# wangkenpu/rsrgan

Hardware: AMD Instinct MI355X
Metric: GAN train frames/sec (G+D step), 257-dim LPS->40-dim MFCC (higher is better)
Workload: dtype f32

## Files before the change

include/rsrgan.h:

```cpp
#ifndef RSRGAN_H_
#define RSRGAN_H_

#include <stddef.h>
#include <stdint.h>

#ifdef __cplusplus
extern "C" {
#endif

typedef enum rsrgan_status {
  RSRGAN_OK = 0,
  RSRGAN_ERR_INVALID = -1,
  RSRGAN_ERR_HIP = -2,
  RSRGAN_ERR_NO_DEVICE = -3,
  RSRGAN_ERR_STATE = -4
} rsrgan_status;

enum { RSRGAN_G_LSTM = 0, RSRGAN_G_RES_LSTM_L = 1, RSRGAN_G_RES_LSTM_BASE = 2,
       RSRGAN_G_DNN = 3,
       RSRGAN_G_RCED = 4,
       RSRGAN_G_BNLSTM = 5 ,
       RSRGAN_G_RES_LSTM_I = 6  };
enum { RSRGAN_D_LSTM = 0, RSRGAN_D_DNN = 1  };
enum { RSRGAN_NET_G = 0, RSRGAN_NET_D = 1 };

typedef enum rsrgan_scalar {
  RSRGAN_G_LEARNING_RATE = 0,
  RSRGAN_D_LEARNING_RATE = 1,
  RSRGAN_MSE_LAMBDA = 2,
  RSRGAN_D_REAL = 3,
  RSRGAN_D_FAKE = 4,
  RSRGAN_L2_SCALE = 5,
  RSRGAN_CLIP_NORM = 6,
  RSRGAN_ADAM_STEP = 7,
  RSRGAN_ADAM_STEP_D = 8,
  RSRGAN_SCALAR_COUNT_
} rsrgan_scalar;

typedef struct rsrgan_cfg {
  int32_t batch_size;
  int32_t max_frames;
  int32_t input_dim;
  int32_t output_dim;
  int32_t g_type;
  int32_t g_layers;
  int32_t g_cells;
  int32_t g_proj;
  int32_t d_type;
  int32_t d_layers;
  int32_t d_cells;
  int32_t d_proj;
  float   l2_scale;
  float   clip_norm;
  float   adam_beta1;
  float   adam_beta2;
  float   adam_eps;
  float   ema_decay;
  float   lrelu_alpha;
  float   forget_bias;
  int32_t cross_validation;
  int32_t flags;
  int32_t d_joint_off;
  int32_t d_joint_dim;
  int32_t g_splice;
} rsrgan_cfg;

enum {
  RSRGAN_FLAG_WAVEFRONT = 1,
  RSRGAN_FLAG_GRAPH = 2,
  RSRGAN_FLAG_NO_SPLITK_B = 8,
  RSRGAN_FLAG_SUPERVISED = 16,
  RSRGAN_FLAG_OVERLAP = 4,
  RSRGAN_FLAG_BATCH_NORM = 32
};

typedef struct rsrgan_handle_s* rsrgan_handle;

int rsrgan_default_cfg(int32_t g_type, rsrgan_cfg* cfg);

int rsrgan_create(const rsrgan_cfg* cfg, uint64_t seed, rsrgan_handle* out);
int rsrgan_destroy(rsrgan_handle h);
const char* rsrgan_last_error(void);

int rsrgan_set_scalar(rsrgan_handle h, int32_t which, double v);
int rsrgan_get_scalar(rsrgan_handle h, int32_t which, double* v);

int rsrgan_num_tensors(rsrgan_handle h, int32_t net);
int rsrgan_tensor_info(rsrgan_handle h, int32_t net, int32_t idx,
                       char* name, int32_t name_cap,
                       int32_t* rows, int32_t* cols, int64_t* dense_offset);
int64_t rsrgan_param_count(rsrgan_handle h, int32_t net);

int rsrgan_get_params(rsrgan_handle h, int32_t net, int32_t what, float* dense, void* stream);
int rsrgan_set_params(rsrgan_handle h, int32_t net, int32_t what, const float* dense, void* stream);
int rsrgan_get_grads(rsrgan_handle h, int32_t net, float* dense, void* stream);

int rsrgan_forward_g(rsrgan_handle h, const float* x, const int32_t* lengths, int32_t T,
                     float* y, void* stream);

int rsrgan_g_state_floats(rsrgan_handle h, int32_t* n);
int rsrgan_g_state_reset(rsrgan_handle h, const int32_t* row_mask, void* stream);
int rsrgan_g_state_get(rsrgan_handle h, float* dst, void* stream);
int rsrgan_g_state_set(rsrgan_handle h, const float* src, void* stream);
int rsrgan_forward_g_stream(rsrgan_handle h, const float* x, const int32_t* lengths, int32_t T,
                            float* y, void* stream);

int rsrgan_d_step(rsrgan_handle h, const float* x, const float* labels, const int32_t* lengths,
                  int32_t T, const float* noise_real, const float* noise_fake,
                  float* out_losses, int32_t train, void* stream);

int rsrgan_g_step(rsrgan_handle h, const float* x, const float* labels, const int32_t* lengths,
                  int32_t T, const float* noise_fake, float* out_losses,
                  int32_t train, int32_t reuse_g_forward, void* stream);

int rsrgan_d_backward(rsrgan_handle h, const float* x, const float* labels, const int32_t* lengths,
                      int32_t T, const float* noise_real, const float* noise_fake,
                      float* out_losses, void* stream);
int rsrgan_g_backward(rsrgan_handle h, const float* x, const float* labels, const int32_t* lengths,
                      int32_t T, const float* noise_fake, float* out_losses,
                      int32_t reuse_g_forward, void* stream);
int rsrgan_apply(rsrgan_handle h, int32_t net, void* stream);
int rsrgan_grad_buffer(rsrgan_handle h, int32_t net, float** ptr, int64_t* count);
int rsrgan_grad_bucket_count(rsrgan_handle h, int32_t net);
int rsrgan_grad_bucket_info(rsrgan_handle h, int32_t net, int32_t i, int64_t* offset, int64_t* count);
int rsrgan_grad_bucket_wait(rsrgan_handle h, int32_t net, int32_t i, void* stream);

int rsrgan_profile_begin(rsrgan_handle h);
int rsrgan_profile_read(rsrgan_handle h, int32_t* launches, double* total_us, double* alg_flops);
int rsrgan_profile_read_kind(rsrgan_handle h, int32_t kind, int32_t* launches, double* total_us, double* alg_flops);

int rsrgan_device_status(rsrgan_handle h, int32_t* code);

int rsrgan_set_dropout(rsrgan_handle h, float keep_prob, uint64_t seed);

int rsrgan_profile_launches(rsrgan_handle h, int64_t* n);
int rsrgan_op_launch_floor(int32_t n, int32_t mode, double* us_per_launch, void* stream);

int rsrgan_op_gemm(const float* A, int32_t lda, int32_t a_kcontig,
                   const float* B, int32_t ldb, int32_t b_kcontig,
                   float* C, int32_t ldc, int32_t M, int32_t N, int32_t K,
                   const float* bias, int32_t act, float alpha, int32_t accumulate, void* stream);

int rsrgan_op_gemm2(const float* A, int32_t lda, int32_t a_kcontig, const float* A2, int32_t lda2, int32_t M1,
                    const float* B, int32_t ldb, int32_t b_kcontig, float* C, int32_t ldc, int32_t M, int32_t N, int32_t K,
                    const float* bias, int32_t act, float alpha, int32_t accumulate,
                    int32_t map_rows_per, int64_t map_outer, int64_t map_inner, int32_t workers, int32_t force_cfg, void* stream);
#define RSRGAN_OP_NOT_APPLICABLE 1
int rsrgan_op_gemm_batch(int32_t nb, const float* const* A, int32_t lda, const float* const* A2, int32_t lda2, int32_t M1,
                         const float* const* B, int32_t ldb, float* const* C, int32_t ldc, int32_t M, int32_t N, int32_t K,
                         int32_t accumulate, int32_t workers, void* stream);
int rsrgan_op_gemm16_batch(int32_t n, const float* const* A, int32_t lda, const float* const* A2, int32_t lda2, int32_t M1,
                           const float* const* B, int32_t ldb, float* const* C, int32_t ldc, int32_t M, int32_t N, int32_t K,
                           int32_t accumulate, void* stream);
int rsrgan_op_gemm_last_plan(int32_t out[8]);
int rsrgan_op_lstm_colsums(int32_t nb, const float* const* dz, const float* const* cprev, const float* const* ccur, float* const* db,
                           float* const* dwi, float* const* dwf, float* const* dwo, int32_t rows, int32_t H, void* stream);
int rsrgan_op_colsum(const float* a, int32_t lda, const float* b, int32_t ldb, float* out, int32_t rows, int32_t cols, int32_t tall,
                     void* stream);

typedef struct rsrgan_segan_cfg {
  int32_t batch_size;
  int32_t input_len;
  int32_t output_dim;
  int32_t n_layers;
  int32_t g_depths[16];
  int32_t d_depths[16];
  int32_t g_kwidth;
  int32_t d_kwidth;
  int32_t g_prelu;
  float   lrelu_alpha;
  float   vbn_eps;
  float   rms_decay;
  float   rms_eps;
} rsrgan_segan_cfg;
typedef struct rsrgan_segan_handle_s* rsrgan_segan_handle;
enum { RSRGAN_SEGAN_G_LR = 0, RSRGAN_SEGAN_D_LR = 1, RSRGAN_SEGAN_L1_LAMBDA = 2 };
int rsrgan_segan_default_cfg(rsrgan_segan_cfg* cfg);
int rsrgan_segan_create(const rsrgan_segan_cfg* cfg, uint64_t seed, rsrgan_segan_handle* out);
int rsrgan_segan_destroy(rsrgan_segan_handle h);
int rsrgan_segan_set_scalar(rsrgan_segan_handle h, int32_t which, double v);
int rsrgan_segan_num_tensors(rsrgan_segan_handle h, int32_t net);
int rsrgan_segan_tensor_info(rsrgan_segan_handle h, int32_t net, int32_t idx, char* name, int32_t name_cap, int32_t* rows, int32_t* cols,
                             int64_t* dense_offset);
int64_t rsrgan_segan_param_count(rsrgan_segan_handle h, int32_t net);
int rsrgan_segan_get_params(rsrgan_segan_handle h, int32_t net, int32_t what, float* dense, void* stream);
int rsrgan_segan_set_params(rsrgan_segan_handle h, int32_t net, int32_t what, const float* dense, void* stream);
int rsrgan_segan_forward_g(rsrgan_segan_handle h, const float* x, const float* z, float* y, void* stream);
int rsrgan_segan_d_backward(rsrgan_segan_handle h, const float* x, const float* labels, const float* z, const float* noise_ref,
                            const float* noise_real, const float* noise_fake, float* out_losses, int32_t train, void* stream);
int rsrgan_segan_g_backward(rsrgan_segan_handle h, const float* x, const float* labels, const float* z, const float* noise_ref,
                            const float* noise_fake, float* out_losses, int32_t train, void* stream);
int rsrgan_segan_grad_buffer(rsrgan_segan_handle h, int32_t net, float** ptr, int64_t* count);
int rsrgan_segan_apply(rsrgan_segan_handle h, int32_t net, void* stream);

int rsrgan_version(void);

#ifdef __cplusplus
}
#endif
#endif
```

rsrgan_amd/_lib.py:

```python
from __future__ import annotations

import ctypes as C
import os

_HERE = os.path.dirname(os.path.abspath(__file__))
LIB_PATH = os.path.join(_HERE, "lib", "librsrgan_hip.so")

G_TYPES = {"lstm": 0, "res_lstm_l": 1, "res_lstm_base": 2, "dnn": 3, "rced": 4, "bnlstm": 5, "res_lstm_i": 6}
FLAG_BATCH_NORM = 32
D_TYPES = {"lstm": 0, "dnn": 1}
NET_G, NET_D = 0, 1
SCALARS = {"g_learning_rate": 0, "d_learning_rate": 1, "mse_lambda": 2, "d_real": 3, "d_fake": 4,
           "l2_scale": 5, "clip_norm": 6, "adam_step": 7, "adam_step_d": 8}
WHAT = {"variables": 0, "adam_m": 1, "adam_v": 2, "ema": 3}

SYMBOLS = ["rsrgan_default_cfg", "rsrgan_create", "rsrgan_destroy", "rsrgan_last_error", "rsrgan_set_scalar",
           "rsrgan_get_scalar", "rsrgan_num_tensors", "rsrgan_tensor_info", "rsrgan_param_count",
           "rsrgan_get_params", "rsrgan_set_params", "rsrgan_get_grads", "rsrgan_forward_g",
           "rsrgan_g_state_floats", "rsrgan_g_state_reset", "rsrgan_g_state_get", "rsrgan_g_state_set", "rsrgan_forward_g_stream",
           "rsrgan_d_step",
           "rsrgan_g_step", "rsrgan_d_backward", "rsrgan_g_backward", "rsrgan_apply", "rsrgan_grad_buffer",
           "rsrgan_grad_bucket_count", "rsrgan_grad_bucket_info", "rsrgan_grad_bucket_wait",
           "rsrgan_profile_begin", "rsrgan_profile_read", "rsrgan_profile_read_kind", "rsrgan_profile_launches", "rsrgan_op_launch_floor", "rsrgan_device_status", "rsrgan_set_dropout",
           "rsrgan_op_gemm", "rsrgan_op_gemm2", "rsrgan_op_gemm_batch", "rsrgan_op_gemm16_batch", "rsrgan_op_gemm_last_plan",
           "rsrgan_op_lstm_colsums", "rsrgan_op_colsum", "rsrgan_version",
           "rsrgan_segan_default_cfg", "rsrgan_segan_create", "rsrgan_segan_destroy", "rsrgan_segan_set_scalar",
           "rsrgan_segan_num_tensors", "rsrgan_segan_tensor_info", "rsrgan_segan_param_count", "rsrgan_segan_get_params",
           "rsrgan_segan_set_params", "rsrgan_segan_forward_g", "rsrgan_segan_d_backward", "rsrgan_segan_g_backward",
           "rsrgan_segan_grad_buffer", "rsrgan_segan_apply"]


class RsrganCfg(C.Structure):
    _fields_ = [("batch_size", C.c_int32), ("max_frames", C.c_int32), ("input_dim", C.c_int32),
                ("output_dim", C.c_int32), ("g_type", C.c_int32), ("g_layers", C.c_int32), ("g_cells", C.c_int32),
                ("g_proj", C.c_int32), ("d_type", C.c_int32), ("d_layers", C.c_int32), ("d_cells", C.c_int32),
                ("d_proj", C.c_int32), ("l2_scale", C.c_float), ("clip_norm", C.c_float), ("adam_beta1", C.c_float),
                ("adam_beta2", C.c_float), ("adam_eps", C.c_float), ("ema_decay", C.c_float),
                ("lrelu_alpha", C.c_float), ("forget_bias", C.c_float), ("cross_validation", C.c_int32),
                ("flags", C.c_int32), ("d_joint_off", C.c_int32), ("d_joint_dim", C.c_int32), ("g_splice", C.c_int32)]


class SeganCfg(C.Structure):
    _fields_ = [("batch_size", C.c_int32), ("input_len", C.c_int32), ("output_dim", C.c_int32), ("n_layers", C.c_int32),
                ("g_depths", C.c_int32 * 16), ("d_depths", C.c_int32 * 16), ("g_kwidth", C.c_int32), ("d_kwidth", C.c_int32),
                ("g_prelu", C.c_int32), ("lrelu_alpha", C.c_float), ("vbn_eps", C.c_float), ("rms_decay", C.c_float),
                ("rms_eps", C.c_float)]


class RsrganError(RuntimeError):
    pass


_lib = None


def load():
    global _lib
    if _lib is not None:
        return _lib
    if not os.path.exists(LIB_PATH):
        raise ImportError("%s is missing: build it with `python -c 'import __graft_entry__ as g; g.build()'` "
                          "(hipcc --offload-arch=gfx950); rsrgan_amd has no CPU fallback" % LIB_PATH)
    lib = C.CDLL(LIB_PATH)
    p, i32, i64, f32, vp = C.c_void_p, C.c_int32, C.c_int64, C.c_float, C.c_void_p
    lib.rsrgan_last_error.restype = C.c_char_p
    lib.rsrgan_default_cfg.argtypes = [i32, C.POINTER(RsrganCfg)]
    lib.rsrgan_create.argtypes = [C.POINTER(RsrganCfg), C.c_uint64, C.POINTER(vp)]
    lib.rsrgan_destroy.argtypes = [vp]
    lib.rsrgan_set_scalar.argtypes = [vp, i32, C.c_double]
    lib.rsrgan_get_scalar.argtypes = [vp, i32, C.POINTER(C.c_double)]
    lib.rsrgan_num_tensors.argtypes = [vp, i32]
    lib.rsrgan_tensor_info.argtypes = [vp, i32, i32, C.c_char_p, i32, C.POINTER(i32), C.POINTER(i32), C.POINTER(i64)]
    lib.rsrgan_param_count.argtypes = [vp, i32]
    lib.rsrgan_param_count.restype = i64
    lib.rsrgan_get_params.argtypes = [vp, i32, i32, p, vp]
    lib.rsrgan_set_params.argtypes = [vp, i32, i32, p, vp]
    lib.rsrgan_get_grads.argtypes = [vp, i32, p, vp]
    lib.rsrgan_forward_g.argtypes = [vp, p, p, i32, p, vp]
    lib.rsrgan_g_state_floats.argtypes = [vp, C.POINTER(i32)]
    lib.rsrgan_g_state_reset.argtypes = [vp, p, vp]
    lib.rsrgan_g_state_get.argtypes = [vp, p, vp]
    lib.rsrgan_g_state_set.argtypes = [vp, p, vp]
    lib.rsrgan_forward_g_stream.argtypes = [vp, p, p, i32, p, vp]
    lib.rsrgan_d_step.argtypes = [vp, p, p, p, i32, p, p, p, i32, vp]
    lib.rsrgan_g_step.argtypes = [vp, p, p, p, i32, p, p, i32, i32, vp]
    lib.rsrgan_d_backward.argtypes = [vp, p, p, p, i32, p, p, p, vp]
    lib.rsrgan_g_backward.argtypes = [vp, p, p, p, i32, p, p, i32, vp]
    lib.rsrgan_apply.argtypes = [vp, i32, vp]
    lib.rsrgan_grad_buffer.argtypes = [vp, i32, C.POINTER(p), C.POINTER(i64)]
    lib.rsrgan_grad_bucket_count.argtypes = [vp, i32]
    lib.rsrgan_grad_bucket_info.argtypes = [vp, i32, i32, C.POINTER(i64), C.POINTER(i64)]
    lib.rsrgan_grad_bucket_wait.argtypes = [vp, i32, i32, vp]
    lib.rsrgan_profile_begin.argtypes = [vp]
    lib.rsrgan_profile_read.argtypes = [vp, C.POINTER(i32), C.POINTER(C.c_double), C.POINTER(C.c_double)]
    lib.rsrgan_profile_read_kind.argtypes = [vp, i32, C.POINTER(i32), C.POINTER(C.c_double), C.POINTER(C.c_double)]
    lib.rsrgan_device_status.argtypes = [vp, C.POINTER(i32)]
    lib.rsrgan_set_dropout.argtypes = [vp, f32, C.c_uint64]
    lib.rsrgan_profile_launches.argtypes = [vp, C.POINTER(i64)]
    lib.rsrgan_op_launch_floor.argtypes = [i32, i32, C.POINTER(C.c_double), vp]
    lib.rsrgan_op_gemm.argtypes = [p, i32, i32, p, i32, i32, p, i32, i32, i32, i32, p, i32, f32, i32, vp]
    pp = C.POINTER(C.c_void_p)
    lib.rsrgan_op_gemm2.argtypes = [p, i32, i32, p, i32, i32, p, i32, i32, p, i32, i32, i32, i32, p, i32, f32, i32, i32, i64, i64, i32, i32, vp]
    lib.rsrgan_op_gemm_batch.argtypes = [i32, pp, i32, pp, i32, i32, pp, i32, pp, i32, i32, i32, i32, i32, i32, vp]
    lib.rsrgan_op_gemm16_batch.argtypes = [i32, pp, i32, pp, i32, i32, pp, i32, pp, i32, i32, i32, i32, i32, vp]
    lib.rsrgan_op_gemm_last_plan.argtypes = [C.POINTER(i32)]
    lib.rsrgan_op_lstm_colsums.argtypes = [i32, pp, pp, pp, pp, pp, pp, pp, i32, i32, vp]
    lib.rsrgan_op_colsum.argtypes = [p, i32, p, i32, p, i32, i32, i32, vp]
    lib.rsrgan_segan_default_cfg.argtypes = [C.POINTER(SeganCfg)]
    lib.rsrgan_segan_create.argtypes = [C.POINTER(SeganCfg), C.c_uint64, C.POINTER(vp)]
    lib.rsrgan_segan_destroy.argtypes = [vp]
    lib.rsrgan_segan_set_scalar.argtypes = [vp, i32, C.c_double]
    lib.rsrgan_segan_num_tensors.argtypes = [vp, i32]
    lib.rsrgan_segan_tensor_info.argtypes = [vp, i32, i32, C.c_char_p, i32, C.POINTER(i32), C.POINTER(i32), C.POINTER(i64)]
    lib.rsrgan_segan_param_count.argtypes = [vp, i32]
    lib.rsrgan_segan_param_count.restype = i64
    lib.rsrgan_segan_get_params.argtypes = [vp, i32, i32, p, vp]
    lib.rsrgan_segan_set_params.argtypes = [vp, i32, i32, p, vp]
    lib.rsrgan_segan_forward_g.argtypes = [vp, p, p, p, vp]
    lib.rsrgan_segan_d_backward.argtypes = [vp, p, p, p, p, p, p, p, i32, vp]
    lib.rsrgan_segan_g_backward.argtypes = [vp, p, p, p, p, p, p, i32, vp]
    lib.rsrgan_segan_grad_buffer.argtypes = [vp, i32, C.POINTER(p), C.POINTER(i64)]
    lib.rsrgan_segan_apply.argtypes = [vp, i32, vp]
    _lib = lib
    return lib


OP_NOT_APPLICABLE = 1
GEMM_CLASSES = {0: "none", 1: "gemm16", 2: "n32", 3: "k_gemm", 4: "k_gemm_s", 5: "gemm16_batch", 6: "k_gemm_batch", 7: "k_gemm_s_batch"}
GEMM_PLAN_FIELDS = ("cls", "bm", "bn", "W", "n_dp", "fixup", "splits", "Ur")
GEMM_FORMS = [("k_gemm", 128, 128), ("k_gemm", 96, 128), ("k_gemm", 128, 96), ("k_gemm", 256, 64), ("k_gemm", 256, 32),
              ("k_gemm_s", 256, 256), ("k_gemm_s", 128, 256), ("k_gemm_s", 256, 128)]


def ptr_table(ptrs):
    return (C.c_void_p * max(len(ptrs), 1))(*[None if q is None else q for q in ptrs])


def check(rc):
    if rc != 0:
        raise RsrganError("librsrgan_hip error %d: %s" % (rc, load().rsrgan_last_error().decode()))
```

rsrgan_amd/csrc/capi.cpp:

```cpp
#include <cstring>
#include <exception>
#include <new>
#include <vector>

#include "model.h"

using namespace rsr;

struct rsrgan_handle_s { Model m; };

#define CHECK_H(h)                                                    \
  if (!(h)) { set_error("null handle"); return RSRGAN_ERR_INVALID; }

template <class F>
static int guard(const char* what, F&& body) {
  try {
    return body();
  } catch (const std::bad_alloc&) {
    set_error("%s: out of host memory", what);
  } catch (const std::exception& e) {
    set_error("%s: %s", what, e.what());
  } catch (...) {
    set_error("%s: unknown C++ exception", what);
  }
// ... 459 lines not shown
  if (g) (void)hipGraphDestroy(g);
  if (s) (void)hipStreamDestroy(s);
  (void)stream;
  return rc;
}

static const size_t g_op_ws_floats = (size_t)32 << 20;
static const size_t g_op_scratch_floats = (size_t)2 << 20;
static float* op_ws() {
  static float* ws = nullptr;
  if (!ws && hipMalloc((void**)&ws, g_op_ws_floats * sizeof(float)) != hipSuccess) ws = nullptr;
  return ws;
}
static float* op_scratch() {
  static float* sc = nullptr;
  if (!sc && hipMalloc((void**)&sc, g_op_scratch_floats * sizeof(float)) != hipSuccess) sc = nullptr;
  return sc;
}
#define OP_REFUSE(cond, ...) do { if (cond) { set_error(__VA_ARGS__); return RSRGAN_ERR_INVALID; } } while (0)
struct WorkersScope {
  int saved;
  explicit WorkersScope(int w) : saved(g_gemm_workers) { if (w > 0) g_gemm_workers = w; }
  ~WorkersScope() { g_gemm_workers = saved; }
};

int rsrgan_op_gemm(const float* A, int32_t lda, int32_t a_kc, const float* B, int32_t ldb, int32_t b_kc, float* C, int32_t ldc,
                   int32_t M, int32_t N, int32_t K, const float* bias, int32_t act, float alpha, int32_t accumulate, void* stream) {
  if (!A || !B || !C || (lda & 3) || (ldb & 3)) { set_error("op_gemm: null pointer or leading dimension not a multiple of 4"); return RSRGAN_ERR_INVALID; }
  float* ws = op_ws();
  launch_gemm(A, lda, a_kc != 0, B, ldb, b_kc != 0, C, ldc, M, N, K, bias, act, alpha, accumulate != 0, (hipStream_t)stream,
              ws, ws ? g_op_ws_floats : 0);
  if (hipGetLastError() != hipSuccess) { set_error("op_gemm launch failed"); return RSRGAN_ERR_HIP; }
  return RSRGAN_OK;
}

int rsrgan_op_gemm2(const float* A, int32_t lda, int32_t a_kc, const float* A2, int32_t lda2, int32_t M1, const float* B, int32_t ldb,
                    int32_t b_kc, float* C, int32_t ldc, int32_t M, int32_t N, int32_t K, const float* bias, int32_t act, float alpha,
                    int32_t accumulate, int32_t map_rows_per, int64_t map_outer, int64_t map_inner, int32_t workers, int32_t force_cfg,
                    void* stream) {
  OP_REFUSE(!A || !B || !C, "op_gemm2: null pointer (A, B or C)");
  OP_REFUSE(M <= 0 || N <= 0 || K <= 0, "op_gemm2: M, N, K must be positive (got %d, %d, %d)", M, N, K);
  OP_REFUSE((lda & 3) || (ldb & 3) || (ldc & 3) || (A2 && (lda2 & 3)), "op_gemm2: leading dimension not a multiple of 4 (lda %d, lda2 %d, ldb %d, ldc %d)", lda, lda2, ldb, ldc);
  OP_REFUSE(workers < 0 || workers > 256, "op_gemm2: workers = %d outside 0 (default) .. 256", workers);
  OP_REFUSE(force_cfg < -1 || force_cfg > 7, "op_gemm2: force_cfg = %d outside -1 (planner) .. 7", force_cfg);
  OP_REFUSE(map_rows_per < 0, "op_gemm2: row map with rows_per = %d", map_rows_per);
  if (map_rows_per > 0) {
    OP_REFUSE(A2 != nullptr, "op_gemm2: A2 together with a row map");
    OP_REFUSE(b_kc != 0, "op_gemm2: a row map together with b_kcontig");
    OP_REFUSE((map_outer & 3) || (map_inner & 3), "op_gemm2: row map strides not multiples of 4 (outer %lld, inner %lld)", (long long)map_outer, (long long)map_inner);
  }
  if (A2) {
    OP_REFUSE(a_kc != 0, "op_gemm2: A2 together with a_kcontig (the stacked operand is m-contiguous)");
    OP_REFUSE(M1 <= 0 || M1 >= M, "op_gemm2: M1 = %d outside (0, M = %d)", M1, M);
    OP_REFUSE(M1 & 3, "op_gemm2: M1 = %d is not a multiple of 4: every kernel moves the stacked operand in 16-byte chunks", M1);
  }
  float* ws = op_ws();
  {
    WorkersScope wsc(workers);
    const GemmRowMap ma{map_rows_per, (long long)map_outer, (long long)map_inner};
    launch_gemm_mapped(A, lda, ma, A2, lda2, M1, a_kc != 0, B, ldb, b_kc != 0, C, ldc, M, N, K, bias, act, alpha, accumulate != 0,
                       (hipStream_t)stream, ws, ws ? g_op_ws_floats : 0, force_cfg);
  }
  if (hipGetLastError() != hipSuccess) { set_error("op_gemm2 launch failed"); return RSRGAN_ERR_HIP; }
  return RSRGAN_OK;
}

int rsrgan_op_gemm_batch(int32_t nb, const float* const* A, int32_t lda, const float* const* A2, int32_t lda2, int32_t M1,
                         const float* const* B, int32_t ldb, float* const* C, int32_t ldc, int32_t M, int32_t N, int32_t K,
                         int32_t accumulate, int32_t workers, void* stream) {
  OP_REFUSE(nb < 1 || nb > 64, "op_gemm_batch: nb = %d outside 1 .. 64 (more than %d: not applicable)", nb, GEMM_MAXB);
  OP_REFUSE(!A || !B || !C, "op_gemm_batch: null pointer table (A, B or C)");
  for (int b = 0; b < nb; ++b) OP_REFUSE(!A[b] || !B[b] || !C[b] || (A2 && !A2[b]), "op_gemm_batch: null pointer in problem %d", b);
  OP_REFUSE(M <= 0 || N <= 0 || K <= 0, "op_gemm_batch: M, N, K must be positive (got %d, %d, %d)", M, N, K);
  OP_REFUSE((lda & 3) || (ldb & 3) || (ldc & 3) || (A2 && (lda2 & 3)), "op_gemm_batch: leading dimension not a multiple of 4 (lda %d, lda2 %d, ldb %d, ldc %d)", lda, lda2, ldb, ldc);
  OP_REFUSE(workers < 0 || workers > 256, "op_gemm_batch: workers = %d outside 0 (default) .. 256", workers);
  if (A2) {
    OP_REFUSE(M1 <= 0 || M1 >= M, "op_gemm_batch: M1 = %d outside (0, M = %d)", M1, M);
    OP_REFUSE(M1 & 3, "op_gemm_batch: M1 = %d is not a multiple of 4: the kernels move the stacked operand in 16-byte chunks", M1);
  }
  float* ws = op_ws();
  bool ran;
  {
    WorkersScope wsc(workers);
    ran = launch_gemm_batch(nb, A, lda, A2, lda2, M1, B, ldb, C, ldc, M, N, K, accumulate != 0, (hipStream_t)stream, ws, ws ? g_op_ws_floats : 0);
  }
  if (hipGetLastError() != hipSuccess) { set_error("op_gemm_batch launch failed"); return RSRGAN_ERR_HIP; }
  return ran ? RSRGAN_OK : RSRGAN_OP_NOT_APPLICABLE;
}

int rsrgan_op_gemm16_batch(int32_t n, const float* const* A, int32_t lda, const float* const* A2, int32_t lda2, int32_t M1,
                           const float* const* B, int32_t ldb, float* const* C, int32_t ldc, int32_t M, int32_t N, int32_t K,
                           int32_t accumulate, void* stream) {
  OP_REFUSE(n < 1 || n > GEMM16_MAXB, "op_gemm16_batch: n = %d outside the table (1 .. %d)", n, GEMM16_MAXB);
  OP_REFUSE(!A || !B || !C, "op_gemm16_batch: null pointer table (A, B or C)");
  for (int p = 0; p < n; ++p) OP_REFUSE(!A[p] || !B[p] || !C[p] || (A2 && !A2[p]), "op_gemm16_batch: null pointer in problem %d", p);
  OP_REFUSE(M <= 0 || N <= 0 || K <= 0, "op_gemm16_batch: M, N, K must be positive (got %d, %d, %d)", M, N, K);
  OP_REFUSE((lda & 3) || (ldb & 3) || (ldc & 3) || (A2 && (lda2 & 3)), "op_gemm16_batch: leading dimension not a multiple of 4 (lda %d, lda2 %d, ldb %d, ldc %d)", lda, lda2, ldb, ldc);
  if (A2) {
    OP_REFUSE(M1 <= 0 || M1 >= M, "op_gemm16_batch: M1 = %d outside (0, M = %d)", M1, M);
    OP_REFUSE(M1 & 3, "op_gemm16_batch: M1 = %d is not a multiple of 4: k_gemm16 loads the stacked operand as float4", M1);
  }
  Gemm16Batch bt{};
  bt.n = n;
  for (int p = 0; p < n; ++p) { bt.A[p] = A[p]; bt.A2[p] = A2 ? A2[p] : nullptr; bt.B[p] = B[p]; bt.C[p] = C[p]; }
  float* ws = op_ws();
  launch_gemm16_batch(bt, lda, lda2, M1, ldb, ldc, M, N, K, accumulate != 0, (hipStream_t)stream, ws, ws ? g_op_ws_floats : 0);
  if (hipGetLastError() != hipSuccess) { set_error("op_gemm16_batch launch failed"); return RSRGAN_ERR_HIP; }
  return RSRGAN_OK;
}

int rsrgan_op_gemm_last_plan(int32_t out[8]) {
  OP_REFUSE(!out, "op_gemm_last_plan: null pointer");
  const GemmPlanRecord& r = g_gemm_last_plan;
  out[0] = r.cls; out[1] = r.bm; out[2] = r.bn; out[3] = r.W; out[4] = r.n_dp; out[5] = r.fixup; out[6] = r.splits; out[7] = r.Ur;
  return RSRGAN_OK;
}

int rsrgan_op_lstm_colsums(int32_t nb, const float* const* dz, const float* const* cprev, const float* const* ccur, float* const* db,
                           float* const* dwi, float* const* dwf, float* const* dwo, int32_t rows, int32_t H, void* stream) {
  OP_REFUSE(nb < 1 || nb > 4, "op_lstm_colsums: nb = %d outside the table (1 .. 4)", nb);
  OP_REFUSE(!dz || !cprev || !ccur || !db || !dwi || !dwf || !dwo, "op_lstm_colsums: null pointer table");
  for (int p = 0; p < nb; ++p)
    OP_REFUSE(!dz[p] || !cprev[p] || !ccur[p] || !db[p] || !dwi[p] || !dwf[p] || !dwo[p], "op_lstm_colsums: null pointer in layer %d", p);
  OP_REFUSE(rows <= 0 || H <= 0, "op_lstm_colsums: rows and H must be positive (got %d, %d)", rows, H);
  OP_REFUSE((size_t)nb * 64 * 7 * (size_t)H > g_op_scratch_floats, "op_lstm_colsums: nb x 64 x 7 x H = %zu floats of partials exceed the entry's scratch", (size_t)nb * 64 * 7 * (size_t)H);
  float* sc = op_scratch();
  if (!sc) { set_error("op_lstm_colsums: hipMalloc failed"); return RSRGAN_ERR_HIP; }
  if (nb == 1) launch_lstm_colsums(dz[0], cprev[0], ccur[0], db[0], dwi[0], dwf[0], dwo[0], rows, H, sc, (hipStream_t)stream);
  else {
    ColsumsBatch cb{};
    cb.n = nb;
    for (int p = 0; p < nb; ++p) { cb.dz[p] = dz[p]; cb.cprev[p] = cprev[p]; cb.ccur[p] = ccur[p]; cb.db[p] = db[p]; cb.dwi[p] = dwi[p]; cb.dwf[p] = dwf[p]; cb.dwo[p] = dwo[p]; }
    launch_lstm_colsums_batch(cb, rows, H, sc, (hipStream_t)stream);
  }
  if (hipGetLastError() != hipSuccess) { set_error("op_lstm_colsums launch failed"); return RSRGAN_ERR_HIP; }
  return RSRGAN_OK;
}

int rsrgan_op_colsum(const float* a, int32_t lda, const float* b, int32_t ldb, float* out, int32_t rows, int32_t cols, int32_t tall,
                     void* stream) {
  OP_REFUSE(!a || !out, "op_colsum: null pointer (a or out)");
  OP_REFUSE(rows <= 0 || cols <= 0, "op_colsum: rows and cols must be positive (got %d, %d)", rows, cols);
  OP_REFUSE(lda < cols || (b && ldb < cols), "op_colsum: leading dimension below cols = %d (lda %d, ldb %d)", cols, lda, ldb);
  OP_REFUSE(tall && b, "op_colsum: the tall form has no multiplier b");
  OP_REFUSE((size_t)(tall ? 512 : 64) * (size_t)cols > g_op_scratch_floats, "op_colsum: cols = %d exceeds the entry's scratch", cols);
  float* sc = op_scratch();
  if (!sc) { set_error("op_colsum: hipMalloc failed"); return RSRGAN_ERR_HIP; }
  if (tall) launch_colsum_tall(a, lda, out, rows, cols, sc, g_op_scratch_floats, (hipStream_t)stream);
  else launch_colsum(a, lda, b, ldb, out, rows, cols, sc, (hipStream_t)stream);
  if (hipGetLastError() != hipSuccess) { set_error("op_colsum launch failed"); return RSRGAN_ERR_HIP; }
  return RSRGAN_OK;
}

}
```

rsrgan_amd/csrc/dnn.cpp:

```cpp
#include "model.h"

namespace rsr {

#define HIPC(expr)                                                                   \
  do {                                                                               \
    hipError_t e_ = (expr);                                                          \
    if (e_ != hipSuccess) {                                                          \
      set_error("%s failed: %s (%s:%d)", #expr, hipGetErrorString(e_), __FILE__, __LINE__); \
      return RSRGAN_ERR_HIP;                                                         \
    }                                                                                \
  } while (0)

static const float kDClipLo = -0.5f, kDClipHi = 1.5f;

BnVars Model::bn_vars(const ParamSet& ps, const int (&tbn)[8]) const {
  BnVars v;
  v.beta = ps.W(tbn[0]); v.gamma = ps.W(tbn[1]); v.mm = ps.W(tbn[2]); v.mv = ps.W(tbn[3]);
  v.rm = ps.W(tbn[4]); v.rmw = ps.W(tbn[5]); v.rs = ps.W(tbn[6]); v.rsw = ps.W(tbn[7]);
  return v;
}
BnVars Model::bn_vars(const ParamSet& ps, const FcLayer& F) const { return bn_vars(ps, F.tbn); }

static inline uint64_t splitmix64(uint64_t x) {
  x += 0x9E3779B97F4A7C15ull;
// ... 68 lines not shown

void Model::rced_forward(int rows, hipStream_t s) {
  const size_t M = (size_t)rows * rcS * rcW;
  for (size_t l = 0; l < gconv.size(); ++l) {
    const ConvLayer& L = gconv[l];
    if (rc_ft_fwd[l]) {
      const float* src = rc_act[l];
      int ldc = L.ldCin;
      if (l == 0) { launch_expand_c4(x_tm, ldDin, rcS * rcW, rc_x4, (size_t)rows, s); src = rc_x4; ldc = 4; }
      launch_conv_fwd(src, ldc, L.Cin, rc_ft_fwd[l], L.bn ? nullptr : G.W(L.tb), !L.bn, L.bn ? L.pre : rc_act[l + 1], L.ldCout, L.Cout, rows,
                      rcS, rcW, L.fw, s);
    } else {
      float* col = rc_keep_cols ? rc_cols[l] : rc_col;
      launch_im2col(rc_act[l], l == 0 ? (size_t)ldDin : (size_t)rcS * rcW * L.ldCin, L.ldCin, L.Cin, rcS, rcW, rcS, L.fw, col, L.ldK, M, s);
      gemm(col, L.ldK, true, G.W(L.tW), L.ldCout, false, L.bn ? L.pre : rc_act[l + 1], L.ldCout, (int)M, L.Cout, L.K, L.bn ? nullptr : G.W(L.tb),
           L.bn ? 0 : 2, 0.f, false, s);
    }
    if (L.bn)
      launch_bn_forward(L.pre, L.ldCout, rc_act[l + 1], L.ldCout, (int)M, L.Cout, bn_vars(G, L.tbn), L.stat, L.ldCout, bn_training(), true,
                        scratch, scratch_floats, s);
  }
  gemm(rc_act[gconv.size()], rc_fc.ld_in, true, G.W(rc_fc.tW), ldDout, false, y_tm, ldDout, rows, Dout, rc_fc.in, G.W(rc_fc.tb), 0, 0.f, false, s);
}

void Model::rced_backward(int rows, float* dy, hipStream_t s) {
  const size_t M = (size_t)rows * rcS * rcW;
  const int Lc = (int)gconv.size();
  gemm(rc_act[Lc], rc_fc.ld_in, false, dy, ldDout, false, G.Gd(rc_fc.tW), ldDout, rc_fc.in, Dout, rows, nullptr, 0, 0.f, false, s);
  launch_colsum(dy, ldDout, nullptr, 0, G.Gd(rc_fc.tb), rows, Dout, scratch, s);
  float* d = rc_dA;
  float* other = rc_dB;
  gemm(dy, ldDout, true, G.W(rc_fc.tW), ldDout, true, d, rc_fc.ld_in, rows, rc_fc.in, Dout, nullptr, 0, 0.f, false, s);
  bool d_masked = false;
  for (int l = Lc - 1; l >= 0; --l) {
    const ConvLayer& L = gconv[l];
    if (L.bn)
      launch_bn_backward(d, L.ldCout, rc_act[l + 1], L.ldCout, L.pre, L.ldCout, (int)M, L.Cout, L.stat, L.ldCout, G.Gd(L.tbn[0]), G.Gd(L.tbn[1]),
                         false, true, bn_sums, scratch, scratch_floats, s);
    else if (!d_masked)
      launch_lrelu_bwd(rc_act[l + 1], d, M, L.Cout, L.ldCout, 0.f, s);
    d_masked = false;
    bool db_done = false;
    if (rc_wgrad_implicit[l] && rc_wg_ws) {
      launch_conv_wgrad(l == 0 ? rc_x4 : rc_act[l], l == 0 ? 4 : L.ldCin, L.Cin, d, L.ldCout, L.Cout, G.Gd(L.tW), L.ldCout, rc_wg_ws, rows,
                        rcS, rcW, L.fw, s, L.bn ? nullptr : G.Gd(L.tb));
      db_done = !L.bn;
    } else {
      float* col = rc_keep_cols ? rc_cols[l] : rc_col;
      if (!rc_keep_cols)
        launch_im2col(rc_act[l], l == 0 ? (size_t)ldDin : (size_t)rcS * rcW * L.ldCin, L.ldCin, L.Cin, rcS, rcW, rcS, L.fw, col, L.ldK, M, s);
      gemm(col, L.ldK, false, d, L.ldCout, false, G.Gd(L.tW), L.ldCout, L.K, L.Cout, (int)M, nullptr, 0, 0.f, false, s);
    }
    if (!L.bn && !db_done) launch_colsum_tall(d, L.ldCout, G.Gd(L.tb), (int)M, L.Cout, scratch, scratch_floats, s);
    if (l > 0) {
      if (rc_ft_bwd[l]) {
        d_masked = !gconv[l - 1].bn;
        launch_conv_fwd(d, L.ldCout, L.Cout, rc_ft_bwd[l], nullptr, false, other, L.ldCin, L.Cin, rows, rcS, rcW, L.fw, s,
                        d_masked ? rc_act[l] : nullptr);
      } else {
        gemm(d, L.ldCout, true, G.W(L.tW), L.ldCout, true, rc_dcol, L.ldK, (int)M, L.K, L.Cout, nullptr, 0, 0.f, false, s);
        launch_col2im(rc_dcol, L.ldK, L.Cin, rcS, rcW, rcS, L.fw, other, L.ldCin, M, s);
      }
      std::swap(d, other);
    }
  }
}

void Model::g_frame_forward(int rows, hipStream_t s) {
  if (g_rced()) rced_forward(rows, s);
  else fc_forward(G, gfc, g_act, rows, s);
}
void Model::g_frame_backward(int rows, float* dy, hipStream_t s) {
  if (g_rced()) rced_backward(rows, dy, s);
  else fc_backward(G, gfc, g_act, rows, dy, true, false, s);
}

void Model::bn_commit_run(bool with_d, hipStream_t s) {
  BnCommitList cl; cl.n = 0;
  bn_commit_stack(G, gfc, 2, 0, cl);
  for (const ConvLayer& L : gconv)
    if (L.bn && cl.n < 24) cl.e[cl.n++] = BnCommit{bn_vars(G, L.tbn), L.stat, L.Cout, L.ldCout, 2, 0};
  if (with_d) bn_commit_stack(D, dfc, 2, 1, cl);
  launch_bn_commit_many(cl, s);
}

void Model::d_dnn_forward_loss(int T, int Nd, int n_real, bool want_grads, float* loss3, hipStream_t s, int calls, int call0) {
  fc_forward(D, dfc, d_act, T * Nd, s, calls, call0);
  launch_lsgan(logits, 4, want_grads ? dlogits : nullptr, T, Nd, n_real, dyn + DYN_D_REAL,
               n_real > 0 ? dyn + DYN_D_FAKE : dyn + DYN_D_REAL, loss3, s, true, kDClipLo, kDClipHi);
}

int Model::dnn_d_backward(const float* x, const float* labels, int T, float* out_losses, bool want_grads, hipStream_t s) {
  const int R = T * B;
  if (!x || !labels) { set_error("null input pointer"); return RSRGAN_ERR_INVALID; }
  if (T <= 0 || T > Tmax) { set_error("T=%d outside (0, max_frames=%d]", T, Tmax); return RSRGAN_ERR_INVALID; }
  bn_eval_call = !want_grads;
  if (want_grads) ++drop_run;
  launch_pack_tm(x, x_tm, B, T, Din, ldDin, s);
  launch_pack_tm(labels, lab_tm, B, T, Dout, ldDout, s);
  cur_T = T;
  g_frame_forward(R, s);
  g_fwd_valid = true;
  launch_build_joint(x_tm, ldDin, cfg.d_joint_off, cfg.d_joint_dim, lab_tm, ldDout, Dout, joint, ldJ, 0, R, s);
  launch_build_joint(x_tm, ldDin, cfg.d_joint_off, cfg.d_joint_dim, y_tm, ldDout, Dout, joint, ldJ, R, R, s);
  d_dnn_forward_loss(1, 2 * R, R, want_grads, losses, s, 2);
  if (want_grads) {
    fc_backward(D, dfc, d_act, 2 * R, dlogits, true, false, s, 2);
    if (bn_training()) bn_commit_run(true, s);
    { finish_buckets(RSRGAN_NET_D, s); d_grads_ready = true; }
  }
  if (out_losses) launch_copy_f(losses, out_losses, 3, s);
  HIPC(hipGetLastError());
  return RSRGAN_OK;
}

int Model::dnn_g_backward(const float* x, const float* labels, int T, float* out_losses, bool want_grads, bool reuse, hipStream_t s) {
  const int R = T * B;
  bn_eval_call = !want_grads;
  if (bn_on()) reuse = false;
  if (want_grads) ++drop_run;
  if (drop_training()) reuse = false;
  if (reuse) {
    if (!g_fwd_valid || T != cur_T) { set_error("reuse_g_forward without a valid generator forward"); return RSRGAN_ERR_STATE; }
  } else {
    if (!x || !labels) { set_error("null input pointer"); return RSRGAN_ERR_INVALID; }
    if (T <= 0 || T > Tmax) { set_error("T=%d outside (0, max_frames=%d]", T, Tmax); return RSRGAN_ERR_INVALID; }
    launch_pack_tm(x, x_tm, B, T, Din, ldDin, s);
    launch_pack_tm(labels, lab_tm, B, T, Dout, ldDout, s);
    cur_T = T;
    g_frame_forward(R, s);
    g_fwd_valid = true;
  }
  const bool sup = supervised();
  if (sup) {
    HIPC(hipMemsetAsync(losses + 3, 0, sizeof(float), s));
  } else if (bn_training() && want_grads) {
    launch_build_joint(x_tm, ldDin, cfg.d_joint_off, cfg.d_joint_dim, lab_tm, ldDout, Dout, joint, ldJ, 0, R, s);
    launch_build_joint(x_tm, ldDin, cfg.d_joint_off, cfg.d_joint_dim, y_tm, ldDout, Dout, joint, ldJ, R, R, s);
    fc_forward(D, dfc, d_act, 2 * R, s, 2);
    launch_lsgan(logits + (size_t)R * 4, 4, dlogits + (size_t)R * 4, 1, R, 0, dyn + DYN_D_REAL, dyn + DYN_D_REAL, tmp3, s, true, kDClipLo, kDClipHi);
    launch_copy_f(tmp3 + 1, losses + 3, 1, s);
  } else {
    launch_build_joint(x_tm, ldDin, cfg.d_joint_off, cfg.d_joint_dim, y_tm, ldDout, Dout, joint, ldJ, 0, R, s);
    d_dnn_forward_loss(1, R, 0, want_grads, tmp3, s, 1, 1);
    launch_copy_f(tmp3 + 1, losses + 3, 1, s);
  }
  const bool l2_on = !cfg.cross_validation && scal[RSRGAN_L2_SCALE] > 0.0;
  if (want_grads) {
    if (!sup) {
      float* dj = bn_training() ? fc_backward(D, dfc, d_act, R, dlogits + (size_t)R * 4, false, true, s, 1, R, 1)
                                : fc_backward(D, dfc, d_act, R, dlogits, false, true, s);
      launch_slice_cols(dj, ldJ, cfg.d_joint_dim, dy_buf, ldDout, R, Dout, s);
    }
    launch_mse(y_tm, lab_tm, ldDout, dy_buf, R, Dout, dyn + DYN_LAMBDA, !sup, losses + 4, scratch, s);
    g_frame_backward(R, dy_buf, s);
    if (l2_on) {
      launch_l2(G.w, G.g, G.ct, dyn + DYN_L2, G.partial, s);
      launch_l2_total(G.partial, G.ct.n_chunks, dyn + DYN_L2, losses + 5, s);
    }
    if (bn_training()) bn_commit_run(!sup, s);
    { finish_buckets(RSRGAN_NET_G, s); g_grads_ready = true; }
  } else {
    launch_mse(y_tm, lab_tm, ldDout, nullptr, R, Dout, dyn + DYN_LAMBDA, false, losses + 4, scratch, s);
  }
  if (!(want_grads && l2_on)) HIPC(hipMemsetAsync(losses + 5, 0, sizeof(float), s));
  launch_g_total(losses + 3, dyn + DYN_LAMBDA, s);
  if (out_losses) launch_copy_f(losses + 3, out_losses, 4, s);
  HIPC(hipGetLastError());
  return RSRGAN_OK;
}

}
```

rsrgan_amd/csrc/kernels.h:

```cpp
#pragma once
#include <hip/hip_runtime.h>
#include <stdint.h>

#include "switches.h"

namespace rsr {

constexpr int MAXJ = 8;

struct Place { int x0, nx, sb, se, nb, w; };
constexpr int JOBMAP_MAX = 768;
struct JobMap { int valid; unsigned char job[JOBMAP_MAX]; };
struct PlanItem { int ncol, nrow; double cost; int mult; };
int plan_places(int n, const PlanItem* items, Place* out);

enum { DYN_G_LR = 0, DYN_D_LR = 1, DYN_LAMBDA = 2, DYN_D_REAL = 3, DYN_D_FAKE = 4, DYN_L2 = 5, DYN_CLIP = 6,
       DYN_B1 = 7, DYN_B2 = 8, DYN_EPS = 9, DYN_EMA = 10, DYN_ADAM_LRT = 11, DYN_ADAM_LRT_D = 12, DYN_COUNT = 16 };

struct FwdGateJob {
  const float* x;
  const float* KxT;
  const float* m;
  const float* KhT;
  const float* Wsw;
// ... 136 lines not shown
  const float *KxT, *KhT;
  const float *bias, *wi, *wf, *wo, *Wp;
  float *gates, *c, *h, *mst, *out;
  const float* in;
  float* dmt;
  int I, P, ldI, ldP, ldH;
  float* res_out;
};
struct GPersistArgs {
  GPersistLayer L[GP_MAXL];
  int nl, N, T, H;
  int NT, NC;
  const int* len;
  unsigned long long *gran1, *gran2;
  unsigned* ctl;
  float forget_bias;
  unsigned long long* gran3;
  const float* dout_top;
  int ld_dout;
  float* din0;
  int ld_din0;
  int res;
  int tags;
  int dout_trail;
  int fwd_trail;
  int ngl, grp0;
  int nrt;
  int sched;
  int carry;
};
constexpr int GP_TMAX = 2046;
bool gpersist_plan(GPersistArgs& a);
void gpersist_arm_bytes(void* p, size_t bytes, hipStream_t s);
extern thread_local int g_gemm_workers;
int gpersist_grid(const GPersistArgs& a);
int gpersist_dt_grid(const GPersistArgs& a, const DPersistArgs& d);
void launch_glstm_fwd_dt(const GPersistArgs& a, const DPersistArgs& d, hipStream_t s);
size_t dpersist_fwdt_lds_bytes();
void launch_glstm_bwd_dt(const GPersistArgs& a, const DPersistArgs& d, hipStream_t s);
size_t gpersist_lds_bytes();
int device_cu_count();
bool resident_probe(int grid, int threads, size_t lds_bytes);
size_t gpersist_gran1_bytes(const GPersistArgs& a);
size_t gpersist_gran2_bytes(const GPersistArgs& a);
size_t gpersist_gran3_bytes(const GPersistArgs& a);
void gpersist_arm(const GPersistArgs& a, hipStream_t s);
void launch_glstm_fwd(const GPersistArgs& a, hipStream_t s);
bool gpersist_np_plan(GPersistArgs& a, int nt_force = 0);
size_t gpersist_np_gran2_bytes(const GPersistArgs& a);
size_t gpersist_np_lds_bytes();
void launch_glstm_np_fwd(const GPersistArgs& a, hipStream_t s);
size_t gpersist_np_gran1_bytes(const GPersistArgs& a);
size_t gpersist_np_gran3_bytes(const GPersistArgs& a);
void gpersist_np_arm(const GPersistArgs& a, hipStream_t s);
void launch_glstm_np_bwd(const GPersistArgs& a, hipStream_t s);
void launch_glstm_bwd(const GPersistArgs& a, hipStream_t s);
extern long long g_chain_launches;
void launch_floor_chain(float* a, float* b, int n, int mode, hipStream_t s);

struct GemmRowMap { int rows_per; long long outer; long long inner; };
enum { GEMM_CLS_NONE = 0, GEMM_CLS_GEMM16 = 1, GEMM_CLS_N32 = 2, GEMM_CLS_KGEMM = 3, GEMM_CLS_KGEMM_S = 4, GEMM_CLS_GEMM16_B = 5,
       GEMM_CLS_KGEMM_B = 6, GEMM_CLS_KGEMM_S_B = 7 };
struct GemmPlanRecord { int cls, bm, bn, W, n_dp, fixup, splits, Ur; };
extern thread_local GemmPlanRecord g_gemm_last_plan;
void launch_gemm_mapped(const float* A, int lda, const GemmRowMap& ma, const float* A2, int lda2, int M1, bool a_kc, const float* B, int ldb,
                        bool b_kc, float* C, int ldc, int M, int N, int K, const float* bias, int act, float alpha,
                        bool accumulate, hipStream_t s, float* ws, size_t ws_floats, int force_cfg = -1);
constexpr int GEMM16_MAXB = 4;
struct Gemm16Batch { const float* A[GEMM16_MAXB]; const float* A2[GEMM16_MAXB]; const float* B[GEMM16_MAXB]; float* C[GEMM16_MAXB]; int n; };
void launch_gemm16_batch(const Gemm16Batch& bt, int lda, int lda2, int M1, int ldb, int ldc, int M, int N, int K, bool accumulate,
                         hipStream_t s, float* ws, size_t ws_floats);
void launch_gemm2(const float* A, int lda, const float* A2, int lda2, int M1, bool a_kc, const float* B, int ldb, bool b_kc,
                  float* C, int ldc, int M, int N, int K, const float* bias, int act, float alpha, bool accumulate,
                  hipStream_t s, float* ws, size_t ws_floats);
constexpr int GEMM_MAXB = 4;
bool launch_gemm_batch(int nb, const float* const* A, int lda, const float* const* A2, int lda2, int M1, const float* const* B, int ldb,
                       float* const* C, int ldc, int M, int N, int K, bool accumulate, hipStream_t s, float* ws, size_t ws_floats);
void launch_gemm(const float* A, int lda, bool a_kc, const float* B, int ldb, bool b_kc,
                 float* C, int ldc, int M, int N, int K,
                 const float* bias, int act, float alpha, bool accumulate, hipStream_t s,
                 float* splitk_ws = nullptr, size_t splitk_ws_floats = 0);

struct StagePack { const float* src; float* dst; int D, ld; };
struct StageCopy { const void* src; void* dst; int n; };
struct StageJobs { StagePack pack[2]; StageCopy copy[4]; int B, T; int Bt; };
void launch_stage_inputs(const StageJobs& j, hipStream_t s);
void launch_pack_tm(const float* src_bm, float* dst_tm, int B, int T, int D, int ld, hipStream_t s);
void launch_unpack_bm(const float* src_tm, int ld, float* dst_bm, int B, int T, int D, hipStream_t s, int Bt = 0);
void launch_build_d_input(const float* lab_tm, const float* y_tm, const float* noise_r, const float* noise_f,
                          float* xd, int B, int T, int D, int ld, bool with_real, hipStream_t s);
void launch_add_noise_rows(const float* src_tm, const float* noise, float* dst, int B, int T, int D, int ld,
                           int Ns, int row0, hipStream_t s);
void launch_transpose(const float* src, int lds, float* dst, int ldd, int R, int C, hipStream_t s);
void launch_fill(float* p, size_t n, float v, hipStream_t s);
struct SwizzleJob { const float* src; float* dst; int ld, gates, H, C, c0, K1, I, P, kx, nct, nkb, blk_base; };
struct SwizzleList { int n; SwizzleJob j[24]; };
void launch_swizzle_many(SwizzleList& sl, hipStream_t s);
inline size_t swizzle_floats(int nct, int nkb) { return (size_t)nct * nkb * 256; }
struct TransposeJob { const float* src; float* dst; int lds, ldd, R, C, blk_base; };
struct TransposeList { int n; TransposeJob j[16]; };
void launch_transpose_many(TransposeList& tl, hipStream_t s);
size_t conv_prep_floats(int S, int fw, int C);
void launch_conv_prep(const float* F, int ldf_src, int S, int fw, int Cin, int Cout, bool flip, float* Ft, hipStream_t s);
bool conv_fwd_supported(int C, int N, int S, int W, int fw);
void launch_conv_fwd(const float* in, int ldc_in, int C, const float* Ft, const float* bias, bool relu, float* out, int ldc_out, int N,
                     int R, int S, int W, int fw, hipStream_t s,
                     const float* mask = nullptr );
bool conv_wgrad_supported(int C, int N, int S, int W, int fw);
size_t conv_wgrad_ws_floats(int C, int R, int S, int W, int fw);
void launch_conv_wgrad(const float* in, int ldc_in, int C, const float* d, int ldc_d, int N, float* dW, int ldw, float* ws, int R, int S,
                       int W, int fw, hipStream_t s,
                       float* db = nullptr );
void launch_im2col(const float* src, size_t row_stride, int ldc, int C, int S, int W, int kh, int kw, float* col, int ldk, size_t M,
                   hipStream_t s);
void launch_expand_c4(const float* src, int ld_src, int n, float* dst, size_t rows, hipStream_t s);
void launch_col2im(const float* dcol, int ldk, int C, int S, int W, int kh, int kw, float* dst, int ldc, size_t M, hipStream_t s);
struct GStateLayer { float *c, *mst; int H, P, ldP, off; };
struct GStateArgs { GStateLayer L[GP_MAXL]; int nl, SF, rows, dir; float* state; size_t slot; const int* mask; };
void launch_gstate(const GStateArgs& a, hipStream_t s);
struct ZeroList { int n; float* p[32]; unsigned len[32]; };
void launch_zero_many(const ZeroList& zl, hipStream_t s);
struct ColsumsBatch { const float* dz[4]; const float* cprev[4]; const float* ccur[4]; float* db[4]; float* dwi[4]; float* dwf[4]; float* dwo[4]; int n; };
void launch_lstm_colsums_batch(const ColsumsBatch& bt, int rows, int H, float* scratch, hipStream_t s);
void launch_lstm_colsums(const float* dz, const float* cprev, const float* ccur, float* db, float* dwi, float* dwf, float* dwo,
                         int rows, int H, float* scratch , hipStream_t s);
void launch_lrelu_bwd(const float* hval, float* d, size_t rows, int cols, int ld, float alpha, hipStream_t s);
void launch_dropout_fwd(float* y, size_t rows, int cols, int ld, unsigned long long key, unsigned thr, float keep, hipStream_t s);
void launch_dropout_bwd(const float* y, float* d, size_t rows, int cols, int ld, float keep, hipStream_t s);
void launch_colsum_tall(const float* a, int lda, float* out, int rows, int cols, float* scratch, size_t scratch_floats, hipStream_t s);

struct BnVars {
  float *beta, *gamma;
  float *mm, *mv, *rm, *rmw, *rs, *rsw;
};
constexpr int BN_STAT_ROWS = 6;
void launch_bn_forward(const float* z, int ldz, float* y, int ldy, int rows, int cols, const BnVars& v, float* stat, int ldc, bool training,
                       bool relu, float* scratch, size_t scratch_floats, hipStream_t s, int calls = 1);
void launch_bn_backward(float* dy, int ldd, const float* y, int ldy, const float* z, int ldz, int rows, int cols, const float* stat, int ldc,
                        float* dbeta, float* dgamma, bool accumulate, bool relu, float* sums, float* scratch, size_t scratch_floats,
                        hipStream_t s, int calls = 1);
void launch_bn_commit(int cols, const BnVars& v, const float* stat, int ldc, int times, hipStream_t s);
struct BnCommit { BnVars v; const float* stat; int cols, ldc, times0, times1; };
struct BnCommitList { int n; BnCommit e[24]; };
void launch_bn_commit_many(const BnCommitList& cl, hipStream_t s);
void launch_colsum(const float* a, int lda, const float* b, int ldb, float* out, int rows, int cols,
                   float* scratch , hipStream_t s);

constexpr int DH_MAXR = 64;
struct DHeadArgs {
  const float* top; int ldt; const float* w; int ldw; const float* b;
  float* logits; int ldl; float* dlogits; float* dout; int ldo; float* gw; float* gb;
  int T, Nd, n_real, dR; const float* t_real; const float* t_fake; float* loss3; float* part; int want_grads, want_wgrads;
  int Bp, Bt;
};
void launch_dhead(const DHeadArgs& a, hipStream_t s);
void launch_lsgan(const float* logits, int ldl, float* dlogits, int T, int Nd, int n_real,
                  const float* target_real, const float* target_fake, float* loss3, hipStream_t s,
                  bool clip_on = false, float clip_lo = 0.f, float clip_hi = 0.f, int Bp = 0, int Bt = 0);
void launch_build_joint(const float* x, int ldx, int off, int dim, const float* tail, int ldt, int Dt, float* joint, int ldj,
                        int row0, int R, hipStream_t s);
void launch_slice_cols(const float* src, int lds, int off, float* dst, int ldd, int R, int C, hipStream_t s);
void launch_mse(const float* y, const float* lab, int ld, float* dy, int rows, int D, const float* lambda,
                bool accumulate, float* loss_out, float* scratch , hipStream_t s, int Bp = 0, int Bt = 0);
void launch_g_total(float* l4 , const float* lambda, hipStream_t s);
void launch_copy_f(const float* src, float* dst, int n, hipStream_t s);

struct ChunkTable {
  const int* tensor;
  const int* off;
  const int* len;
  const int* t_first;
  const int* t_count;
  const int* t_l2;
  int n_chunks, n_tensors;
};
void launch_sumsq(const float* g, const ChunkTable& ct, float* partial, hipStream_t s);
void launch_dw_reduce(const float* ws, size_t stride, int ntiles, const long long* src, float* g, const ChunkTable& ct, float* partial, hipStream_t s);
void launch_l2(const float* w, float* g, const ChunkTable& ct, const float* l2_scale, float* partial, hipStream_t s);
void launch_l2_total(const float* partial, int n_chunks, const float* l2_scale, float* out, hipStream_t s);
void launch_apply_sgd(float* w, const float* g, float* ema, const ChunkTable& ct, const float* partial,
                      const float* dyn, hipStream_t s);
void launch_apply_adam(float* w, const float* g, float* m, float* v, float* ema, const ChunkTable& ct,
                       const float* partial, const float* dyn, hipStream_t s, int lrt_slot = DYN_ADAM_LRT);
void launch_adam_tick(float* dyn, int* t, double b1, double b2, hipStream_t s, int lr_slot = DYN_G_LR, int lrt_slot = DYN_ADAM_LRT);
void launch_pad_copy(const float* dense, float* padded, int rows, int cols, int ld, bool to_padded, hipStream_t s);

}
```

rsrgan_amd/csrc/kernels.hip:

```cpp
#include <algorithm>
#include <cstdlib>

#include "kernels.h"

namespace rsr {

typedef float f32x4 __attribute__((ext_vector_type(4)));

__device__ __forceinline__ float sigmoid_(float x) { return 1.0f / (1.0f + expf(-x)); }

#ifdef RSR_TRACE
__device__ unsigned long long g_trace[8192 * 16];
#define TR_BEGIN() do { if (threadIdx.x == 0 && blockIdx.x < 8192) { unsigned long long* t_ = g_trace + (size_t)blockIdx.x * 16; \
    t_[0] = __builtin_amdgcn_s_memrealtime(); t_[1] = __builtin_amdgcn_s_memtime(); \
    t_[14] = __builtin_amdgcn_s_getreg(4 | (0 << 6) | (31 << 11)); t_[15] = __builtin_amdgcn_s_getreg(20 | (0 << 6) | (3 << 11)); \
    for (int i_ = 2; i_ < 14; ++i_) t_[i_] = 0; } } while (0)
#define TR_ID(ptr) do { if (threadIdx.x == 0 && blockIdx.x < 8192) g_trace[(size_t)blockIdx.x * 16 + 12] = (unsigned long long)(size_t)(ptr); } while (0)
#define TR(i) do { if (threadIdx.x == 0 && blockIdx.x < 8192) g_trace[(size_t)blockIdx.x * 16 + (i)] = __builtin_amdgcn_s_memtime(); } while (0)
#define TR_END() do { if (threadIdx.x == 0 && blockIdx.x < 8192) { g_trace[(size_t)blockIdx.x * 16 + 9] = __builtin_amdgcn_s_memtime(); \
    g_trace[(size_t)blockIdx.x * 16 + 13] = __builtin_amdgcn_s_memrealtime(); } } while (0)
#else
#define TR_BEGIN() do { } while (0)
#define TR_ID(ptr) do { } while (0)
#define TR(i) do { } while (0)
// ... 1346 lines not shown
  __syncthreads();
  if (g == 0 && c < cols) out[c] = ((red[0][threadIdx.x] + red[1][threadIdx.x]) + red[2][threadIdx.x]) + red[3][threadIdx.x];
}
void launch_colsum_tall(const float* a, int lda, float* out, int rows, int cols, float* scratch, size_t scratch_floats, hipStream_t s) {
  int slices = (int)std::min<size_t>(512, scratch_floats / (size_t)std::max(cols, 1));
  slices = std::max(1, std::min(slices, (rows + 63) / 64));
  const int per = (rows + slices - 1) / slices;
  slices = (rows + per - 1) / per;
  hipLaunchKernelGGL(k_colsum1_n, dim3((cols + 63) / 64, slices), dim3(256), 0, s, a, lda, scratch, rows, cols, per);
  hipLaunchKernelGGL(k_colsum2_n, dim3((cols + 63) / 64), dim3(256), 0, s, scratch, out, cols, slices);
}

__global__ __launch_bounds__(256) void k_lstm_colsums1(const float* __restrict__ dz, const float* __restrict__ cprev,
                                                       const float* __restrict__ ccur, float* __restrict__ scratch, int rows, int H) {
  __shared__ float red[7][4][64];
  const int c = blockIdx.x * 64 + (threadIdx.x & 63), rl = threadIdx.x >> 6;
  const int per = (rows + CS_SLICES - 1) / CS_SLICES;
  const int rbeg = blockIdx.y * per, rend = min(rows, rbeg + per);
  float s[7] = {0.f, 0.f, 0.f, 0.f, 0.f, 0.f, 0.f};
  if (c < H) {
#pragma unroll 4
    for (int r = rbeg + rl; r < rend; r += 4) {
      const float* z = dz + (size_t)r * 4 * H + c;
      const float di = z[0], dj = z[H], df = z[2 * H], d_o = z[3 * H];
      const float cp = cprev[(size_t)r * H + c], cc = ccur[(size_t)r * H + c];
      s[0] += di; s[1] += dj; s[2] += df; s[3] += d_o; s[4] += di * cp; s[5] += df * cp; s[6] += d_o * cc;
    }
  }
#pragma unroll
  for (int k = 0; k < 7; ++k) red[k][rl][threadIdx.x & 63] = s[k];
  __syncthreads();
  if (rl == 0 && c < H) {
    const int x = threadIdx.x;
#pragma unroll
    for (int k = 0; k < 7; ++k)
      scratch[((size_t)blockIdx.y * 7 + k) * H + c] = ((red[k][0][x] + red[k][1][x]) + red[k][2][x]) + red[k][3][x];
  }
}
__global__ void k_lstm_colsums2(const float* __restrict__ scratch, float* __restrict__ db, float* __restrict__ dwi,
                                float* __restrict__ dwf, float* __restrict__ dwo, int H) {
  const int c = blockIdx.x * blockDim.x + threadIdx.x;
  if (c >= H) return;
  float s[7] = {0.f, 0.f, 0.f, 0.f, 0.f, 0.f, 0.f};
#pragma unroll 8
  for (int i = 0; i < CS_SLICES; ++i)
#pragma unroll
    for (int k = 0; k < 7; ++k) s[k] += scratch[((size_t)i * 7 + k) * H + c];
  db[c] = s[0]; db[H + c] = s[1]; db[2 * H + c] = s[2]; db[3 * H + c] = s[3];
  dwi[c] = s[4]; dwf[c] = s[5]; dwo[c] = s[6];
}
__global__ __launch_bounds__(256) void k_lstm_colsums1_b(const ColsumsBatch bt, float* __restrict__ scratch, int rows, int H) {
  __shared__ float red[7][4][64];
  const int p = blockIdx.z;
  const float* __restrict__ dz = bt.dz[p]; const float* __restrict__ cprev = bt.cprev[p]; const float* __restrict__ ccur = bt.ccur[p];
  scratch += (size_t)p * CS_SLICES * 7 * H;
  const int c = blockIdx.x * 64 + (threadIdx.x & 63), rl = threadIdx.x >> 6;
  const int per = (rows + CS_SLICES - 1) / CS_SLICES;
  const int rbeg = blockIdx.y * per, rend = min(rows, rbeg + per);
  float s[7] = {0.f, 0.f, 0.f, 0.f, 0.f, 0.f, 0.f};
  if (c < H) {
#pragma unroll 4
    for (int r = rbeg + rl; r < rend; r += 4) {
      const float* z = dz + (size_t)r * 4 * H + c;
      const float di = z[0], dj = z[H], df = z[2 * H], d_o = z[3 * H];
      const float cp = cprev[(size_t)r * H + c], cc = ccur[(size_t)r * H + c];
      s[0] += di; s[1] += dj; s[2] += df; s[3] += d_o; s[4] += di * cp; s[5] += df * cp; s[6] += d_o * cc;
    }
  }
#pragma unroll
  for (int k = 0; k < 7; ++k) red[k][rl][threadIdx.x & 63] = s[k];
  __syncthreads();
  if (rl == 0 && c < H) {
    const int x = threadIdx.x;
#pragma unroll
    for (int k = 0; k < 7; ++k)
      scratch[((size_t)blockIdx.y * 7 + k) * H + c] = ((red[k][0][x] + red[k][1][x]) + red[k][2][x]) + red[k][3][x];
  }
}
__global__ void k_lstm_colsums2_b(const float* __restrict__ scratch, const ColsumsBatch bt, int H) {
  const int p = blockIdx.y;
  scratch += (size_t)p * CS_SLICES * 7 * H;
  const int c = blockIdx.x * blockDim.x + threadIdx.x;
  if (c >= H) return;
  float s[7] = {0.f, 0.f, 0.f, 0.f, 0.f, 0.f, 0.f};
#pragma unroll 8
  for (int i = 0; i < CS_SLICES; ++i)
#pragma unroll
    for (int k = 0; k < 7; ++k) s[k] += scratch[((size_t)i * 7 + k) * H + c];
  float* db = bt.db[p];
  db[c] = s[0]; db[H + c] = s[1]; db[2 * H + c] = s[2]; db[3 * H + c] = s[3];
  bt.dwi[p][c] = s[4]; bt.dwf[p][c] = s[5]; bt.dwo[p][c] = s[6];
}
void launch_lstm_colsums_batch(const ColsumsBatch& bt, int rows, int H, float* scratch, hipStream_t s) {
  hipLaunchKernelGGL(k_lstm_colsums1_b, dim3((H + 63) / 64, CS_SLICES, bt.n), dim3(256), 0, s, bt, scratch, rows, H);
  hipLaunchKernelGGL(k_lstm_colsums2_b, dim3((H + 255) / 256, bt.n), dim3(256), 0, s, scratch, bt, H);
}
void launch_lstm_colsums(const float* dz, const float* cprev, const float* ccur, float* db, float* dwi, float* dwf, float* dwo,
                         int rows, int H, float* scratch, hipStream_t s) {
  hipLaunchKernelGGL(k_lstm_colsums1, dim3((H + 63) / 64, CS_SLICES), dim3(256), 0, s, dz, cprev, ccur, scratch, rows, H);
  hipLaunchKernelGGL(k_lstm_colsums2, dim3((H + 255) / 256), dim3(256), 0, s, scratch, db, dwi, dwf, dwo, H);
}

void launch_colsum(const float* a, int lda, const float* b, int ldb, float* out, int rows, int cols, float* scratch, hipStream_t s) {
  hipLaunchKernelGGL(k_colsum1, dim3((cols + 63) / 64, CS_SLICES), dim3(256), 0, s, a, lda, b, ldb, scratch, rows, cols);
  hipLaunchKernelGGL(k_colsum2, dim3((cols + 255) / 256), dim3(256), 0, s, scratch, out, cols);
}

__device__ __forceinline__ float block_sum_1024(float v, float* red) {
  for (int o = 32; o > 0; o >>= 1) v += __shfl_down(v, o, 64);
  const int w = threadIdx.x >> 6;
  if ((threadIdx.x & 63) == 0) red[w] = v;
  __syncthreads();
  float s = 0.f;
  const int nw = (blockDim.x + 63) >> 6;
  for (int i = 0; i < nw; ++i) s += red[i];
  __syncthreads();
  return s;
}

__global__ __launch_bounds__(1024) void k_lsgan(const float* __restrict__ logits, int ldl, float* __restrict__ dlogits,
                                                int T, int Nd, int n_real, const float* __restrict__ t_real,
                                                const float* __restrict__ t_fake, float* __restrict__ loss3,
                                                int clip_on, float clip_lo, float clip_hi, int Bp, int Bt) {
  __shared__ float red[16];
  const int rows = T * Nd;
  const float tr = *t_real, tf = *t_fake;
  const int nr_ = Bp > 0 ? n_real / Bp * Bt : n_real, nf_ = Bp > 0 ? (Nd - n_real) / Bp * Bt : Nd - n_real;
  const float cr = (float)T * (float)nr_, cf = (float)T * (float)nf_;
  float sr = 0.f, sf = 0.f;
  for (int r = threadIdx.x; r < rows; r += blockDim.x) {
    const bool real = (r % Nd) < n_real;
    const bool valid = Bp <= 0 || ((r % Nd) % Bp) < Bt;
    const float raw = logits[(size_t)r * ldl];
    const float val = clip_on ? fminf(fmaxf(raw, clip_lo), clip_hi) : raw;
    const float d = valid ? val - (real ? tr : tf) : 0.f;
    if (real) sr += d * d; else sf += d * d;
    if (dlogits) dlogits[(size_t)r * ldl] = (clip_on && (raw < clip_lo || raw > clip_hi)) ? 0.f : 2.f * d / (real ? cr : cf);
  }
  sr = block_sum_1024(sr, red);
  sf = block_sum_1024(sf, red);
  if (threadIdx.x == 0) {
    const float lr_ = n_real > 0 ? sr / cr : 0.f;
    const float lf_ = (Nd - n_real) > 0 ? sf / cf : 0.f;
    loss3[0] = lr_; loss3[1] = lf_; loss3[2] = lr_ + lf_;
  }
}
void launch_lsgan(const float* logits, int ldl, float* dlogits, int T, int Nd, int n_real,
                  const float* t_real, const float* t_fake, float* loss3, hipStream_t s, bool clip_on, float clip_lo, float clip_hi,
                  int Bp, int Bt) {
  hipLaunchKernelGGL(k_lsgan, dim3(1), dim3(1024), 0, s, logits, ldl, dlogits, T, Nd, n_real, t_real, t_fake, loss3,
                     clip_on ? 1 : 0, clip_lo, clip_hi, Bp, Bt);
}

__global__ __launch_bounds__(64) void k_dhead1(const DHeadArgs a) {
  __shared__ float wsh[DH_MAXR + 1];
  const int lane = threadIdx.x;
  const int rows = a.T * a.Nd, dR = a.dR;
  if (lane < dR) wsh[lane] = a.w[(size_t)lane * a.ldw];
  if (lane == 0) wsh[DH_MAXR] = a.b[0];
  __syncthreads();
  const int r = blockIdx.x * 64 + lane;
  const bool on = r < rows;
  const float tr = *a.t_real, tf = *a.t_fake;
  const int nr_ = a.Bp > 0 ? a.n_real / a.Bp * a.Bt : a.n_real, nf_ = a.Bp > 0 ? (a.Nd - a.n_real) / a.Bp * a.Bt : a.Nd - a.n_real;
  const float cr = (float)a.T * (float)nr_, cf = (float)a.T * (float)nf_;
  float x[DH_MAXR];
  float logit = wsh[DH_MAXR];
  const float* xr = a.top + (size_t)(on ? r : 0) * a.ldt;
#pragma unroll
  for (int c = 0; c < DH_MAXR; c += 4) {
    float4 v = make_float4(0.f, 0.f, 0.f, 0.f);
    if (c < dR) v = *reinterpret_cast<const float4*>(xr + c);
    x[c] = v.x; x[c + 1] = v.y; x[c + 2] = v.z; x[c + 3] = v.w;
  }
#pragma unroll
  for (int c = 0; c < DH_MAXR; ++c) if (c < dR) logit += x[c] * wsh[c];
  const bool real = on && (r % a.Nd) < a.n_real;
  const bool valid = a.Bp <= 0 || ((r % a.Nd) % a.Bp) < a.Bt;
  const float d = valid ? logit - (real ? tr : tf) : 0.f;
  float sr = (on && real) ? d * d : 0.f, sf = (on && !real) ? d * d : 0.f;
  const float dl = on ? 2.f * d / (real ? cr : cf) : 0.f;
  if (on) {
    a.logits[(size_t)r * a.ldl] = logit;
    if (a.want_grads) {
      a.dlogits[(size_t)r * a.ldl] = dl;
      float* o = a.dout + (size_t)r * a.ldo;
#pragma unroll
      for (int c = 0; c < DH_MAXR; c += 4)
        if (c < dR) *reinterpret_cast<float4*>(o + c) = make_float4(dl * wsh[c], dl * wsh[c + 1], dl * wsh[c + 2], dl * wsh[c + 3]);
    }
  }
  auto wsum = [&](float v) { for (int o = 32; o > 0; o >>= 1) v += __shfl_down(v, o, 64); return v; };
  float* part = a.part + (size_t)blockIdx.x * (DH_MAXR + 3);
  sr = wsum(sr); sf = wsum(sf);
  if (lane == 0) { part[0] = sr; part[1] = sf; }
  if (a.want_wgrads) {
    const float sd = wsum(dl);
    if (lane == 0) part[2] = sd;
#pragma unroll
    for (int c = 0; c < DH_MAXR; ++c)
      if (c < dR) { const float v = wsum(x[c] * dl); if (lane == 0) part[3 + c] = v; }
  }
}
__global__ __launch_bounds__(1024) void k_dhead2(const DHeadArgs a, int nblocks) {
  __shared__ float tot[DH_MAXR + 3];
  const int q = threadIdx.x >> 4, j = threadIdx.x & 15;
  const int nq = a.want_wgrads ? 3 + a.dR : 2;
  float s = 0.f;
  if (q < nq)
    for (int b = j; b < nblocks; b += 16) s += a.part[(size_t)b * (DH_MAXR + 3) + q];
  s += __shfl_xor(s, 8); s += __shfl_xor(s, 4); s += __shfl_xor(s, 2); s += __shfl_xor(s, 1);
  if (q < nq && j == 0) {
    tot[q] = s;
    if (a.want_wgrads) {
      if (q == 2) a.gb[0] = s;
      if (q >= 3) a.gw[(size_t)(q - 3) * a.ldw] = s;
    }
  }
  __syncthreads();
  if (threadIdx.x == 0) {
    const int nr_ = a.Bp > 0 ? a.n_real / a.Bp * a.Bt : a.n_real, nf_ = a.Bp > 0 ? (a.Nd - a.n_real) / a.Bp * a.Bt : a.Nd - a.n_real;
    const float cr = (float)a.T * (float)nr_, cf = (float)a.T * (float)nf_;
    const float lr_ = a.n_real > 0 ? tot[0] / cr : 0.f;
    const float lf_ = (a.Nd - a.n_real) > 0 ? tot[1] / cf : 0.f;
    a.loss3[0] = lr_; a.loss3[1] = lf_; a.loss3[2] = lr_ + lf_;
  }
}
void launch_dhead(const DHeadArgs& a, hipStream_t s) {
  const int rows = a.T * a.Nd, nb = (rows + 63) / 64;
  hipLaunchKernelGGL(k_dhead1, dim3(nb), dim3(64), 0, s, a);
  hipLaunchKernelGGL(k_dhead2, dim3(1), dim3(1024), 0, s, a, nb);
}

__global__ void k_build_joint(const float* __restrict__ x, int ldx, int off, int dim, const float* __restrict__ tail, int ldt, int Dt,
                              float* __restrict__ joint, int ldj, int row0, int R) {
  const int W = dim + Dt;
  const size_t total = (size_t)R * W;
  for (size_t i = (size_t)blockIdx.x * blockDim.x + threadIdx.x; i < total; i += (size_t)gridDim.x * blockDim.x) {
    const int r = (int)(i / W), c = (int)(i % W);
    joint[(size_t)(row0 + r) * ldj + c] = c < dim ? x[(size_t)r * ldx + off + c] : tail[(size_t)r * ldt + (c - dim)];
  }
}
void launch_build_joint(const float* x, int ldx, int off, int dim, const float* tail, int ldt, int Dt, float* joint, int ldj,
                        int row0, int R, hipStream_t s) {
  const size_t total = (size_t)R * (dim + Dt);
  const int blocks = (int)min((size_t)2048, (total + 255) / 256);
  hipLaunchKernelGGL(k_build_joint, dim3(blocks), dim3(256), 0, s, x, ldx, off, dim, tail, ldt, Dt, joint, ldj, row0, R);
}
__global__ void k_slice_cols(const float* __restrict__ src, int lds_, int off, float* __restrict__ dst, int ldd, int R, int C) {
  const size_t total = (size_t)R * C;
  for (size_t i = (size_t)blockIdx.x * blockDim.x + threadIdx.x; i < total; i += (size_t)gridDim.x * blockDim.x) {
    const int r = (int)(i / C), c = (int)(i % C);
    dst[(size_t)r * ldd + c] = src[(size_t)r * lds_ + off + c];
  }
}
void launch_slice_cols(const float* src, int lds_, int off, float* dst, int ldd, int R, int C, hipStream_t s) {
  const size_t total = (size_t)R * C;
  const int blocks = (int)min((size_t)2048, (total + 255) / 256);
  hipLaunchKernelGGL(k_slice_cols, dim3(blocks), dim3(256), 0, s, src, lds_, off, dst, ldd, R, C);
}

constexpr int MSE_BLOCKS = 256;
__global__ __launch_bounds__(256) void k_mse1(const float* __restrict__ y, const float* __restrict__ lab, int ld,
                                              float* __restrict__ dy, int rows, int D, const float* __restrict__ lambda,
                                              int accumulate, float* __restrict__ scratch, int Bp, int Bt) {
  __shared__ float red[16];
  const size_t total = (size_t)rows * D;
  const int rows_eff = Bp > 0 ? rows / Bp * Bt : rows;
  const float scale = dy ? (*lambda) / (float)rows_eff : 0.f;
  float s = 0.f;
  for (size_t i = (size_t)blockIdx.x * blockDim.x + threadIdx.x; i < total; i += (size_t)gridDim.x * blockDim.x) {
    const size_t r = i / D; const int c = (int)(i % D);
    const size_t o = r * ld + c;
    const bool valid = Bp <= 0 || (int)(r % Bp) < Bt;
    const float d = valid ? y[o] - lab[o] : 0.f;
    s += d * d;
    if (dy) dy[o] = (accumulate ? dy[o] : 0.f) + scale * d;
  }
  s = block_sum_1024(s, red);
  if (threadIdx.x == 0) scratch[blockIdx.x] = s;
}
__global__ void k_mse2(const float* __restrict__ scratch, int rows, float* __restrict__ out) {
  if (threadIdx.x == 0) {
    float s = 0.f;
    for (int i = 0; i < MSE_BLOCKS; ++i) s += scratch[i];
    *out = 0.5f * s / (float)rows;
  }
}
void launch_mse(const float* y, const float* lab, int ld, float* dy, int rows, int D, const float* lambda,
                bool accumulate, float* loss_out, float* scratch, hipStream_t s, int Bp, int Bt) {
  hipLaunchKernelGGL(k_mse1, dim3(MSE_BLOCKS), dim3(256), 0, s, y, lab, ld, dy, rows, D, lambda, accumulate ? 1 : 0, scratch, Bp, Bt);
  hipLaunchKernelGGL(k_mse2, dim3(1), dim3(64), 0, s, scratch, Bp > 0 ? rows / Bp * Bt : rows, loss_out);
}

__global__ void k_g_total(float* l4, const float* lambda) {
  if (threadIdx.x == 0) l4[3] = l4[0] + (*lambda) * l4[1] + l4[2];
}
void launch_g_total(float* l4, const float* lambda, hipStream_t s) {
  hipLaunchKernelGGL(k_g_total, dim3(1), dim3(64), 0, s, l4, lambda);
}
__global__ void k_copy_f(const float* src, float* dst, int n) {
  const int i = blockIdx.x * blockDim.x + threadIdx.x;
  if (i < n) dst[i] = src[i];
}
void launch_copy_f(const float* src, float* dst, int n, hipStream_t s) {
  hipLaunchKernelGGL(k_copy_f, dim3((n + 255) / 256), dim3(256), 0, s, src, dst, n);
}


__global__ __launch_bounds__(256) void k_sumsq(const float* __restrict__ g, ChunkTable ct, float* __restrict__ partial) {
  __shared__ float red[16];
  const int c = blockIdx.x;
  const float* p = g + ct.off[c];
  const int n = ct.len[c];
  float s = 0.f;
  for (int i = threadIdx.x * 4; i < n; i += 1024) {
    const float4 v = *reinterpret_cast<const float4*>(p + i);
    s += (v.x * v.x + v.y * v.y) + (v.z * v.z + v.w * v.w);
  }
  s = block_sum_1024(s, red);
  if (threadIdx.x == 0) partial[c] = s;
}
void launch_sumsq(const float* g, const ChunkTable& ct, float* partial, hipStream_t s) {
  hipLaunchKernelGGL(k_sumsq, dim3(ct.n_chunks), dim3(256), 0, s, g, ct, partial);
}

__global__ __launch_bounds__(256) void k_dw_reduce(const float* __restrict__ ws, size_t stride, int ntiles, const long long* __restrict__ src,
                                                   float* __restrict__ g, ChunkTable ct, float* __restrict__ partial) {
  __shared__ float red[16];
  const int c = blockIdx.x;
  const int t = ct.tensor[c];
  const int off = ct.off[c], n = ct.len[c];
  const long long so = src[t];
  float s = 0.f;
  if (so < 0) {
    for (int i = threadIdx.x * 4; i < n; i += 1024) {
      const float4 v = *reinterpret_cast<const float4*>(g + off + i);
      s += (v.x * v.x + v.y * v.y) + (v.z * v.z + v.w * v.w);
    }
  } else {
    const float* p = ws + so + (off - ct.off[ct.t_first[t]]);
    for (int i = threadIdx.x * 4; i < n; i += 1024) {
      float4 a = *reinterpret_cast<const float4*>(p + i);
      for (int r = 1; r < ntiles; ++r) {
        const float4 b = *reinterpret_cast<const float4*>(p + (size_t)r * stride + i);
        a.x += b.x; a.y += b.y; a.z += b.z; a.w += b.w;
      }
      *reinterpret_cast<float4*>(g + off + i) = a;
      s += (a.x * a.x + a.y * a.y) + (a.z * a.z + a.w * a.w);
    }
  }
  s = block_sum_1024(s, red);
  if (threadIdx.x == 0) partial[c] = s;
}
void launch_dw_reduce(const float* ws, size_t stride, int ntiles, const long long* src, float* g, const ChunkTable& ct, float* partial, hipStream_t s) {
  hipLaunchKernelGGL(k_dw_reduce, dim3(ct.n_chunks), dim3(256), 0, s, ws, stride, ntiles, src, g, ct, partial);
}

__global__ __launch_bounds__(256) void k_l2(const float* __restrict__ w, float* __restrict__ g, ChunkTable ct,
                                            const float* __restrict__ l2_scale, float* __restrict__ partial) {
  __shared__ float red[16];
  const int c = blockIdx.x;
  const bool on = ct.t_l2[ct.tensor[c]] != 0;
  const int off = ct.off[c], n = ct.len[c];
  const float sc = *l2_scale;
  float s = 0.f;
  if (on) {
    for (int i = threadIdx.x; i < n; i += 256) {
      const float v = w[off + i];
      s += v * v;
      g[off + i] += sc * v;
    }
  }
  s = block_sum_1024(s, red);
  if (threadIdx.x == 0) partial[c] = s;
}
void launch_l2(const float* w, float* g, const ChunkTable& ct, const float* l2_scale, float* partial, hipStream_t s) {
  hipLaunchKernelGGL(k_l2, dim3(ct.n_chunks), dim3(256), 0, s, w, g, ct, l2_scale, partial);
}
__global__ __launch_bounds__(1024) void k_l2_total(const float* __restrict__ partial, int n, const float* __restrict__ l2_scale, float* out) {
  __shared__ float red[16];
  float s = 0.f;
  for (int i = threadIdx.x; i < n; i += blockDim.x) s += partial[i];
  s = block_sum_1024(s, red);
  if (threadIdx.x == 0) *out = 0.5f * (*l2_scale) * s;
}
void launch_l2_total(const float* partial, int n, const float* l2_scale, float* out, hipStream_t s) {
  hipLaunchKernelGGL(k_l2_total, dim3(1), dim3(1024), 0, s, partial, n, l2_scale, out);
}

__device__ __forceinline__ float tensor_clip_scale(const ChunkTable& ct, const float* partial, int c, float clip, float* red) {
  const int t = ct.tensor[c];
  const int first = ct.t_first[t], cnt = ct.t_count[t];
  float s = 0.f;
  for (int i = threadIdx.x; i < cnt; i += blockDim.x) s += partial[first + i];
  s = block_sum_1024(s, red);
  if (!(clip > 0.f)) return 1.0f;
  const float inv = s > 0.f ? 1.0f / sqrtf(s) : __builtin_inff();
  return clip * fminf(inv, 1.0f / clip);
}

__global__ __launch_bounds__(256) void k_apply_sgd(float* __restrict__ w, const float* __restrict__ g, float* __restrict__ ema,
                                                   ChunkTable ct, const float* __restrict__ partial, const float* __restrict__ dyn) {
  __shared__ float red[16];
  const int c = blockIdx.x;
  const float scale = tensor_clip_scale(ct, partial, c, dyn[DYN_CLIP], red);
  const float lr = dyn[DYN_D_LR], dec = dyn[DYN_EMA];
  const int off = ct.off[c], n = ct.len[c];
  for (int i = threadIdx.x; i < n; i += 256) {
    const float nw = w[off + i] - lr * (g[off + i] * scale);
    w[off + i] = nw;
    if (ema) ema[off + i] = dec * ema[off + i] + (1.f - dec) * nw;
  }
}
void launch_apply_sgd(float* w, const float* g, float* ema, const ChunkTable& ct, const float* partial, const float* dyn, hipStream_t s) {
  hipLaunchKernelGGL(k_apply_sgd, dim3(ct.n_chunks), dim3(256), 0, s, w, g, ema, ct, partial, dyn);
}

__global__ __launch_bounds__(256) void k_apply_adam(float* __restrict__ w, const float* __restrict__ g, float* __restrict__ m,
                                                    float* __restrict__ v, float* __restrict__ ema, ChunkTable ct,
                                                    const float* __restrict__ partial, const float* __restrict__ dyn, int lrt_slot) {
  __shared__ float red[16];
  const int c = blockIdx.x;
  const float scale = tensor_clip_scale(ct, partial, c, dyn[DYN_CLIP], red);
  const float b1 = dyn[DYN_B1], b2 = dyn[DYN_B2], eps = dyn[DYN_EPS], lrt = dyn[lrt_slot], dec = dyn[DYN_EMA];
  const int off = ct.off[c], n = ct.len[c];
  for (int i = threadIdx.x; i < n; i += 256) {
    const float gg = g[off + i] * scale;
    const float mm = b1 * m[off + i] + (1.f - b1) * gg;
    const float vv = b2 * v[off + i] + (1.f - b2) * gg * gg;
    m[off + i] = mm; v[off + i] = vv;
    const float nw = w[off + i] - lrt * mm / (sqrtf(vv) + eps);
    w[off + i] = nw;
    if (ema) ema[off + i] = dec * ema[off + i] + (1.f - dec) * nw;
  }
}
void launch_apply_adam(float* w, const float* g, float* m, float* v, float* ema, const ChunkTable& ct,
                       const float* partial, const float* dyn, hipStream_t s, int lrt_slot) {
  hipLaunchKernelGGL(k_apply_adam, dim3(ct.n_chunks), dim3(256), 0, s, w, g, m, v, ema, ct, partial, dyn, lrt_slot);
}

__global__ void k_adam_tick(float* dyn, int* t, double b1, double b2, int lr_slot, int lrt_slot) {
  if (threadIdx.x == 0) {
    const int tt = *t + 1;
    *t = tt;
    dyn[lrt_slot] = (float)((double)dyn[lr_slot] * sqrt(1.0 - pow(b2, (double)tt)) / (1.0 - pow(b1, (double)tt)));
  }
}
void launch_adam_tick(float* dyn, int* t, double b1, double b2, hipStream_t s, int lr_slot, int lrt_slot) {
  hipLaunchKernelGGL(k_adam_tick, dim3(1), dim3(64), 0, s, dyn, t, b1, b2, lr_slot, lrt_slot);
}

__global__ void k_pad_copy(const float* __restrict__ dense_c, float* __restrict__ dense_m, float* __restrict__ padded,
                           int rows, int cols, int ld, int to_padded) {
  const size_t total = (size_t)rows * cols;
  for (size_t i = (size_t)blockIdx.x * blockDim.x + threadIdx.x; i < total; i += (size_t)gridDim.x * blockDim.x) {
    const size_t r = i / cols; const int c = (int)(i % cols);
    if (to_padded) padded[r * ld + c] = dense_c[i];
    else dense_m[i] = padded[r * ld + c];
  }
}
void launch_pad_copy(const float* dense, float* padded, int rows, int cols, int ld, bool to_padded, hipStream_t s) {
  const size_t total = (size_t)rows * cols;
  const int blocks = (int)min((size_t)1024, (total + 255) / 256);
  hipLaunchKernelGGL(k_pad_copy, dim3(blocks), dim3(256), 0, s, dense, const_cast<float*>(dense), padded, rows, cols, ld, to_padded ? 1 : 0);
}

}
```

rsrgan_amd/csrc/model.cpp:

```cpp
#include "model.h"

#include <cmath>
#include <cstdarg>
#include <cstdio>
#include <cstdlib>
#include <cstring>
#include <random>

namespace rsr {

static thread_local char g_err[512] = "";
void set_error(const char* fmt, ...) {
  va_list ap;
  va_start(ap, fmt);
  vsnprintf(g_err, sizeof(g_err), fmt, ap);
  va_end(ap);
}
const char* get_error() { return g_err; }

#define HIPC(expr)                                                                   \
  do {                                                                               \
    hipError_t e_ = (expr);                                                          \
    if (e_ != hipSuccess) {                                                          \
      set_error("%s failed: %s (%s:%d)", #expr, hipGetErrorString(e_), __FILE__, __LINE__); \
// ... 354 lines not shown
        g_res.push_back(alloc<float>(TB * ldP));
        g_ins[l + 1] = g_res.back();
      } else {
        g_ins[l + 1] = g_st[l].out;
      }
    }
  }
  const int gmaxld = std::max(std::max(ldP, ldDin), ldDout);
  g_dA = alloc<float>(TB * gmaxld); g_dB = alloc<float>(TB * gmaxld); g_dC = alloc<float>(TB * gmaxld);
  const size_t TB2 = TB * 2;
  const int ldPd = d_dnn() ? 4 : pad4(dR);
  xd = alloc<float>(TB2 * ldDout); logits = alloc<float>(TB2 * 4); dlogits = alloc<float>(TB2 * 4);
  if (d_dnn()) {
    ldJ = pad4(c.d_joint_dim + Dout);
    if (c.d_joint_dim > 0) joint = alloc<float>(TB2 * ldJ);
    d_act.push_back(c.d_joint_dim > 0 ? joint : xd);
    for (size_t l = 0; l + 1 < dfc.size(); ++l) d_act.push_back(alloc<float>(TB2 * dfc[l].ld_out));
    d_act.push_back(logits);
    dy_buf = alloc<float>(TB * ldDout);
  }
  if (g_dnn() || d_dnn()) {
    int mx = std::max(ldJ, ldDin);
    for (auto& F : gfc) mx = std::max(mx, std::max(F.ld_in, F.ld_out));
    for (auto& F : dfc) mx = std::max(mx, std::max(F.ld_in, F.ld_out));
    fc_dA = alloc<float>(TB2 * mx); fc_dB = alloc<float>(TB2 * mx);
    if (bn_on()) {
      bn_sums = alloc<float>((size_t)2 * mx);
      for (auto& F : gfc) if (F.bn) { F.pre = alloc<float>(TB * F.ld_out); F.stat = alloc<float>((size_t)2 * BN_STAT_ROWS * F.ld_out); }
      for (auto& F : dfc) if (F.bn) { F.pre = alloc<float>(TB2 * F.ld_out); F.stat = alloc<float>((size_t)2 * BN_STAT_ROWS * F.ld_out); }
    }
  }
  adam_t_dev_d = alloc<int>(1);
  d_st.resize(dl.size());
  for (size_t l = 0; l < dl.size(); ++l) alloc_stash(*this, d_st[l], dl[l], 2 * B, Tmax);
  {
    bool ok = sw.dfold && !dl.empty();
    for (auto& L : dl) ok = ok && L.has_proj && L.H <= 288 && (L.ldH & 3) == 0;
    if (ok) {
      dl_fold.resize(dl.size()); dl_fold_K.resize(dl.size()); d_fold_st.resize(dl.size());
      for (size_t l = 0; l < dl.size(); ++l) {
        LstmLayer F = dl[l];
        F.has_proj = false; F.tWp = -1;
        F.I = l == 0 ? dl[0].I : dl[l - 1].H; F.ldI = l == 0 ? dl[0].ldI : dl[l - 1].ldH;
        F.P = dl[l].H; F.ldP = dl[l].ldH;
        F.KxT = F.KhT = F.WpT = nullptr; F.WpT_sw = F.Wp_sw = F.Kb_full = F.Kb_rec = nullptr;
        const int ncb = (F.H + 15) / 16;
        F.Wg_full = alloc<float>(swizzle_floats(4 * ncb, (F.ldI + F.ldP + 15) / 16));
        F.Wg_h = alloc<float>(swizzle_floats(4 * ncb, (F.ldP + 15) / 16));
        dl_fold_K[l] = alloc<float>((size_t)(F.I + F.H) * 4 * F.H);
        dl_fold[l] = F;
        LstmStash S = d_st[l];
        S.mst = alloc<float>((size_t)(Tmax + 1) * 2 * B * F.ldP);
        S.out = nullptr; S.dmt = nullptr; S.dmst = nullptr;
        d_fold_st[l] = S;
      }
    }
  }
  if (dp_live && !dl.empty() && dl.size() <= (size_t)DP_MAXL && B % 16 == 0) {
    const int nl_ = (int)dl.size();
    for (int rows : {2 * B, B}) {
      const int g_ = dpersist_grid(nl_, rows);
      if (g_ <= 128 && resident_probe(g_, 512, dpersist_lds_bytes())) { dp_max_grid = g_; break; }
    }
  }
  if (dp_max_grid > 0) {
    dp_gran_bytes = dpersist_granule_bytes((int)dl.size(), 2 * B, Tmax);
    dp_gran = (unsigned long long*)alloc<float>(dp_gran_bytes / sizeof(float));
    dp_ctl = (unsigned*)alloc<float>(16);
    HIPC(ctl_reset(dp_ctl));
    DPersistArgs pa{};
    pa.nl = (int)dl.size(); pa.N = 2 * B; pa.H = dl[0].H;
    for (size_t l = 0; l < dl.size(); ++l) { pa.L[l].I = dl[l].I; pa.L[l].P = dl[l].P; pa.L[l].ldP = dl[l].ldP; pa.L[l].ldI = dl[l].ldI; }
    bool shapes = switches().dw_inkernel && (dp_live & 2) && dpersist_dw_supported(pa) && !d_adam();
    for (auto& L : dl) shapes = shapes && L.has_proj && L.H == dl[0].H && L.ldH == dl[0].ldH;
    if (shapes && dpersist_grid(pa.nl, pa.N) == dp_max_grid) {
      const int nt = pa.N / 16;
      dw_stride = dpersist_dw_stride(pa);
      dw_ws = alloc<float>((size_t)pa.nl * nt * dw_stride);
      dw_flag = (unsigned*)alloc<float>(dpersist_dw_flag_bytes(pa.nl, pa.N, Tmax) / sizeof(float));
      std::vector<long long> src(D.t.size(), -1);
      const int IP = dl[0].I + dl[0].P, H4 = 4 * dl[0].H, H_ = dl[0].H;
      for (size_t l = 0; l < dl.size(); ++l) {
        const long long base = (long long)l * nt * (long long)dw_stride;
        src[dl[l].tK] = base; src[dl[l].tb] = base + (long long)IP * H4;
        const long long pp = base + (long long)(IP + 1) * H4;
        src[dl[l].twi] = pp; src[dl[l].twf] = pp + H_; src[dl[l].two] = pp + 2 * H_; src[dl[l].tWp] = pp + 3 * H_;
      }
      dw_src = (long long*)alloc<float>(src.size() * 2);
      if (dw_ws && dw_flag && dw_src) HIPC(hipMemcpy(dw_src, src.data(), src.size() * sizeof(long long), hipMemcpyHostToDevice));
      else dw_ws = nullptr;
    }
  }
  if (gp_live && !g_dnn() && !g_bnl()) {
    GPersistArgs ga{};
    gp_Tcap = std::min(Tmax, (int)GP_TMAX);
    gp_noproj = !gl.empty() && !gl[0].has_proj;
    if (gp_noproj) {
      bool fits = false;
      for (int nt : {2, 4}) {
        gp_np_nt = nt;
        if (gpersist_shape(ga, gp_Tcap) && resident_probe(gpersist_grid(ga), GP_THREADS, gpersist_np_lds_bytes())) { fits = true; break; }
      }
      if (!fits) gp_np_nt = 0;
      if (fits) {
        gp_gran2_bytes = gpersist_np_gran2_bytes(ga);
        gp_gran2 = (unsigned long long*)alloc<float>(gp_gran2_bytes / sizeof(float));
        gp_ctl = (unsigned*)alloc<float>(16);
        if (gp_np_nt == 2 && (gp_live & 2) && switches().gp_np_bwd) {
          gp_gran1 = (unsigned long long*)alloc<float>(gpersist_np_gran1_bytes(ga) / sizeof(float));
          gp_gran3 = (unsigned long long*)alloc<float>(gpersist_np_gran3_bytes(ga) / sizeof(float));
          if (!gp_gran1 || !gp_gran3) { gp_gran1 = gp_gran3 = nullptr; }
        }
        if (!gp_gran1) gp_gran1 = gp_gran2;
        if (gp_gran2 && gp_ctl) {
          HIPC(ctl_reset(gp_ctl));
          gpersist_rearm();
        } else { gp_gran1 = gp_gran2 = gp_gran3 = nullptr; gp_ctl = nullptr; }
      }
    } else if (gpersist_args(ga, gp_Tcap) && resident_probe(gpersist_grid(ga), GP_THREADS, gpersist_lds_bytes())) {
      gp_gran1 = (unsigned long long*)alloc<float>(gpersist_gran1_bytes(ga) / sizeof(float));
      gp_gran2_bytes = gpersist_gran2_bytes(ga);
      gp_gran2 = (unsigned long long*)alloc<float>(gp_gran2_bytes / sizeof(float));
      gp_ctl = (unsigned*)alloc<float>(16);
      bool bwd_ok = (gp_live & 2) != 0;
      for (auto& L : gl) bwd_ok = bwd_ok && L.P > 16;
      if (bwd_ok) gp_gran3 = (unsigned long long*)alloc<float>(gpersist_gran3_bytes(ga) / sizeof(float));
      if (gp_gran1 && gp_gran2 && gp_ctl) {
        HIPC(ctl_reset(gp_ctl));
        gpersist_rearm();
      } else { gp_gran1 = gp_gran2 = nullptr; gp_ctl = nullptr; }
    }
  }
  {
    GPersistArgs ga{};
    if (sw.trail && dp_gran && (dp_live & 2) && gp_gran1 && gp_gran3 && !gp_noproj && (gp_live & 2) && B % 32 == 0 && gpersist_args(ga, gp_Tcap))
      trail_fits = resident_probe(gpersist_grid(ga) + ((dpersist_trail_grid((int)dl.size(), B) + 7) & ~7), GP_THREADS,
                                  std::max(gpersist_lds_bytes(), dpersist_trail_lds_bytes()));
  }
  {
    lazy_sw = switches().lazy_swizzle && wavefront() && gp_gran1 && gp_gran3 && (gp_live & 3) == 3 && dp_gran && (dp_live & 3) == 3;
  }
  drop_ctr = (unsigned long long*)alloc<float>(4);
  HIPC(hipMemset(drop_ctr, 0, 16));
  const int dmaxld = std::max(ldPd, ldDout);
  d_dA = alloc<float>(TB2 * dmaxld); d_dB = alloc<float>(TB2 * dmaxld);
  len_dev = alloc<int>(2 * B);
  zeros = alloc<float>(64);
  noise_r_buf = alloc<float>((size_t)B * Dout); noise_f_buf = alloc<float>((size_t)B * Dout);
  if (hipStreamCreateWithFlags(&main_s, hipStreamNonBlocking) != hipSuccess) main_s = nullptr;
  if (main_s && (hipEventCreateWithFlags(&ev_in, hipEventDisableTiming) != hipSuccess ||
                 hipEventCreateWithFlags(&ev_out, hipEventDisableTiming) != hipSuccess)) { (void)hipStreamDestroy(main_s); main_s = nullptr; }
  dyn = alloc<float>(DYN_COUNT); adam_t_dev = alloc<int>(1);
  losses = alloc<float>(8); tmp3 = alloc<float>(4);
  size_t maxcols = 7 * (size_t)std::max(c.g_cells, c.d_cells);
  maxcols = std::max(maxcols, (size_t)Din + 4);
  maxcols = std::max(maxcols, (size_t)std::max(ldP, ldDin));
  scratch_floats = std::max<size_t>(4 * 64 * maxcols, 16384);
  scratch = alloc<float>(scratch_floats);
  scratch2 = alloc<float>(std::max<size_t>(4 * 64 * maxcols, 1024));
  g_fc_out_wT = g_dnn() ? nullptr : alloc<float>((size_t)Dout * ldP);
  if (hipStreamCreateWithFlags(&side, hipStreamNonBlocking) != hipSuccess) side = nullptr;
  if (hipEventCreateWithFlags(&ev_last, hipEventDisableTiming) != hipSuccess) ev_last = nullptr;
  {
    if (sw.dpipe > 0 && trail_fits && side && !d_dnn() && dp_max_grid >= dpersist_grid((int)dl.size(), B)) {
      const size_t gb = dpersist_granule_bytes((int)dl.size(), B, Tmax) / 2;
      dp_gran2 = (unsigned long long*)alloc<float>(gb / sizeof(float));
      dp_ctl2 = (unsigned*)alloc<float>(16);
      if (dp_gran2 && dp_ctl2 && hipEventCreateWithFlags(&ev_dfree, hipEventDisableTiming) == hipSuccess &&
          hipEventCreateWithFlags(&ev_real, hipEventDisableTiming) == hipSuccess) {
        HIPC(ctl_reset(dp_ctl2));
        dpipe = true;
      }
    }
  }
  if (side) {
    for (auto& e : ev_pool)
      if (hipEventCreateWithFlags(&e, hipEventDisableTiming) != hipSuccess) { side = nullptr; break; }
  }
  gemm_ws_floats = (size_t)32 << 20;
  gemm_ws = alloc<float>(gemm_ws_floats);
  if (!gemm_ws) gemm_ws_floats = 0;
  bwdb_ws_floats = (size_t)8 << 20;
  bwdb_ws = alloc<float>(bwdb_ws_floats);
  gemm_ws2 = alloc<float>(gemm_ws_floats ? gemm_ws_floats : 1);
  if (switches().dk_pad && !gl.empty() && gl[0].has_proj && gl[0].I % 4 != 0 && gl[0].ldI % 4 == 0 && gl.size() <= (size_t)GEMM_MAXB) {
    dk_tmp_per = (size_t)(gl[0].ldI + gl[0].P) * 4 * gl[0].H;
    dk_tmp = alloc<float>(dk_tmp_per * gl.size());
    if (!dk_tmp) dk_tmp_per = 0;
  }
  if (!gemm_ws2) side = nullptr;
  if (!side) dpipe = false;
  if (!scratch || !d_dB || !g_dB || !xd) { set_error("hipMalloc failed (activations)"); return RSRGAN_ERR_HIP; }

  std::mt19937_64 rng(seed);
  for (ParamSet* ps : {&G, &D}) {
    std::vector<float> host((size_t)ps->padded, 0.f);
    if (ps == &G && g_bnl()) bnl_init(host, seed);
    else for (auto& t : ps->t) {
      if (!t.l2) {
        if (t.bias_init != 0.f)
          for (int cc = 0; cc < t.cols; ++cc) host[(size_t)t.off + cc] = t.bias_init;
        continue;
      }
      const double fan_in = t.is_vector ? t.cols : t.rows, fan_out = t.xavier_fan_out > 0 ? t.xavier_fan_out : t.cols;
      const double lim = std::sqrt(6.0 / (fan_in + fan_out));
      std::uniform_real_distribution<double> u(-lim, lim);
      for (int r = 0; r < t.rows; ++r)
        for (int cc = 0; cc < t.cols; ++cc) host[(size_t)t.off + (size_t)r * t.ld + cc] = (float)u(rng);
    }
    HIPC(hipMemcpy(ps->w, host.data(), host.size() * sizeof(float), hipMemcpyHostToDevice));
    if (ps->ema) HIPC(hipMemcpy(ps->ema, host.data(), host.size() * sizeof(float), hipMemcpyHostToDevice));
  }
  scal[RSRGAN_G_LEARNING_RATE] = 8e-5; scal[RSRGAN_D_LEARNING_RATE] = 1e-3; scal[RSRGAN_MSE_LAMBDA] = 10.0;
  scal[RSRGAN_D_REAL] = 1.0; scal[RSRGAN_D_FAKE] = 0.0; scal[RSRGAN_L2_SCALE] = c.l2_scale;
  scal[RSRGAN_CLIP_NORM] = c.clip_norm; scal[RSRGAN_ADAM_STEP] = 0;
  float hdyn[DYN_COUNT] = {0};
  hdyn[DYN_G_LR] = 8e-5f; hdyn[DYN_D_LR] = 1e-3f; hdyn[DYN_LAMBDA] = 10.f; hdyn[DYN_D_REAL] = 1.f; hdyn[DYN_D_FAKE] = 0.f;
  hdyn[DYN_L2] = c.l2_scale; hdyn[DYN_CLIP] = c.clip_norm; hdyn[DYN_B1] = c.adam_beta1; hdyn[DYN_B2] = c.adam_beta2;
  hdyn[DYN_EPS] = c.adam_eps; hdyn[DYN_EMA] = c.ema_decay;
  HIPC(hipMemcpy(dyn, hdyn, sizeof(hdyn), hipMemcpyHostToDevice));
  refresh_transposes(RSRGAN_NET_G, nullptr);
  refresh_transposes(RSRGAN_NET_D, nullptr);
  { int rc = build_buckets(); if (rc) return rc; }
  HIPC(hipDeviceSynchronize());
  HIPC(hipGetLastError());
  return RSRGAN_OK;
}

void Model::destroy() {
  drop_graphs();
  if (main_s) {
    (void)hipStreamSynchronize(main_s);
    if (ev_in) (void)hipEventDestroy(ev_in);
    if (ev_out) (void)hipEventDestroy(ev_out);
    (void)hipStreamDestroy(main_s);
    main_s = nullptr;
  }
  if (side) {
    (void)hipStreamSynchronize(side);
    for (auto& e : ev_pool) if (e) (void)hipEventDestroy(e);
    (void)hipStreamDestroy(side);
    side = nullptr;
  }
  if (ev_last) { (void)hipEventDestroy(ev_last); ev_last = nullptr; ev_last_set = false; }
  if (ev_dfree) { (void)hipEventDestroy(ev_dfree); ev_dfree = nullptr; }
  if (ev_real) { (void)hipEventDestroy(ev_real); ev_real = nullptr; }
  dpipe = false;
  for (auto& v : gbk) { for (auto& b : v) if (b.ev) (void)hipEventDestroy(b.ev); v.clear(); }
  for (auto& e : prof_ev) if (e) (void)hipEventDestroy(e);
  prof_ev.clear();
  for (auto& e : prof_gp_ev) if (e) (void)hipEventDestroy(e);
  prof_gp_ev.clear();
  for (auto& e : prof_gb_ev) if (e) (void)hipEventDestroy(e);
  prof_gb_ev.clear();
  for (void* p : allocs) (void)hipFree(p);
  allocs.clear();
}

int Model::build_buckets() {
  auto range = [](const ParamSet& ps, int lo, int hi, GradBucket& b) {
    b.off = ps.t[lo].off;
    b.count = (hi + 1 < (int)ps.t.size() ? ps.t[hi + 1].off : ps.padded) - b.off;
  };
  auto whole = [](const ParamSet& ps, std::vector<GradBucket>& v) { GradBucket b; b.off = 0; b.count = ps.padded; v.assign(1, b); };
  whole(D, gbk[RSRGAN_NET_D]);
  whole(G, gbk[RSRGAN_NET_G]);
  if (!g_dnn() && wavefront()) {
    std::vector<GradBucket> v;
    bool ok = true;
    GradBucket b;
    range(G, g_fc_out_w, g_fc_out_b, b); ok = ok && g_fc_out_b == g_fc_out_w + 1; v.push_back(b);
    if (cfg.g_type == RSRGAN_G_LSTM) { range(G, g_fc_in_w, g_fc_in_b, b); ok = ok && g_fc_in_b == g_fc_in_w + 1; v.push_back(b); }
    for (auto& L : gl) {
      const int lo = L.tK, hi = L.has_proj ? L.tWp : L.two;
      ok = ok && L.tb > lo && L.tb < hi && L.twf > lo && L.twi > lo && L.two <= hi && hi - lo == (L.has_proj ? 5 : 4);
      range(G, lo, hi, b); v.push_back(b);
    }
    int64_t covered = 0;
    for (auto& x : v) covered += x.count;
    if (ok && covered == G.padded) gbk[RSRGAN_NET_G] = v;
  }
  for (auto& v : gbk)
    for (auto& b : v)
      if (hipEventCreateWithFlags(&b.ev, hipEventDisableTiming) != hipSuccess) { set_error("hipEventCreate failed"); return RSRGAN_ERR_HIP; }
  return RSRGAN_OK;
}
void Model::mark_bucket(int net, int i, hipStream_t s) {
  GradBucket& b = gbk[net][i];
  (void)hipEventRecord(b.ev, s);
  b.marked = true;
}
void Model::finish_buckets(int net, hipStream_t s) {
  for (auto& b : gbk[net]) {
    if (!b.marked) (void)hipEventRecord(b.ev, s);
    b.marked = false;
  }
}

void Model::refresh_transposes(int net, hipStream_t s) {
  const ParamSet& ps = net == RSRGAN_NET_G ? G : D;
  auto& layers = net == RSRGAN_NET_G ? gl : dl;
  TransposeList tl{};
  auto add = [&](const float* src, int lds_, float* dst, int ldd, int R, int C) {
    if (tl.n == 16) { launch_transpose_many(tl, s); tl.n = 0; }
    tl.j[tl.n++] = TransposeJob{src, dst, lds_, ldd, R, C, 0};
  };
// ... 835 lines not shown
      for (int l = Lc - 1; l >= 0; --l) {
        const int t = T - 1 - (d - off - (Lc - 1 - l));
        if (t < 0 || t >= T) continue;
        if (aj.n == MAXJ) flush_a();
        BwdAJob& a = aj.j[aj.n++]; fill_bwd_a(a, ch[l], t); ab += bwd_a_blocks(ch[l].L->H, ch[l].N);
        ak = std::max(ak, kb16(ch[l].L->ldP));
      }
    }
    flush_a();
    for (size_t c = 0; c < chains.size(); ++c) {
      Chain& ch = chains[c];
      const int Lc = (int)ch.size(), off = offsets ? (*offsets)[c] : 0;
      for (int l = Lc - 1; l >= 0; --l) {
        const int t = T - 1 - (d - off - (Lc - 1 - l));
        if (t < 0 || t >= T) continue;
        const LayerRun& R = ch[l];
        if (bj.n == MAXJ) flush_b();
        BwdBJob& b = bj.j[bj.n++]; fill_bwd_b(b, R, t, R.din != nullptr); bb += job_blocks(b.nblk_c, R.N);
        bk = std::max(bk, kb16(4 * R.L->H));
      }
    }
    if (fcs)
      for (auto& F : *fcs) {
        const int t = T - 1 - (d - F.offset);
        if (t < 0 || t >= T) continue;
        if (bj.n == MAXJ) flush_b();
        BwdBJob& b = bj.j[bj.n++]; fill_fc_bwd(b, F, t); bb += job_blocks(b.nblk_c, F.N);
        bk = std::max(bk, kb16(F.ld_in));
      }
    flush_b();
    if (ovl) {
      for (size_t c = 0; c < chains.size(); ++c) {
        Chain& ch = chains[c];
        if (!ch[0].want_wgrads) continue;
        const int off = offsets ? (*offsets)[c] : 0, Lc = (int)ch.size();
        while (chunk_done[c] < nchunk && d >= (T - 1 - chunk_lo(chunk_done[c])) + off + Lc - 1) {
          const int cc = chunk_done[c]++;
          hipEvent_t ev = ev_pool[ev_next++ & 15];
          (void)hipEventRecord(ev, s);
          (void)hipStreamWaitEvent(side, ev, 0);
          for (auto& R : ch)
            if (R.want_wgrads) layer_wgrads_gemms(R, chunk_lo(cc), chunk_hi(cc), cc > 0, side);
        }
      }
    }
  }
  if (ovl) {
    for (auto& ch : chains)
      for (auto& R : ch)
        if (R.want_wgrads) layer_wgrads_colsums(R, T, side, scratch2);
    hipEvent_t ev = ev_pool[ev_next++ & 15];
    (void)hipEventRecord(ev, side);
    (void)hipStreamWaitEvent(s, ev, 0);
  } else if (!defer_wgrads) {
    for (auto& ch : chains)
      for (auto& R : ch)
        if (R.want_wgrads) layer_wgrads(R, T, s);
  }
}

int Model::prepare_batch(const float* x, const float* labels, const int32_t* lengths, int T, hipStream_t s, const float** nr,
                         const float** nf, hipStream_t early) {
  if (T <= 0 || T > Tmax) { set_error("T=%d outside (0, max_frames=%d]", T, Tmax); return RSRGAN_ERR_INVALID; }
  if (!x || (!lengths && !g_dnn())) { set_error("null input pointer"); return RSRGAN_ERR_INVALID; }
  StageJobs j{}; j.B = B; j.T = T; j.Bt = Bt;
  j.pack[0] = StagePack{x, x_tm, Din, ldDin};
  if (labels) j.pack[1] = StagePack{labels, lab_tm, Dout, ldDout};
  if (lengths) { j.copy[0] = StageCopy{lengths, len_dev, Bt}; j.copy[1] = StageCopy{lengths, len_dev + B, Bt}; }
  if (nr && *nr) { j.copy[2] = StageCopy{*nr, noise_r_buf, Bt * Dout}; *nr = noise_r_buf; }
  if (nf && *nf) { j.copy[3] = StageCopy{*nf, noise_f_buf, Bt * Dout}; *nf = noise_f_buf; }
  if (early) {
    StageJobs e{}; e.B = B; e.T = T; e.Bt = Bt;
    e.pack[1] = j.pack[1]; e.copy[0] = j.copy[0]; e.copy[1] = j.copy[1]; e.copy[2] = j.copy[2];
    j.pack[1] = StagePack{}; j.copy[0] = StageCopy{}; j.copy[1] = StageCopy{}; j.copy[2] = StageCopy{};
    (void)hipStreamWaitEvent(early, ev_dfree, 0);
    launch_stage_inputs(e, early);
  }
  launch_stage_inputs(j, s);
  cur_T = T;
  g_fwd_valid = false;
  return RSRGAN_OK;
}

Chain Model::g_chain(int T) {
  (void)T;
  Chain ch;
  const bool res = cfg.g_type == RSRGAN_G_RES_LSTM_L;
  for (size_t l = 0; l < gl.size(); ++l) {
    LayerRun R;
    R.ps = &G; R.L = &gl[l]; R.S = &g_st[l]; R.in = g_ins[l];
    R.N = B; R.Ns = B; R.row0 = 0; R.len = len_dev;
    R.zx_batched = (l == 0);
    R.carry = g_carry;
    if (res) { R.res_in = g_ins[l]; R.res_out = g_res[l]; }
    if (g_resi()) { R.res_in = g_ins[0]; R.res_out = g_res[l]; }
    if (seq_drop_on()) R.drop = DropSpec{drop_ctr, drop_seed, (1ull << 40) | ((unsigned long long)l << 20), drop_thr(), keep_prob};
    ch.push_back(R);
  }
  return ch;
}

Chain Model::d_chain(int N, int Ns, int row0) {
  Chain ch;
  for (size_t l = 0; l < dl.size(); ++l) {
    LayerRun R;
    R.ps = &D; R.L = &dl[l]; R.S = &d_st[l]; R.in = l == 0 ? xd : d_st[l - 1].out;
    R.N = N; R.Ns = Ns; R.row0 = row0; R.len = len_dev + row0;
    R.zx_batched = false;
    ch.push_back(R);
  }
  return ch;
}

void Model::gstate_xfer(int dir, int T, int rows, const int* mask, hipStream_t s) {
  GStateArgs a{};
  a.nl = (int)gl.size(); a.SF = g_state_sf; a.rows = rows; a.dir = dir; a.state = g_state; a.slot = (size_t)T * B; a.mask = mask;
  int off = 0;
  for (size_t l = 0; l < gl.size(); ++l) {
    a.L[l] = GStateLayer{g_st[l].c, g_st[l].mst, gl[l].H, gl[l].P, gl[l].ldP, off};
    off += gl[l].H + gl[l].P;
  }
  launch_gstate(a, s);
}

void Model::g_forward_head(int T, hipStream_t s) {
  if (cfg.g_type == RSRGAN_G_LSTM) {
    const int P = gR, ldP = pad4(P);
    gemm(x_tm, ldDin, true, G.W(g_fc_in_w), ldP, false, g_h0, ldP, T * B, P, Din, G.W(g_fc_in_b), 1, cfg.lrelu_alpha, false, s);
  }
}
void Model::g_forward_tail(int T, hipStream_t s) {
  const int P = gR, ldP = pad4(P);
  gemm(g_ins[gl.size()], ldP, true, G.W(g_fc_out_w), ldDout, false, y_tm, ldDout, T * B, Dout, P, G.W(g_fc_out_b), 0, 0.f, false, s);
  g_fwd_valid = true;
}
void Model::g_forward(int T, hipStream_t s, Chain* extra) {
  if (g_dnn()) { bn_eval_call = false; g_frame_forward(T * B, s); g_fwd_valid = true; return; }
  if (g_bnl()) { bnl_forward(T, false, s); return; }
  g_forward_head(T, s);
  if (!extra && persist_forward_g(T, s)) { g_forward_tail(T, s); return; }
  std::vector<Chain> chains;
  chains.push_back(g_chain(T));
  if (extra) chains.push_back(*extra);
  rnn_forward(chains, T, s);
  g_forward_tail(T, s);
}

void Model::d_logits(int N, int T, hipStream_t s) {
  const int ldPd = pad4(dR);
  gemm(d_st[dl.size() - 1].out, ldPd, true, D.W(d_fc_w), 4, false, logits, 4, T * N, 1, dR, D.W(d_fc_b), 0, 0.f, false, s);
}

bool Model::d_head(int N, int T, int n_real, const float* t_real, const float* t_fake, float* loss3, bool want_grads, bool want_wgrads,
                   hipStream_t s) {
  const int ldPd = pad4(dR), nb = (T * N + 63) / 64;
  if (!switches().dhead || d_dnn() || dl.empty() || dR % 4 != 0 || dR + 3 > 64 ||
      (size_t)nb * (DH_MAXR + 3) > scratch_floats) return false;
  DHeadArgs a{};
  a.top = d_st[dl.size() - 1].out; a.ldt = ldPd; a.w = D.W(d_fc_w); a.ldw = 4; a.b = D.W(d_fc_b);
  a.logits = logits; a.ldl = 4; a.dlogits = dlogits; a.dout = d_dB; a.ldo = ldPd; a.gw = D.Gd(d_fc_w); a.gb = D.Gd(d_fc_b);
  a.T = T; a.Nd = N; a.n_real = n_real; a.dR = dR; a.t_real = t_real; a.t_fake = t_fake; a.loss3 = loss3; a.part = scratch;
  a.want_grads = want_grads ? 1 : 0; a.want_wgrads = want_wgrads ? 1 : 0;
  a.Bp = pad_Bp(); a.Bt = Bt;
  launch_dhead(a, s);
  return true;
}

void Model::d_backward_pass(int N, int T, bool want_wgrads, bool need_dx0, const float* dlog, hipStream_t s, bool head_done) {
  const int R = T * N;
  const int ldPd = pad4(dR);
  const size_t Ld = dl.size();
  const float* top = d_st[Ld - 1].out;
  if (want_wgrads && !head_done) {
    gemm(top, ldPd, false, dlog, 4, false, D.Gd(d_fc_w), 4, dR, 1, R, nullptr, 0, 0.f, false, s);
    launch_colsum(dlog, 4, nullptr, 0, D.Gd(d_fc_b), R, 1, scratch, s);
  }
  float* cur = d_dB;
  float* other = d_dA;
  if (!head_done) gemm(dlog, 4, true, D.W(d_fc_w), 4, true, cur, ldPd, R, dR, 1, nullptr, 0, 0.f, false, s);
  std::vector<Chain> chains(1, d_chain(N, N, 0));
  Chain& ch = chains[0];
  for (int l = (int)Ld - 1; l >= 0; --l) {
    ch[l].dout = cur;
    ch[l].din = (l > 0 || need_dx0) ? other : nullptr;
    ch[l].din_accumulate = false;
    ch[l].want_wgrads = want_wgrads;
    std::swap(cur, other);
  }
  if (!persist_backward(ch, T, s)) rnn_backward(chains, T, s);
  last_dx0 = cur;
}

void Model::g_backward_pass(int T, float* dy, hipStream_t s) {
  const int R = T * B;
  const int P = gR, ldP = pad4(P);
  const size_t Lg = gl.size();
  gemm(g_ins[Lg], ldP, false, dy, ldDout, false, G.Gd(g_fc_out_w), ldDout, P, Dout, R, nullptr, 0, 0.f, false, s);
  launch_colsum(dy, ldDout, nullptr, 0, G.Gd(g_fc_out_b), R, Dout, scratch, s);
  float* cur = g_dA;
  float* other = g_dB;
  gemm(dy, ldDout, true, G.W(g_fc_out_w), ldDout, true, cur, ldP, R, P, Dout, nullptr, 0, 0.f, false, s);
  std::vector<Chain> chains(1, g_chain(T));
  Chain& ch = chains[0];
  for (auto& r : ch) r.want_wgrads = true;
  if (cfg.g_type == RSRGAN_G_LSTM) {
    for (int l = (int)Lg - 1; l >= 0; --l) {
      ch[l].dout = cur; ch[l].din = other; ch[l].din_accumulate = false;
      std::swap(cur, other);
    }
    if (!persist_backward_g(ch, T, s)) rnn_backward(chains, T, s);
    launch_lrelu_bwd(g_h0, cur, (size_t)R, P, ldP, cfg.lrelu_alpha, s);
    gemm(x_tm, ldDin, false, cur, ldP, false, G.Gd(g_fc_in_w), ldP, Din, P, R, nullptr, 0, 0.f, false, s);
    launch_colsum(cur, ldP, nullptr, 0, G.Gd(g_fc_in_b), R, P, scratch, s);
  } else if (cfg.g_type == RSRGAN_G_RES_LSTM_L) {
    for (int l = (int)Lg - 1; l >= 0; --l) {
      ch[l].dout = cur; ch[l].din = l > 0 ? cur : nullptr; ch[l].din_accumulate = true;
    }
    if (!persist_backward_g(ch, T, s)) rnn_backward(chains, T, s);
  } else {
    for (int l = (int)Lg - 1; l >= 0; --l) {
      ch[l].dout = cur; ch[l].din = l > 0 ? other : nullptr; ch[l].din_accumulate = false;
      std::swap(cur, other);
    }
    if (!persist_backward_g(ch, T, s)) rnn_backward(chains, T, s);
  }
}

int Model::d_backward(const float* x, const float* labels, const int32_t* lengths, int T, const float* nr, const float* nf,
                      float* out_losses, bool want_grads, hipStream_t s) {
  if (!labels) { set_error("labels required"); return RSRGAN_ERR_INVALID; }
  if (supervised()) { set_error("RSRGAN_FLAG_SUPERVISED: the trainer graph has no discriminator step"); return RSRGAN_ERR_STATE; }
  if (g_dnn()) return dnn_d_backward(x, labels, T, out_losses, want_grads, s);
  if (d_dnn()) { nr = nullptr; nf = nullptr; }
  bn_eval_call = !want_grads;
  dfree_current = false;
  bool dsplit = false;
  if (dpipe && (!nr || sw.dpipe >= 2) && wavefront() && gp_fwd_on() && !d_dnn() && !seq_drop_on() && T > 0 && T <= Tmax) {
    Chain dchk = d_chain(B, 2 * B, B);
    dsplit = persist_forward_real(T, side, true) && persist_forward_g_trail(dchk, T, s, nf, true);
  }
  int rc = prepare_batch(x, labels, lengths, T, s, &nr, &nf, dsplit ? side : nullptr);
  if (rc) return rc;
  if (dsplit) {
    launch_add_noise_rows(lab_tm, nr, xd, B, T, Dout, ldDout, 2 * B, 0, side);
    (void)persist_forward_real(T, side);
    (void)hipEventRecord(ev_real, side);
    (void)hipStreamWaitEvent(s, ev_real, 0);
  }
  if (seq_drop_on()) launch_drop_tick(drop_ctr, s);
  const bool inl = fused_apply && switches().fused_seg && want_grads && !d_dnn() && graphs_on();
  const unsigned kbits = (want_grads ? 1u : 0u) | (nr ? 2u : 0u) | (nf ? 4u : 0u) | (inl ? 8u : 0u) | (dsplit ? 16u : 0u);
  run_seg(seg_key(SEG_D, T, kbits), s, [&]() {
  if (!dsplit) launch_add_noise_rows(lab_tm, nr, xd, B, T, Dout, ldDout, 2 * B, 0, s);
  bool g_done = false;
  if (dsplit) {
    g_forward_head(T, s);
    Chain dch = d_chain(B, 2 * B, B);
    g_done = persist_forward_g_trail(dch, T, s, nf);
  }
  if (!g_done && wavefront() && gp_fwd_on()) {
    g_forward_head(T, s);
    g_done = persist_forward_g(T, s);
    if (g_done) {
      g_forward_tail(T, s);
      launch_add_noise_rows(y_tm, nf, xd, B, T, Dout, ldDout, 2 * B, B, s);
      if (!d_dnn()) {
        std::vector<Chain> chains(1, d_chain(2 * B, 2 * B, 0));
        if (!persist_forward(chains[0], T, s)) rnn_forward(chains, T, s);
      }
    }
  }
  if (g_done) {
  } else if (wavefront()) {
    if (!gp_fwd_on()) g_forward_head(T, s);
    const int Lg = (int)gl.size(), ldP = pad4(gR);
    std::vector<Chain> chains{g_chain(T)};
    std::vector<int> offs{0};
    if (!d_dnn()) {
      chains.push_back(d_chain(B, 2 * B, 0)); offs.push_back(0);
      chains.push_back(d_chain(B, 2 * B, B)); offs.push_back(Lg + 1);
    }
    FcStage F;
    F.offset = Lg; F.N = B; F.K = gR; F.D = Dout;
    F.in = g_ins[Lg]; F.ld_in = ldP; F.WT = g_fc_out_wT; F.bias = G.W(g_fc_out_b); F.noise = nf;
    F.y = y_tm; F.ldy = ldDout; F.out2 = xd; F.ld2 = ldDout; F.Ns2 = 2 * B; F.row02 = B;
    std::vector<FcStage> fcs{F};
    rnn_forward(chains, T, s, &offs, &fcs);
  } else {
    g_forward(T, s);
    launch_add_noise_rows(y_tm, nf, xd, B, T, Dout, ldDout, 2 * B, B, s);
    if (!d_dnn()) {
      std::vector<Chain> chains(1, d_chain(2 * B, 2 * B, 0));
      rnn_forward(chains, T, s);
    }
  }
  if (d_dnn()) {
    d_dnn_forward_loss(T, 2 * B, B, want_grads, losses, s);
    if (want_grads) fc_backward(D, dfc, d_act, T * 2 * B, dlogits, true, false, s);
  } else {
    const bool head = d_head(2 * B, T, B, dyn + DYN_D_REAL, dyn + DYN_D_FAKE, losses, want_grads, want_grads, s);
    if (!head) {
      d_logits(2 * B, T, s);
      launch_lsgan(logits, 4, want_grads ? dlogits : nullptr, T, 2 * B, B, dyn + DYN_D_REAL, dyn + DYN_D_FAKE, losses, s, false, 0.f, 0.f, pad_Bp(), Bt);
    }
    if (want_grads) d_backward_pass(2 * B, T, true, false, dlogits, s, head);
  }
  if (inl) apply_body(RSRGAN_NET_D, s);
  });
  d_partial_fresh = false;
  g_fwd_valid = true;
  if (inl) apply_inlined |= 2;
  if (want_grads) { finish_buckets(RSRGAN_NET_D, s); d_grads_ready = true; }
  if (out_losses) launch_copy_f(losses, out_losses, 3, s);
  HIPC(hipGetLastError());
  return RSRGAN_OK;
}

int Model::g_backward(const float* x, const float* labels, const int32_t* lengths, int T, const float* nf,
                      float* out_losses, bool want_grads, bool reuse, hipStream_t s) {
  if (!labels) { set_error("labels required"); return RSRGAN_ERR_INVALID; }
  if (g_dnn()) return dnn_g_backward(x, labels, T, out_losses, want_grads, reuse, s);
  if (g_bnl()) return bnl_step(x, labels, lengths, T, out_losses, want_grads, s);
  bn_eval_call = !want_grads;
  dfree_current = false;
  if (seq_drop_on()) { reuse = false; launch_drop_tick(drop_ctr, s); }
  if (supervised()) {
    int rc = prepare_batch(x, labels, lengths, T, s);
    if (rc) return rc;
    g_forward(T, s);
    const bool l2s = !cfg.cross_validation && scal[RSRGAN_L2_SCALE] > 0.0;
    HIPC(hipMemsetAsync(losses + 3, 0, sizeof(float), s));
    if (want_grads) {
      float* dy = g_dC;
      launch_mse(y_tm, lab_tm, ldDout, dy, T * B, Dout, dyn + DYN_LAMBDA, false, losses + 4, scratch, s, pad_Bp(), Bt);
      g_backward_pass(T, dy, s);
      if (l2s) {
        launch_l2(G.w, G.g, G.ct, dyn + DYN_L2, G.partial, s);
        launch_l2_total(G.partial, G.ct.n_chunks, dyn + DYN_L2, losses + 5, s);
      }
      { finish_buckets(RSRGAN_NET_G, s); g_grads_ready = true; }
    } else {
      launch_mse(y_tm, lab_tm, ldDout, nullptr, T * B, Dout, dyn + DYN_LAMBDA, false, losses + 4, scratch, s, pad_Bp(), Bt);
    }
    if (!(want_grads && l2s)) HIPC(hipMemsetAsync(losses + 5, 0, sizeof(float), s));
    launch_g_total(losses + 3, dyn + DYN_LAMBDA, s);
    if (out_losses) launch_copy_f(losses + 3, out_losses, 4, s);
    HIPC(hipGetLastError());
    return RSRGAN_OK;
  }
  if (d_dnn()) nf = nullptr;
  if (reuse) {
    if (!g_fwd_valid || T != cur_T) { set_error("reuse_g_forward without a valid generator forward"); return RSRGAN_ERR_STATE; }
  } else {
    int rc = prepare_batch(x, labels, lengths, T, s);
    if (rc) return rc;
  }
  nf = stage_noise(nf, noise_f_buf, s);
  const bool l2_on = !cfg.cross_validation && scal[RSRGAN_L2_SCALE] > 0.0;
  const bool wave_bwd = want_grads && !d_dnn() && wavefront();
  const bool fused_seg = switches().fused_seg;
  const bool bucketed = wave_bwd && gbk[RSRGAN_NET_G].size() > 1 && !overlap() && !(fused_apply && fused_seg);
  const int R = T * B, Ld = (int)dl.size(), Lg = (int)gl.size();
  const int ldPd = pad4(dR), P = gR, ldP = pad4(P);
  float* dy = g_dB;
  float* bufA = g_dA; float* bufB = g_dC;
  std::vector<Chain> bw_chains;
  auto build_bw_chains = [&]() {
    Chain dch = d_chain(B, B, 0);
    float* cur = d_dB; float* other = d_dA;
    for (int l = Ld - 1; l >= 0; --l) {
      dch[l].dout = cur; dch[l].want_wgrads = false;
      if (l == 0) { dch[l].din = dy; dch[l].din_accumulate = true; }
      else { dch[l].din = other; dch[l].din_accumulate = false; std::swap(cur, other); }
    }
    Chain gch = g_chain(T);
    bufA = g_dA; bufB = g_dC;
    for (int l = Lg - 1; l >= 0; --l) {
      gch[l].want_wgrads = true;
      if (cfg.g_type == RSRGAN_G_RES_LSTM_L) {
        gch[l].dout = g_dA; gch[l].din = l > 0 ? g_dA : nullptr; gch[l].din_accumulate = true;
      } else {
        const bool need = cfg.g_type == RSRGAN_G_LSTM || l > 0;
        gch[l].dout = bufA; gch[l].din = need ? bufB : nullptr; gch[l].din_accumulate = false;
        std::swap(bufA, bufB);
      }
    }
    bw_chains = std::vector<Chain>{dch, gch};
  };
  if (wave_bwd) build_bw_chains();
  const bool fc_side_env = switches().wgrad_streams >= 2 && switches().fc_side;
  const bool fcs_inside = wave_bwd && !bucketed && side && fc_side_env && cfg.g_type == RSRGAN_G_LSTM && dl[0].ldI == ldDout &&
                          persist_backward_g(bw_chains[1], T, s, true);
  const bool inl = fused_apply && fused_seg && wave_bwd && !bucketed && graphs_on() && !(cfg.g_type == RSRGAN_G_LSTM && !fcs_inside);
  const unsigned kbits = (want_grads ? 1u : 0u) | (nf ? 2u : 0u) | (reuse ? 4u : 0u) | (l2_on ? 8u : 0u) | (bucketed ? 16u : 0u) | (inl ? 32u : 0u);
  auto tail_body = [&]() {
    if (want_grads && l2_on) {
      launch_l2(G.w, G.g, G.ct, dyn + DYN_L2, G.partial, s);
      launch_l2_total(G.partial, G.ct.n_chunks, dyn + DYN_L2, losses + 5, s);
    } else {
      (void)hipMemsetAsync(losses + 5, 0, sizeof(float), s);
    }
    launch_g_total(losses + 3, dyn + DYN_LAMBDA, s);
  };

  bool trail_plan = false;
  if (wave_bwd && want_grads && !d_dnn() && dl[0].ldI == ldDout && persist_backward_g(bw_chains[1], T, s, true)) {
    Chain dc0 = bw_chains[0];
    dc0[0].din = nullptr;
    trail_plan = persist_backward_trail(dc0, T, s, dy, ldDout, g_dA, ldP, true);
  }
  const bool gsplit = dpipe && trail_plan;
  auto bwd_rest = [&]() {
    const int ldP_ = pad4(gR);
    StreamFn pre, post;
    if (fcs_inside) {
      pre = [&](hipStream_t q) {
        gemm(g_ins[Lg], ldP_, false, dy, ldDout, false, G.Gd(g_fc_out_w), ldDout, gR, Dout, R, nullptr, 0, 0.f, false, q);
        launch_colsum(dy, ldDout, nullptr, 0, G.Gd(g_fc_out_b), R, Dout, (side && q == side) ? scratch2 : scratch, q);
      };
      post = [&](hipStream_t q) {
        launch_lrelu_bwd(g_h0, bufA, (size_t)R, gR, ldP_, cfg.lrelu_alpha, q);
        gemm(x_tm, ldDin, false, bufA, ldP_, false, G.Gd(g_fc_in_w), ldP_, Din, gR, R, nullptr, 0, 0.f, false, q);
        launch_colsum(bufA, ldP_, nullptr, 0, G.Gd(g_fc_in_b), R, gR, (side && q == side) ? scratch2 : scratch, q);
      };
    }
    const int saved_w = g_gemm_workers;
    g_gemm_workers = std::min(saved_w, switches().dpipe_w);
    defer_wgrads = bucketed;
    gp_phase = 2; persist_backward_g(bw_chains[1], T, s, false, pre, post); gp_phase = 0;
    defer_wgrads = false;
    if (!fcs_inside) {
      gemm(g_ins[Lg], ldP_, false, dy, ldDout, false, G.Gd(g_fc_out_w), ldDout, gR, Dout, R, nullptr, 0, 0.f, false, s);
      launch_colsum(dy, ldDout, nullptr, 0, G.Gd(g_fc_out_b), R, Dout, scratch, s);
    }
    g_gemm_workers = saved_w;
    if (inl) { tail_body(); apply_body(RSRGAN_NET_G, s); }
  };
  run_seg(seg_key(SEG_G_MAIN, T, kbits | (trail_plan ? 64u : 0u) | (gsplit ? 128u : 0u)), s, [&]() {
  if (trail_plan) gpersist_arm_bytes(g_dA, (size_t)T * B * ldP * sizeof(float), s);
  bool g_done = false;
  if (!reuse && !wavefront()) g_forward(T, s);
  bool d_trailed = false;
  if (!reuse && wavefront() && gp_fwd_on()) {
    g_forward_head(T, s);
    if (!d_dnn()) {
      Chain dch = d_chain(B, B, 0);
      g_done = d_trailed = persist_forward_g_trail(dch, T, s, nf);
    }
    if (!g_done) {
      g_done = persist_forward_g(T, s);
      if (g_done) g_forward_tail(T, s);
    }
  }
  if (d_trailed) {
  } else if (!reuse && wavefront() && !g_done) {
    if (!gp_fwd_on()) g_forward_head(T, s);
    std::vector<Chain> chains{g_chain(T)};
    std::vector<int> offs{0};
    if (!d_dnn()) { chains.push_back(d_chain(B, B, 0)); offs.push_back(Lg + 1); }
    FcStage F;
    F.offset = Lg; F.N = B; F.K = gR; F.D = Dout;
    F.in = g_ins[Lg]; F.ld_in = pad4(gR); F.WT = g_fc_out_wT; F.bias = G.W(g_fc_out_b); F.noise = nf;
    F.y = y_tm; F.ldy = ldDout; F.out2 = xd; F.ld2 = ldDout; F.Ns2 = B; F.row02 = 0;
    std::vector<FcStage> fcs{F};
    rnn_forward(chains, T, s, &offs, &fcs);
  } else {
    const bool direct = !nf && !d_dnn() && dl[0].ldI == ldDout;
    if (!direct) launch_add_noise_rows(y_tm, nf, xd, B, T, Dout, ldDout, B, 0, s);
    if (!d_dnn()) {
      std::vector<Chain> chains(1, d_chain(B, B, 0));
      if (direct) chains[0][0].in = y_tm;
      if (!persist_forward(chains[0], T, s) && !fold_forward(chains[0], T, s)) rnn_forward(chains, T, s);
    }
  }
  bool g_head = false;
  if (d_dnn()) {
    d_dnn_forward_loss(T, B, 0, want_grads, tmp3, s);
  } else {
    g_head = d_head(B, T, 0, dyn + DYN_D_REAL, dyn + DYN_D_REAL, tmp3, want_grads, false, s);
    if (!g_head) {
      d_logits(B, T, s);
      launch_lsgan(logits, 4, want_grads ? dlogits : nullptr, T, B, 0, dyn + DYN_D_REAL, dyn + DYN_D_REAL, tmp3, s, false, 0.f, 0.f, pad_Bp(), Bt);
    }
  }
  launch_copy_f(tmp3 + 1, losses + 3, 1, s);
  if (want_grads && d_dnn()) {
    float* dyd = fc_backward(D, dfc, d_act, T * B, dlogits, false, true, s);
    launch_mse(y_tm, lab_tm, ldDout, dyd, T * B, Dout, dyn + DYN_LAMBDA, true, losses + 4, scratch, s, pad_Bp(), Bt);
    g_backward_pass(T, dyd, s);
  } else if (wave_bwd) {
    if (!g_head) gemm(dlogits, 4, true, D.W(d_fc_w), 4, true, d_dB, ldPd, R, dR, 1, nullptr, 0, 0.f, false, s);
    launch_mse(y_tm, lab_tm, ldDout, dy, R, Dout, dyn + DYN_LAMBDA, false, losses + 4, scratch, s, pad_Bp(), Bt);
    FcStage F;
    F.offset = Ld; F.N = B; F.K = Dout; F.D = P;
    F.in = dy; F.ld_in = ldDout; F.WT = G.W(g_fc_out_w); F.y = g_dA; F.ldy = ldP; F.accumulate = false;
    std::vector<int> offs{0, Ld + 1};
    std::vector<FcStage> fcs{F};
    defer_wgrads = bucketed;
    if (dl[0].ldI == ldDout && persist_backward_g(bw_chains[1], T, s, true)) {
      std::vector<Chain> dc1(1, bw_chains[0]);
      dc1[0][0].din = nullptr;
      const bool trailed = trail_plan && persist_backward_trail(dc1[0], T, s, dy, ldDout, g_dA, ldP);
      if (!trailed) {
        if (!persist_backward(dc1[0], T, s)) rnn_backward(dc1, T, s);
        const int H4d = 4 * dl[0].H;
        gemm(d_st[0].gates, H4d, true, D.W(dl[0].tK), H4d, true, dy, ldDout, R, dl[0].I, H4d, nullptr, 0, 0.f, true, s);
        gemm(dy, ldDout, true, G.W(g_fc_out_w), ldDout, true, g_dA, ldP, R, P, Dout, nullptr, 0, 0.f, false, s);
      }
      gp_trail_next = trailed;
      StreamFn pre, post;
      if (fcs_inside) {
        pre = [&](hipStream_t q) {
          gemm(g_ins[Lg], ldP, false, dy, ldDout, false, G.Gd(g_fc_out_w), ldDout, P, Dout, R, nullptr, 0, 0.f, false, q);
          launch_colsum(dy, ldDout, nullptr, 0, G.Gd(g_fc_out_b), R, Dout, (side && q == side) ? scratch2 : scratch, q);
        };
        post = [&](hipStream_t q) {
          launch_lrelu_bwd(g_h0, bufA, (size_t)R, P, ldP, cfg.lrelu_alpha, q);
          gemm(x_tm, ldDin, false, bufA, ldP, false, G.Gd(g_fc_in_w), ldP, Din, P, R, nullptr, 0, 0.f, false, q);
          launch_colsum(bufA, ldP, nullptr, 0, G.Gd(g_fc_in_b), R, P, (side && q == side) ? scratch2 : scratch, q);
        };
      }
      if (gsplit) {
        gp_phase = 1; persist_backward_g(bw_chains[1], T, s, false, pre, post); gp_phase = 0;
        gp_trail_next = false;
        return;
      }
      persist_backward_g(bw_chains[1], T, s, false, pre, post);
      gp_trail_next = false;
    } else {
      rnn_backward(bw_chains, T, s, &offs, &fcs);
    }
    defer_wgrads = false;
    if (!fcs_inside) {
      gemm(g_ins[Lg], ldP, false, dy, ldDout, false, G.Gd(g_fc_out_w), ldDout, P, Dout, R, nullptr, 0, 0.f, false, s);
      launch_colsum(dy, ldDout, nullptr, 0, G.Gd(g_fc_out_b), R, Dout, scratch, s);
    }
  } else if (want_grads) {
    d_backward_pass(B, T, false, true, dlogits, s, g_head);
    float* dyd = last_dx0;
    launch_mse(y_tm, lab_tm, ldDout, dyd, T * B, Dout, dyn + DYN_LAMBDA, true, losses + 4, scratch, s, pad_Bp(), Bt);
    g_backward_pass(T, dyd, s);
  } else {
    launch_mse(y_tm, lab_tm, ldDout, nullptr, T * B, Dout, dyn + DYN_LAMBDA, false, losses + 4, scratch, s, pad_Bp(), Bt);
  }
  if (inl) { tail_body(); apply_body(RSRGAN_NET_G, s); }
  });
  if (gsplit) {
    defer_wgrads = false;
    (void)hipEventRecord(ev_dfree, s);
    dfree_inside = true; dfree_current = true;
    run_seg(seg_key(SEG_G_MAIN, T, kbits | 64u | 256u), s, bwd_rest);
  }
  if (inl) apply_inlined |= 1;
  if (!reuse) g_fwd_valid = true;
  if (wave_bwd) {
    int bi = 0;
    if (bucketed) mark_bucket(RSRGAN_NET_G, bi++, s);
    if (cfg.g_type == RSRGAN_G_LSTM && !fcs_inside) {
      run_seg(seg_key(SEG_G_FCIN, T, kbits), s, [&]() {
        launch_lrelu_bwd(g_h0, bufA, (size_t)R, P, ldP, cfg.lrelu_alpha, s);
        gemm(x_tm, ldDin, false, bufA, ldP, false, G.Gd(g_fc_in_w), ldP, Din, P, R, nullptr, 0, 0.f, false, s);
        launch_colsum(bufA, ldP, nullptr, 0, G.Gd(g_fc_in_b), R, P, scratch, s);
      });
      if (bucketed) mark_bucket(RSRGAN_NET_G, bi++, s);
    }
    if (bucketed) {
      bool dkd = false;
      const bool gb = batch_wgrads(bw_chains[1], T, s, false, &dkd, true);
      if (gb) run_seg(seg_key(SEG_G_BATCH, T, kbits), s, [&]() { bool d_ = false; (void)batch_wgrads(bw_chains[1], T, s, false, &d_); });
      int li = 0;
      for (auto& Rr : bw_chains[1]) {
        run_seg(seg_key(SEG_G_LAYER0 + li, T, kbits), s, [&]() { if (gb) layer_wgrads_gemms(Rr, 0, T, false, s, true, false); else layer_wgrads(Rr, T, s); });
        mark_bucket(RSRGAN_NET_G, bi++, s);
        ++li;
      }
    }
  }
  if (!inl) run_seg(seg_key(SEG_G_TAIL, T, kbits), s, tail_body);
  if (want_grads) {
    if (l2_on) for (auto& bk : gbk[RSRGAN_NET_G]) bk.marked = false;
    finish_buckets(RSRGAN_NET_G, s);
    g_grads_ready = true;
  }
  if (out_losses) launch_copy_f(losses + 3, out_losses, 4, s);
  HIPC(hipGetLastError());
  return RSRGAN_OK;
}

int Model::bnl_step(const float* x, const float* labels, const int32_t* lengths, int T, float* out_losses, bool want_grads, hipStream_t s) {
  if (want_grads && cfg.cross_validation) {
    set_error("g_type bnlstm: gradients of the cross_validation model (moving-statistics batch norm) are not built");
    return RSRGAN_ERR_INVALID;
  }
  int rc = prepare_batch(x, labels, lengths, T, s);
  if (rc) return rc;
  const bool l2s = want_grads && scal[RSRGAN_L2_SCALE] > 0.0;
  run_seg(seg_key(SEG_BNL, T, (want_grads ? 1u : 0u) | (l2s ? 2u : 0u)), s, [&]() {
    bnl_forward(T, want_grads, s);
    (void)hipMemsetAsync(losses + 3, 0, sizeof(float), s);
    float* dy = want_grads ? g_dC : nullptr;
    launch_mse(y_tm, lab_tm, ldDout, dy, T * B, Dout, dyn + DYN_LAMBDA, false, losses + 4, scratch, s, pad_Bp(), Bt);
    if (want_grads) bnl_backward(T, dy, s);
    if (l2s) {
      launch_l2(G.w, G.g, G.ct, dyn + DYN_L2, G.partial, s);
      launch_l2_total(G.partial, G.ct.n_chunks, dyn + DYN_L2, losses + 5, s);
    } else {
      (void)hipMemsetAsync(losses + 5, 0, sizeof(float), s);
    }
    launch_g_total(losses + 3, dyn + DYN_LAMBDA, s);
  });
  if (want_grads) { finish_buckets(RSRGAN_NET_G, s); g_grads_ready = true; }
  g_fwd_valid = false;
  if (out_losses) launch_copy_f(losses + 3, out_losses, 4, s);
  HIPC(hipGetLastError());
  return RSRGAN_OK;
}

void Model::apply_body(int net, hipStream_t s) {
  if (net == RSRGAN_NET_D) {
    if (!d_partial_fresh) launch_sumsq(D.g, D.ct, D.partial, s);
    d_partial_fresh = false;
    if (d_adam()) {
      launch_adam_tick(dyn, adam_t_dev_d, (double)cfg.adam_beta1, (double)cfg.adam_beta2, s, DYN_D_LR, DYN_ADAM_LRT_D);
      launch_apply_adam(D.w, D.g, D.m, D.v, D.ema, D.ct, D.partial, dyn, s, DYN_ADAM_LRT_D);
    } else {
      launch_apply_sgd(D.w, D.g, D.ema, D.ct, D.partial, dyn, s);
    }
    refresh_transposes(RSRGAN_NET_D, s);
  } else {
    launch_sumsq(G.g, G.ct, G.partial, s);
    launch_adam_tick(dyn, adam_t_dev, (double)cfg.adam_beta1, (double)cfg.adam_beta2, s);
    launch_apply_adam(G.w, G.g, G.m, G.v, G.ema, G.ct, G.partial, dyn, s);
    refresh_transposes(RSRGAN_NET_G, s);
  }
}

int Model::apply(int net, hipStream_t s) {
  if (net == RSRGAN_NET_D) {
    if (!d_grads_ready) { set_error("apply(D) without gradients"); return RSRGAN_ERR_STATE; }
    if (!(apply_inlined & 2)) run_seg(seg_key(SEG_APPLY_D, 0, 0), s, [&]() { apply_body(RSRGAN_NET_D, s); });
    apply_inlined &= ~2;
    if (d_adam()) scal[RSRGAN_ADAM_STEP_D] += 1;
    d_grads_ready = false;
  } else if (net == RSRGAN_NET_G) {
    if (!g_grads_ready) { set_error("apply(G) without gradients"); return RSRGAN_ERR_STATE; }
    if (!(apply_inlined & 1)) run_seg(seg_key(SEG_APPLY_G, 0, 0), s, [&]() { apply_body(RSRGAN_NET_G, s); });
    if (dfree_current) dfree_inside = true;
    apply_inlined &= ~1;
    scal[RSRGAN_ADAM_STEP] += 1;
    g_grads_ready = false;
    g_fwd_valid = false;
  } else {
    set_error("bad net %d", net);
    return RSRGAN_ERR_INVALID;
  }
  HIPC(hipGetLastError());
  return RSRGAN_OK;
}

}
```

rsrgan_amd/csrc/model.h:

```cpp
#pragma once
#include <hip/hip_runtime.h>
#include <stdint.h>
#include <string>
#include <unordered_map>
#include <functional>
#include <vector>

#include "../../include/rsrgan.h"
#include "kernels.h"

namespace rsr {

inline int pad4(int x) { return (x + 3) & ~3; }

struct TensorDesc {
  std::string name;
  int rows, cols, ld;
  int64_t off;
  int64_t dense_off;
  bool l2;
  bool trainable = true;
  bool is_vector;
  int xavier_fan_out = 0;
  float bias_init = 0.f;
// ... 88 lines not shown
  float *mm_in, *mv_in, *mm_s, *mv_s, *mm_c, *mv_c;
  float *xh_in, *yin, *xh_s, *act, *cnew, *chat, *ccar, *h, *mst, *out;
  float *mu, *var;
  const float* dout;
  float *dz, *dhh, *dyc, *dmn, *dcc, *dmc;
};
struct BnlCell {
  int tWx, tWh, tin[4], tst[4], tb, twf, twi, two, tce[4], tWp;
  float *zx = nullptr, *xh_in = nullptr, *yin = nullptr, *xh_s = nullptr, *act = nullptr, *cnew = nullptr, *chat = nullptr;
  float *ccar = nullptr, *h = nullptr, *mst = nullptr, *out = nullptr, *mu = nullptr, *var = nullptr;
  float *dz = nullptr, *dyc = nullptr, *dmn = nullptr, *dcc = nullptr, *dmc = nullptr;
};
bool bnl_supported(int B);
void launch_bnl_bn_in(const BnlLayer& a, const float* zx, int T, hipStream_t s);
void launch_bnl_cell_fwd(const BnlLayer& a, int t, hipStream_t s);
void launch_bnl_proj(const BnlLayer& a, int t, hipStream_t s);
void launch_bnl_ema(const BnlLayer& a, int T, float decay, hipStream_t s);
void launch_bnl_cell_bwd(const BnlLayer& a, int t, hipStream_t s);
void launch_bnl_dm(const BnlLayer& a, int t, hipStream_t s);
void launch_bnl_bn_in_bwd(const BnlLayer& a, float* dzx, int T, hipStream_t s);

struct Model {
  rsrgan_cfg cfg{};
  const HandleSwitches sw;
  int B = 0, Tmax = 0, Din = 0, Dout = 0, ldDin = 0, ldDout = 0;
  int Bt = 0;
  int pad_Bp() const { return Bt != B ? B : 0; }
  int gR = 0, dR = 0;
  ParamSet G, D;
  std::vector<LstmLayer> gl, dl;
  int g_fc_in_w = -1, g_fc_in_b = -1, g_fc_out_w = -1, g_fc_out_b = -1, d_fc_w = -1, d_fc_b = -1;

  float *x_tm = nullptr, *lab_tm = nullptr, *g_h0 = nullptr, *y_tm = nullptr;
  std::vector<float*> g_ins;
  std::vector<float*> g_res;
  std::vector<LstmStash> g_st;
  float *g_dA = nullptr, *g_dB = nullptr, *g_dC = nullptr;
  float *xd = nullptr, *logits = nullptr, *dlogits = nullptr;
  std::vector<LstmStash> d_st;
  float *d_dA = nullptr, *d_dB = nullptr, *last_dx0 = nullptr;
  int *len_dev = nullptr;
  float *zeros = nullptr;
  std::vector<LstmLayer> dl_fold;
  std::vector<float*> dl_fold_K;
  std::vector<LstmStash> d_fold_st;
  bool fold_forward(Chain& ch, int T, hipStream_t s);
  void refresh_fold(hipStream_t s);
  unsigned long long* dp_gran = nullptr;
  unsigned* dp_ctl = nullptr;
  size_t dp_gran_bytes = 0;
  int dp_live = sw.dpersist;
  bool persist_forward(Chain& ch, int T, hipStream_t s);
  bool persist_backward(Chain& ch, int T, hipStream_t s);
  bool persist_backward_trail(Chain& ch, int T, hipStream_t s, float* dy, int ld_dy, float* dtop, int ld_dtop, bool check_only = false);
  bool persist_forward_g_trail(Chain& ch, int T, hipStream_t s, const float* nf, bool check_only = false);
  bool dpipe = false;
  bool dfree_inside = false;
  bool dfree_current = false;
  int gp_phase = 0;
  hipEvent_t ev_dfree = nullptr, ev_real = nullptr;
  unsigned long long* dp_gran2 = nullptr;
  unsigned* dp_ctl2 = nullptr;
  bool persist_forward_real(int T, hipStream_t q, bool check_only = false);
  bool trail_fits = false;
  bool gp_trail_next = false;
  DPersistArgs dt_args{};
  unsigned long long *gp_gran1 = nullptr, *gp_gran2 = nullptr, *gp_gran3 = nullptr;
  unsigned* gp_ctl = nullptr;
  size_t gp_gran2_bytes = 0;
  int gp_live = sw.gpersist;
  int gp_Tcap = 0;
  float* dw_ws = nullptr; unsigned* dw_flag = nullptr; long long* dw_src = nullptr; size_t dw_stride = 0;
  bool d_partial_fresh = false;
  int dp_max_grid = 0;
  void persist_disable(int which);
  bool gp_fwd_on() const { return gp_gran1 && (gp_live & 1); }
  bool gpersist_shape(GPersistArgs& a, int T) const;
  int gp_np_nt = 0;
  bool gp_noproj = false;
  bool gpersist_args(GPersistArgs& a, int T) const;
  void gpersist_rearm();
  bool persist_forward_g(int T, hipStream_t s);
  float* g_state = nullptr;
  int g_state_sf = 0;
  bool g_carry = false;
  void gstate_xfer(int dir, int T, int rows, const int* mask, hipStream_t s);
  typedef std::function<void(hipStream_t)> StreamFn;
  bool persist_backward_g(Chain& ch, int T, hipStream_t s, bool check_only = false, const StreamFn& pre = nullptr, const StreamFn& post = nullptr);
  std::vector<FcLayer> gfc, dfc;
  std::vector<float*> g_act, d_act;
  float *fc_dA = nullptr, *fc_dB = nullptr, *joint = nullptr, *dy_buf = nullptr;
  int ldJ = 0;
  int *adam_t_dev_d = nullptr;
  bool g_dnn() const { return cfg.g_type == RSRGAN_G_DNN || cfg.g_type == RSRGAN_G_RCED; }
  bool g_rced() const { return cfg.g_type == RSRGAN_G_RCED; }
  bool g_resi() const { return cfg.g_type == RSRGAN_G_RES_LSTM_I; }
  std::vector<BnlCell> bnl;
  bool g_bnl() const { return cfg.g_type == RSRGAN_G_BNLSTM; }
  int bnl_check(const rsrgan_cfg& c) const;
  void bnl_params();
  int bnl_alloc();
  void bnl_init(std::vector<float>& host, uint64_t seed) const;
  BnlLayer bnl_args(int l, bool train) const;
  void bnl_forward(int T, bool train, hipStream_t s);
  void bnl_backward(int T, float* dy, hipStream_t s);
  int bnl_step(const float* x, const float* labels, const int32_t* lengths, int T, float* out_losses, bool want_grads, hipStream_t s);
  std::vector<ConvLayer> gconv;
  FcLayer rc_fc{};
  std::vector<float*> rc_act;
  float *rc_col = nullptr, *rc_dcol = nullptr, *rc_dA = nullptr, *rc_dB = nullptr;
  std::vector<float*> rc_cols;
  std::vector<float*> rc_ft_fwd, rc_ft_bwd;
  std::vector<char> rc_wgrad_implicit;
  float* rc_wg_ws = nullptr;
  float* rc_x4 = nullptr;
  bool rc_keep_cols = false;
  size_t scratch_floats = 0;
  int rcS = 0, rcW = 0;
  void g_frame_forward(int rows, hipStream_t s);
  void g_frame_backward(int rows, float* dy, hipStream_t s);
  void rced_forward(int rows, hipStream_t s);
  void rced_backward(int rows, float* dy, hipStream_t s);
  bool d_dnn() const { return cfg.d_type == RSRGAN_D_DNN; }
  bool d_adam() const { return g_dnn(); }
  void fc_forward(const ParamSet& ps, const std::vector<FcLayer>& L, const std::vector<float*>& act, int rows, hipStream_t s, int calls = 1,
                  int call0 = 0);
  float keep_prob = 1.f;
  uint64_t drop_seed = 0, drop_run = 0;
  bool drop_training() const {
    return g_dnn() && keep_prob < 1.f && !cfg.cross_validation && !bn_eval_call && scal[RSRGAN_L2_SCALE] > 0.0;
  }
  uint64_t drop_key(int net, int layer, int call) const;
  unsigned long long* drop_ctr = nullptr;
  bool seq_drop_on() const { return !g_dnn() && keep_prob < 1.f && !cfg.cross_validation && !bn_eval_call; }
  unsigned drop_thr() const { return (unsigned)((double)keep_prob * 16777216.0); }
  float* fc_backward(const ParamSet& ps, const std::vector<FcLayer>& L, const std::vector<float*>& act, int rows, float* dtop,
                     bool want_wgrads, bool want_din, hipStream_t s, int calls = 1, int row0 = 0, int call0 = 0);
  bool bn_on() const { return (cfg.flags & RSRGAN_FLAG_BATCH_NORM) != 0; }
  bool bn_eval_call = false;
  bool bn_training() const { return bn_on() && !cfg.cross_validation && !bn_eval_call; }
  BnVars bn_vars(const ParamSet& ps, const FcLayer& F) const;
  BnVars bn_vars(const ParamSet& ps, const int (&tbn)[8]) const;
  void bn_commit_stack(const ParamSet& ps, const std::vector<FcLayer>& L, int times0, int times1, BnCommitList& cl);
  float* bn_sums = nullptr;
  void d_dnn_forward_loss(int T, int Nd, int n_real, bool want_grads, float* loss3, hipStream_t s, int calls = 1, int call0 = 0);
  void bn_commit_run(bool with_d, hipStream_t s);
  int dnn_d_backward(const float* x, const float* labels, int T, float* out_losses, bool want_grads, hipStream_t s);
  int dnn_g_backward(const float* x, const float* labels, int T, float* out_losses, bool want_grads, bool reuse, hipStream_t s);

  float *dyn = nullptr;
  int *adam_t_dev = nullptr;
  float *losses = nullptr;
  float *tmp3 = nullptr;
  float *scratch = nullptr;
  double scal[RSRGAN_SCALAR_COUNT_] = {0};
  bool g_fwd_valid = false;
  int cur_T = 0;
  bool d_grads_ready = false, g_grads_ready = false;
  std::vector<void*> allocs;

  int init(const rsrgan_cfg& c, uint64_t seed);
  void destroy();

  int prepare_batch(const float* x, const float* labels, const int32_t* lengths, int T, hipStream_t s, const float** nr = nullptr,
                    const float** nf = nullptr, hipStream_t early = nullptr);
  void g_forward(int T, hipStream_t s, Chain* extra = nullptr);
  void g_forward_head(int T, hipStream_t s);
  void g_forward_tail(int T, hipStream_t s);
  void d_logits(int N, int T, hipStream_t s);
  void d_backward_pass(int N, int T, bool want_wgrads, bool need_dx0, const float* dlog, hipStream_t s, bool head_done = false);
  bool d_head(int N, int T, int n_real, const float* t_real, const float* t_fake, float* loss3, bool want_grads, bool want_wgrads, hipStream_t s);
  void g_backward_pass(int T, float* dy, hipStream_t s);
  int d_backward(const float* x, const float* labels, const int32_t* lengths, int T, const float* nr, const float* nf,
                 float* out_losses, bool want_grads, hipStream_t s);
  int g_backward(const float* x, const float* labels, const int32_t* lengths, int T, const float* nf,
                 float* out_losses, bool want_grads, bool reuse, hipStream_t s);
  int apply(int net, hipStream_t s);
  void apply_body(int net, hipStream_t s);
  int apply_inlined = 0;
  void refresh_transposes(int net, hipStream_t s);
  void refresh_swizzles(int net, hipStream_t s);
  bool lazy_sw = false;

  void rnn_forward(std::vector<Chain>& chains, int T, hipStream_t s, const std::vector<int>* offsets = nullptr,
                   const std::vector<FcStage>* fcs = nullptr);
  void rnn_backward(std::vector<Chain>& chains, int T, hipStream_t s, const std::vector<int>* offsets = nullptr,
                    const std::vector<FcStage>* fcs = nullptr);
  void layer_wgrads(const LayerRun& R, int T, hipStream_t s);
  void chain_wgrads(Chain& ch, int T, hipStream_t s, const StreamFn& between, const StreamFn& pre = nullptr, const StreamFn& post = nullptr);
  void layer_wgrads_gemms(const LayerRun& R, int t0, int t1, bool accumulate, hipStream_t s, bool do_dK = true, bool do_dWp = true);
  int trail_nrt() const;
  bool batch_wgrads(Chain& ch, int T, hipStream_t s, bool dK_too, bool* dK_done, bool check_only = false);
  void layer_wgrads_colsums(const LayerRun& R, int T, hipStream_t s, float* scr);
  hipStream_t side = nullptr;
  struct GradBucket { int64_t off = 0, count = 0; hipEvent_t ev = nullptr; bool marked = false; };
  std::vector<GradBucket> gbk[2];
  bool fused_apply = false;
  bool defer_wgrads = false;
  int build_buckets();
  void mark_bucket(int net, int i, hipStream_t s);
  void finish_buckets(int net, hipStream_t s);
  bool prof_on = false;
  std::vector<hipEvent_t> prof_ev;
  int prof_n = 0;
  double prof_flops = 0.0;
  std::vector<hipEvent_t> prof_gp_ev;
  int prof_gp_n = 0;
  double prof_gp_flops = 0.0;
  std::vector<hipEvent_t> prof_gb_ev;
  int prof_gb_n = 0;
  int prof_fdt_n = 0;
  int prof_cnt[9] = {};
  double prof_gb_flops = 0.0;
  void gates_launch(const FwdGateJobs& gj, int blocks, int kb, hipStream_t s);
  int gates_blocks(int H, int N) const;
  int proj_blocks(int P, int N) const;
  int bwd_a_blocks(int H, int N) const;
  void run_bwd_b_splitk(BwdBJobs& bj, hipStream_t s);
  hipEvent_t ev_pool[16] = {};
  int ev_next = 0;
  float* gemm_ws2 = nullptr;
  float* dk_tmp = nullptr;
  size_t dk_tmp_per = 0;
  float* scratch2 = nullptr;
  bool overlap() const { return side != nullptr && (cfg.flags & RSRGAN_FLAG_OVERLAP) != 0; }
  Chain g_chain(int T);
  Chain d_chain(int N, int Ns, int row0);
  void gemm(const float* A, int lda, bool a_kc, const float* B, int ldb, bool b_kc, float* C, int ldc, int M, int N,
            int K, const float* bias, int act, float alpha, bool accumulate, hipStream_t s);
  bool supervised() const { return (cfg.flags & RSRGAN_FLAG_SUPERVISED) != 0; }
  bool wavefront() const { return (cfg.flags & RSRGAN_FLAG_WAVEFRONT) != 0; }
  float* g_fc_out_wT = nullptr;
  float* bwdb_ws = nullptr;
  size_t bwdb_ws_floats = 0;
  bool bwd_b_splitk_ok(const BwdBJobs& jobs) const;
  float* gemm_ws = nullptr;
  size_t gemm_ws_floats = 0;

  struct GraphSlot { int uses = 0; hipGraphExec_t exec = nullptr; };
  std::unordered_map<uint64_t, GraphSlot> graphs;
  hipStream_t main_s = nullptr;
  hipEvent_t ev_in = nullptr, ev_out = nullptr;
  hipEvent_t ev_last = nullptr; bool ev_last_set = false;
  float *noise_r_buf = nullptr, *noise_f_buf = nullptr;
  bool graphs_on() const { return (cfg.flags & RSRGAN_FLAG_GRAPH) != 0 && wavefront() && !overlap() && !prof_on && !g_dnn() && sw.graphs; }
  template <class F> void run_seg(uint64_t key, hipStream_t s, F&& body);
  void drop_graphs();
  hipStream_t enter(hipStream_t caller);
  void leave(hipStream_t caller, hipStream_t work);
  const float* stage_noise(const float* src, float* buf, hipStream_t s);

  template <typename T> T* alloc(size_t n);
};

void set_error(const char* fmt, ...);
const char* get_error();

}
```

rsrgan_amd/engine_hip.py:

```python
from __future__ import annotations

import contextlib
import ctypes as C
import os
from typing import List, Optional, Tuple

import numpy as np
import torch

from . import _lib
from ._lib import NET_D, NET_G, RsrganCfg, SCALARS, WHAT, check


def _ptr(t: Optional[torch.Tensor]):
    return None if t is None else C.c_void_p(t.data_ptr())


class _RawDeviceBuffer:

    def __init__(self, ptr: int, count: int):
        self.__cuda_array_interface__ = {"shape": (count,), "typestr": "<f4", "data": (ptr, False),
                                         "version": 2, "strides": None}


# ... 259 lines not shown

    def g_state_floats(self) -> int:
        n = C.c_int32()
        check(self.lib.rsrgan_g_state_floats(self.h, C.byref(n)))
        return n.value

    def g_state_reset(self, rows=None):
        mask = None
        if rows is not None:
            m = np.zeros(self.batch_size, dtype=np.int32)
            for r in rows:
                if not 0 <= int(r) < self.batch_size:
                    raise ValueError("row %d outside [0, batch_size=%d)" % (int(r), self.batch_size))
                m[int(r)] = 1
            mask = self._i32(m)
        check(self.lib.rsrgan_g_state_reset(self.h, _ptr(mask), self._stream()))
        self._keep_mask = mask

    def g_state_get(self) -> torch.Tensor:
        out = torch.empty(self.batch_size, self.g_state_floats(), dtype=torch.float32, device=self.device)
        check(self.lib.rsrgan_g_state_get(self.h, _ptr(out), self._stream()))
        return out

    def g_state_set(self, t):
        t = self._f32(t, (self.batch_size, self.g_state_floats()))
        check(self.lib.rsrgan_g_state_set(self.h, _ptr(t), self._stream()))
        self._keep_state = t

    def forward_g_stream(self, x, lengths) -> torch.Tensor:
        x = self._f32(x)
        if lengths is None:
            raise ValueError("forward_g_stream needs lengths")
        ln = self._i32(lengths)
        T = self._check_batch(x, None, ln)
        y = torch.empty(self.batch_size, T, self.output_dim, dtype=torch.float32, device=self.device)
        check(self.lib.rsrgan_forward_g_stream(self.h, _ptr(x), _ptr(ln), T, _ptr(y), self._stream()))
        self._keep3 = (x, ln)
        return y

    def d_backward(self, x, lab, lengths, noise_real=None, noise_fake=None, train=True, apply=False) -> torch.Tensor:
        if os.environ.get("RSRGAN_DPIPE", "0") not in ("", "0"):
            lab = self.upload_ready(lab)
            lengths = self.upload_ready(lengths, int32=True) if lengths is not None else None
        x, lab = self._f32(x), self._f32(lab)
        ln = self._i32(lengths) if lengths is not None else None
        nr, nf = self._noise(noise_real), self._noise(noise_fake)
        out = torch.empty(3, dtype=torch.float32, device=self.device)
        T = self._check_batch(x, lab, ln)
        if apply or not train:
            check(self.lib.rsrgan_d_step(self.h, _ptr(x), _ptr(lab), _ptr(ln), T, _ptr(nr), _ptr(nf), _ptr(out),
                                         1 if train else 0, self._stream()))
        else:
            check(self.lib.rsrgan_d_backward(self.h, _ptr(x), _ptr(lab), _ptr(ln), T, _ptr(nr), _ptr(nf), _ptr(out),
                                             self._stream()))
        self._keep = (x, lab, ln, nr, nf)
        return out

    def g_backward(self, x, lab, lengths, noise_fake=None, train=True, reuse=False, apply=False) -> torch.Tensor:
        x, lab = self._f32(x), self._f32(lab)
        ln = self._i32(lengths) if lengths is not None else None
        nf = self._noise(noise_fake)
        out = torch.empty(4, dtype=torch.float32, device=self.device)
        T = self._check_batch(x, lab, ln)
        if apply or not train:
            check(self.lib.rsrgan_g_step(self.h, _ptr(x), _ptr(lab), _ptr(ln), T, _ptr(nf), _ptr(out),
                                         1 if train else 0, 1 if reuse else 0, self._stream()))
        else:
            check(self.lib.rsrgan_g_backward(self.h, _ptr(x), _ptr(lab), _ptr(ln), T, _ptr(nf), _ptr(out),
                                             1 if reuse else 0, self._stream()))
        self._keep2 = (x, lab, ln, nf)
        return out

    def apply(self, net: int):
        check(self.lib.rsrgan_apply(self.h, net, self._stream()))

    def profile_begin(self):
        check(self.lib.rsrgan_profile_begin(self.h))

    def profile_read_kind(self, kind):
        n, us, fl = C.c_int32(), C.c_double(), C.c_double()
        check(self.lib.rsrgan_profile_read_kind(self.h, kind, C.byref(n), C.byref(us), C.byref(fl)))
        return n.value, us.value, fl.value

    def profile_read(self):
        n, us, fl = C.c_int32(), C.c_double(), C.c_double()
        check(self.lib.rsrgan_profile_read(self.h, C.byref(n), C.byref(us), C.byref(fl)))
        return n.value, us.value, fl.value

    def device_status(self):
        code = C.c_int32()
        check(self.lib.rsrgan_device_status(self.h, C.byref(code)))
        return code.value

    def set_dropout(self, keep_prob, seed=0):
        check(self.lib.rsrgan_set_dropout(self.h, float(keep_prob), int(seed) & 0xFFFFFFFFFFFFFFFF))

    def profile_launches(self):
        n = C.c_int64()
        check(self.lib.rsrgan_profile_launches(self.h, C.byref(n)))
        return n.value

    def launch_floor(self, n=400, mode=1):
        us = C.c_double()
        check(self.lib.rsrgan_op_launch_floor(n, mode, C.byref(us), self._stream()))
        return us.value

    def op_gemm(self, A, a_kc, B, b_kc, C_, M, N, K, bias=None, act=0, alpha=0.3, accumulate=False):
        check(self.lib.rsrgan_op_gemm(_ptr(A), A.stride(0), 1 if a_kc else 0, _ptr(B), B.stride(0), 1 if b_kc else 0,
                                      _ptr(C_), C_.stride(0), M, N, K, _ptr(bias), act, alpha, 1 if accumulate else 0,
                                      self._stream()))

    def op_gemm2(self, A, a_kc, B, b_kc, C_, M, N, K, A2=None, M1=0, lda=None, lda2=None, bias=None, act=0, alpha=0.3,
                 accumulate=False, row_map=None, workers=0, force_cfg=-1):
        rp, outer, inner = row_map if row_map else (0, 0, 0)
        check(self.lib.rsrgan_op_gemm2(_ptr(A), A.stride(0) if lda is None else lda, 1 if a_kc else 0, _ptr(A2),
                                       0 if A2 is None else (A2.stride(0) if lda2 is None else lda2), M1, _ptr(B), B.stride(0),
                                       1 if b_kc else 0, _ptr(C_), C_.stride(0), M, N, K, _ptr(bias), act, alpha,
                                       1 if accumulate else 0, rp, outer, inner, workers, force_cfg, self._stream()))

    @staticmethod
    def _table(ts):
        from ._lib import ptr_table
        return None if ts is None else ptr_table([None if t is None else t.data_ptr() for t in ts])

    def op_gemm_batch(self, As, A2s, Bs, Cs, M, N, K, M1=0, accumulate=False, workers=0) -> bool:
        rc = self.lib.rsrgan_op_gemm_batch(len(As), self._table(As), As[0].stride(0), self._table(A2s),
                                           A2s[0].stride(0) if A2s else 0, M1, self._table(Bs), Bs[0].stride(0), self._table(Cs),
                                           Cs[0].stride(0), M, N, K, 1 if accumulate else 0, workers, self._stream())
        if rc == 1:
            return False
        check(rc)
        return True

    def op_gemm16_batch(self, As, A2s, Bs, Cs, M, N, K, M1=0, accumulate=False):
        check(self.lib.rsrgan_op_gemm16_batch(len(As), self._table(As), As[0].stride(0), self._table(A2s),
                                              A2s[0].stride(0) if A2s else 0, M1, self._table(Bs), Bs[0].stride(0), self._table(Cs),
                                              Cs[0].stride(0), M, N, K, 1 if accumulate else 0, self._stream()))

    def op_gemm_last_plan(self) -> dict:
        from ._lib import GEMM_CLASSES, GEMM_PLAN_FIELDS
        out = (C.c_int32 * 8)()
        check(self.lib.rsrgan_op_gemm_last_plan(out))
        d = dict(zip(GEMM_PLAN_FIELDS, list(out)))
        d["cls"] = GEMM_CLASSES[d["cls"]]
        return d

    def op_lstm_colsums(self, dz, cprev, ccur, db, dwi, dwf, dwo, rows, H):
        check(self.lib.rsrgan_op_lstm_colsums(len(dz), self._table(dz), self._table(cprev), self._table(ccur), self._table(db),
                                              self._table(dwi), self._table(dwf), self._table(dwo), rows, H, self._stream()))

    def op_colsum(self, a, out, rows, cols, b=None, tall=False):
        check(self.lib.rsrgan_op_colsum(_ptr(a), a.stride(0), _ptr(b), 0 if b is None else b.stride(0), _ptr(out), rows, cols,
                                        1 if tall else 0, self._stream()))
```

Measured before the change: 1.335 million.

## Fuse two-pass reductions into single kernels using last-block ticket finalization

Merges the two-kernel MSE loss, discriminator-head and sum-of-squares reductions into single launches. The last block to finish, found through an atomic ticket counter, does the final reduction. The Adam tick and loss-total updates also fold into the sumsq kernel, and a redundant copy launch is dropped when the head writes the fake loss directly. The goal is to cut kernel launch count and the serial dependencies between small kernels on the GAN step. In exchange it relies on correct atomic and fence ordering and on ticket counters that must reset themselves, and it adds small test entry points.

```diff
diff --git a/include/rsrgan.h b/include/rsrgan.h
--- a/include/rsrgan.h
+++ b/include/rsrgan.h
@@ -157,6 +157,11 @@
                            float* const* dwi, float* const* dwf, float* const* dwo, int32_t rows, int32_t H, void* stream);
 int rsrgan_op_colsum(const float* a, int32_t lda, const float* b, int32_t ldb, float* out, int32_t rows, int32_t cols, int32_t tall,
                      void* stream);
+int rsrgan_op_mse(const float* y, const float* lab, int32_t ld, float* dy, int32_t rows, int32_t D, const float* lambda, int32_t accumulate,
+                  float* loss_out, int32_t Bp, int32_t Bt, void* stream);
+int rsrgan_op_dhead(const float* top, int32_t ldt, const float* w, const float* b, int32_t T, int32_t Nd, int32_t n_real, int32_t dR,
+                    const float* t_real, const float* t_fake, float* logits, float* dlogits, float* dout, float* gw, float* gb, float* loss3,
+                    int32_t Bp, int32_t Bt, void* stream);
 
 typedef struct rsrgan_segan_cfg {
   int32_t batch_size;
diff --git a/rsrgan_amd/_lib.py b/rsrgan_amd/_lib.py
--- a/rsrgan_amd/_lib.py
+++ b/rsrgan_amd/_lib.py
@@ -23,7 +23,7 @@
            "rsrgan_grad_bucket_count", "rsrgan_grad_bucket_info", "rsrgan_grad_bucket_wait",
            "rsrgan_profile_begin", "rsrgan_profile_read", "rsrgan_profile_read_kind", "rsrgan_profile_launches", "rsrgan_op_launch_floor", "rsrgan_device_status", "rsrgan_set_dropout",
            "rsrgan_op_gemm", "rsrgan_op_gemm2", "rsrgan_op_gemm_batch", "rsrgan_op_gemm16_batch", "rsrgan_op_gemm_last_plan",
-           "rsrgan_op_lstm_colsums", "rsrgan_op_colsum", "rsrgan_version",
+           "rsrgan_op_lstm_colsums", "rsrgan_op_colsum", "rsrgan_op_mse", "rsrgan_op_dhead", "rsrgan_version",
            "rsrgan_segan_default_cfg", "rsrgan_segan_create", "rsrgan_segan_destroy", "rsrgan_segan_set_scalar",
            "rsrgan_segan_num_tensors", "rsrgan_segan_tensor_info", "rsrgan_segan_param_count", "rsrgan_segan_get_params",
            "rsrgan_segan_set_params", "rsrgan_segan_forward_g", "rsrgan_segan_d_backward", "rsrgan_segan_g_backward",
@@ -106,6 +106,8 @@
     lib.rsrgan_op_gemm_last_plan.argtypes = [C.POINTER(i32)]
     lib.rsrgan_op_lstm_colsums.argtypes = [i32, pp, pp, pp, pp, pp, pp, pp, i32, i32, vp]
     lib.rsrgan_op_colsum.argtypes = [p, i32, p, i32, p, i32, i32, i32, vp]
+    lib.rsrgan_op_mse.argtypes = [p, p, i32, p, i32, i32, p, i32, p, i32, i32, vp]
+    lib.rsrgan_op_dhead.argtypes = [p, i32, p, p, i32, i32, i32, i32, p, p, p, p, p, p, p, p, i32, i32, vp]
     lib.rsrgan_segan_default_cfg.argtypes = [C.POINTER(SeganCfg)]
     lib.rsrgan_segan_create.argtypes = [C.POINTER(SeganCfg), C.c_uint64, C.POINTER(vp)]
     lib.rsrgan_segan_destroy.argtypes = [vp]
diff --git a/rsrgan_amd/csrc/capi.cpp b/rsrgan_amd/csrc/capi.cpp
--- a/rsrgan_amd/csrc/capi.cpp
+++ b/rsrgan_amd/csrc/capi.cpp
@@ -635,4 +635,50 @@
   return RSRGAN_OK;
 }
 
-}
+static unsigned* op_tickets() {
+  static unsigned* t = nullptr;
+  if (!t) {
+    if (hipMalloc((void**)&t, 4 * sizeof(unsigned)) != hipSuccess) { t = nullptr; return nullptr; }
+    if (hipMemset(t, 0, 4 * sizeof(unsigned)) != hipSuccess) { (void)hipFree(t); t = nullptr; }
+  }
+  return t;
+}
+
+int rsrgan_op_mse(const float* y, const float* lab, int32_t ld, float* dy, int32_t rows, int32_t D, const float* lambda, int32_t accumulate,
+                  float* loss_out, int32_t Bp, int32_t Bt, void* stream) {
+  OP_REFUSE(!y || !lab || !lambda || !loss_out, "op_mse: null pointer (y, lab, lambda or loss_out)");
+  OP_REFUSE(rows <= 0 || D <= 0, "op_mse: rows and D must be positive (got %d, %d)", rows, D);
+  OP_REFUSE(ld < D, "op_mse: leading dimension %d below D = %d", ld, D);
+  OP_REFUSE(Bp < 0 || (Bp > 0 && (Bt <= 0 || Bt > Bp || rows % Bp != 0)), "op_mse: bad row padding (Bp %d, Bt %d, rows %d)", Bp, Bt, rows);
+  float* sc = op_scratch();
+  unsigned* tk = op_tickets();
+  if (!sc || !tk) { set_error("op_mse: hipMalloc failed"); return RSRGAN_ERR_HIP; }
+  launch_mse(y, lab, ld, dy, rows, D, lambda, accumulate != 0, loss_out, sc, tk + 1, (hipStream_t)stream, Bp, Bt);
+  if (hipGetLastError() != hipSuccess) { set_error("op_mse launch failed"); return RSRGAN_ERR_HIP; }
+  return RSRGAN_OK;
+}
+
+int rsrgan_op_dhead(const float* top, int32_t ldt, const float* w, const float* b, int32_t T, int32_t Nd, int32_t n_real, int32_t dR,
+                    const float* t_real, const float* t_fake, float* logits, float* dlogits, float* dout, float* gw, float* gb, float* loss3,
+                    int32_t Bp, int32_t Bt, void* stream) {
+  OP_REFUSE(!top || !w || !b || !t_real || !t_fake || !logits || !loss3, "op_dhead: null pointer (top, w, b, targets, logits or loss3)");
+  OP_REFUSE((dlogits == nullptr) != (dout == nullptr) || (gw == nullptr) != (gb == nullptr) || (gw && !dlogits),
+            "op_dhead: dlogits and dout come together, and gw and gb with them");
+  OP_REFUSE(T <= 0 || Nd <= 0 || n_real < 0 || n_real > Nd, "op_dhead: bad row counts (T %d, Nd %d, n_real %d)", T, Nd, n_real);
+  OP_REFUSE(dR <= 0 || (dR & 3) || dR + 3 > 64 || ldt < dR || (ldt & 3), "op_dhead: dR = %d (ldt %d) outside the kernel's range", dR, ldt);
+  OP_REFUSE(Bp < 0 || (Bp > 0 && (Bt <= 0 || Bt > Bp || Nd % Bp != 0 || n_real % Bp != 0)), "op_dhead: bad row padding (Bp %d, Bt %d)", Bp, Bt);
+  const size_t nb = ((size_t)T * Nd + 63) / 64;
+  OP_REFUSE(nb * (DH_MAXR + 3) > g_op_scratch_floats, "op_dhead: %zu rows exceed the entry's scratch", (size_t)T * Nd);
+  float* sc = op_scratch();
+  unsigned* tk = op_tickets();
+  if (!sc || !tk) { set_error("op_dhead: hipMalloc failed"); return RSRGAN_ERR_HIP; }
+  DHeadArgs a{};
+  a.top = top; a.ldt = ldt; a.w = w; a.ldw = 4; a.b = b; a.logits = logits; a.ldl = 4; a.dlogits = dlogits; a.dout = dout; a.ldo = ldt;
+  a.gw = gw; a.gb = gb; a.T = T; a.Nd = Nd; a.n_real = n_real; a.dR = dR; a.t_real = t_real; a.t_fake = t_fake; a.loss3 = loss3;
+  a.part = sc; a.want_grads = dlogits ? 1 : 0; a.want_wgrads = gw ? 1 : 0; a.Bp = Bp; a.Bt = Bt; a.ticket = tk; a.fake_out = nullptr;
+  launch_dhead(a, (hipStream_t)stream);
+  if (hipGetLastError() != hipSuccess) { set_error("op_dhead launch failed"); return RSRGAN_ERR_HIP; }
+  return RSRGAN_OK;
+}
+
+}
diff --git a/rsrgan_amd/csrc/dnn.cpp b/rsrgan_amd/csrc/dnn.cpp
--- a/rsrgan_amd/csrc/dnn.cpp
+++ b/rsrgan_amd/csrc/dnn.cpp
@@ -244,7 +244,7 @@
                                 : fc_backward(D, dfc, d_act, R, dlogits, false, true, s);
       launch_slice_cols(dj, ldJ, cfg.d_joint_dim, dy_buf, ldDout, R, Dout, s);
     }
-    launch_mse(y_tm, lab_tm, ldDout, dy_buf, R, Dout, dyn + DYN_LAMBDA, !sup, losses + 4, scratch, s);
+    launch_mse(y_tm, lab_tm, ldDout, dy_buf, R, Dout, dyn + DYN_LAMBDA, !sup, losses + 4, scratch, tickets + 1, s);
     g_frame_backward(R, dy_buf, s);
     if (l2_on) {
       launch_l2(G.w, G.g, G.ct, dyn + DYN_L2, G.partial, s);
@@ -253,7 +253,7 @@
     if (bn_training()) bn_commit_run(!sup, s);
     { finish_buckets(RSRGAN_NET_G, s); g_grads_ready = true; }
   } else {
-    launch_mse(y_tm, lab_tm, ldDout, nullptr, R, Dout, dyn + DYN_LAMBDA, false, losses + 4, scratch, s);
+    launch_mse(y_tm, lab_tm, ldDout, nullptr, R, Dout, dyn + DYN_LAMBDA, false, losses + 4, scratch, tickets + 1, s);
   }
   if (!(want_grads && l2_on)) HIPC(hipMemsetAsync(losses + 5, 0, sizeof(float), s));
   launch_g_total(losses + 3, dyn + DYN_LAMBDA, s);
diff --git a/rsrgan_amd/csrc/kernels.h b/rsrgan_amd/csrc/kernels.h
--- a/rsrgan_amd/csrc/kernels.h
+++ b/rsrgan_amd/csrc/kernels.h
@@ -312,6 +312,8 @@
   float* logits; int ldl; float* dlogits; float* dout; int ldo; float* gw; float* gb;
   int T, Nd, n_real, dR; const float* t_real; const float* t_fake; float* loss3; float* part; int want_grads, want_wgrads;
   int Bp, Bt;
+  unsigned* ticket;
+  float* fake_out;
 };
 void launch_dhead(const DHeadArgs& a, hipStream_t s);
 void launch_lsgan(const float* logits, int ldl, float* dlogits, int T, int Nd, int n_real,
@@ -321,7 +323,8 @@
                         int row0, int R, hipStream_t s);
 void launch_slice_cols(const float* src, int lds, int off, float* dst, int ldd, int R, int C, hipStream_t s);
 void launch_mse(const float* y, const float* lab, int ld, float* dy, int rows, int D, const float* lambda,
-                bool accumulate, float* loss_out, float* scratch , hipStream_t s, int Bp = 0, int Bt = 0);
+                bool accumulate, float* loss_out, float* scratch , unsigned* ticket ,
+                hipStream_t s, int Bp = 0, int Bt = 0);
 void launch_g_total(float* l4 , const float* lambda, hipStream_t s);
 void launch_copy_f(const float* src, float* dst, int n, hipStream_t s);
 
@@ -334,7 +337,8 @@
   const int* t_l2;
   int n_chunks, n_tensors;
 };
-void launch_sumsq(const float* g, const ChunkTable& ct, float* partial, hipStream_t s);
+struct UpdateScalars { float* l4; const float* lambda; int zero_l2; float* dyn; int* t; double b1, b2; int lr_slot, lrt_slot; };
+void launch_sumsq(const float* g, const ChunkTable& ct, float* partial, hipStream_t s, const UpdateScalars& u = UpdateScalars{});
 void launch_dw_reduce(const float* ws, size_t stride, int ntiles, const long long* src, float* g, const ChunkTable& ct, float* partial, hipStream_t s);
 void launch_l2(const float* w, float* g, const ChunkTable& ct, const float* l2_scale, float* partial, hipStream_t s);
 void launch_l2_total(const float* partial, int n_chunks, const float* l2_scale, float* out, hipStream_t s);
diff --git a/rsrgan_amd/csrc/kernels.hip b/rsrgan_amd/csrc/kernels.hip
--- a/rsrgan_amd/csrc/kernels.hip
+++ b/rsrgan_amd/csrc/kernels.hip
@@ -1522,14 +1522,37 @@
                      clip_on ? 1 : 0, clip_lo, clip_hi, Bp, Bt);
 }
 
-__global__ __launch_bounds__(64) void k_dhead1(const DHeadArgs a) {
-  __shared__ float wsh[DH_MAXR + 1];
-  const int lane = threadIdx.x;
-  const int rows = a.T * a.Nd, dR = a.dR;
-  if (lane < dR) wsh[lane] = a.w[(size_t)lane * a.ldw];
-  if (lane == 0) wsh[DH_MAXR] = a.b[0];
-  __syncthreads();
-  const int r = blockIdx.x * 64 + lane;
+__device__ __forceinline__ bool last_block_arrived(unsigned* ticket, unsigned nblocks, float* flag) {
+  asm volatile("s_waitcnt vmcnt(0)" ::: "memory");
+  __syncthreads();
+  if (threadIdx.x == 0) {
+    __builtin_amdgcn_fence(__ATOMIC_RELEASE, "agent");
+    asm volatile("s_waitcnt vmcnt(0)" ::: "memory");
+    const unsigned old = __hip_atomic_fetch_add(ticket, 1u, __ATOMIC_RELAXED, __HIP_MEMORY_SCOPE_AGENT);
+    const bool last = old + 1u == nblocks;
+    if (last) {
+      __hip_atomic_store(ticket, 0u, __ATOMIC_RELAXED, __HIP_MEMORY_SCOPE_AGENT);
+      __builtin_amdgcn_fence(__ATOMIC_ACQUIRE, "agent");
+      asm volatile("s_waitcnt vmcnt(0)" ::: "memory");
+    }
+    *flag = last ? 1.f : 0.f;
+  }
+  __syncthreads();
+  return *flag != 0.f;
+}
+
+constexpr int DH_WAVES = 4;
+__global__ __launch_bounds__(64 * DH_WAVES) void k_dhead(const DHeadArgs a) {
+  __shared__ float sm[DH_MAXR + 2 + DH_MAXR + 3];
+  float* wsh = sm;
+  float* tot = sm + DH_MAXR + 2;
+  const int lane = threadIdx.x & 63, wave = threadIdx.x >> 6;
+  const int rows = a.T * a.Nd, dR = a.dR, nwaves = (rows + 63) / 64;
+  if (threadIdx.x < dR) wsh[threadIdx.x] = a.w[(size_t)threadIdx.x * a.ldw];
+  if (threadIdx.x == 0) wsh[DH_MAXR] = a.b[0];
+  __syncthreads();
+  const int gw = blockIdx.x * DH_WAVES + wave;
+  const int r = gw * 64 + lane;
   const bool on = r < rows;
   const float tr = *a.t_real, tf = *a.t_fake;
   const int nr_ = a.Bp > 0 ? a.n_real / a.Bp * a.Bt : a.n_real, nf_ = a.Bp > 0 ? (a.Nd - a.n_real) / a.Bp * a.Bt : a.Nd - a.n_real;
@@ -1561,45 +1584,44 @@
     }
   }
   auto wsum = [&](float v) { for (int o = 32; o > 0; o >>= 1) v += __shfl_down(v, o, 64); return v; };
-  float* part = a.part + (size_t)blockIdx.x * (DH_MAXR + 3);
+  const bool wr = lane == 0 && gw < nwaves;
+  float* part = a.part + (size_t)(gw < nwaves ? gw : 0) * (DH_MAXR + 3);
   sr = wsum(sr); sf = wsum(sf);
-  if (lane == 0) { part[0] = sr; part[1] = sf; }
+  if (wr) { part[0] = sr; part[1] = sf; }
   if (a.want_wgrads) {
     const float sd = wsum(dl);
-    if (lane == 0) part[2] = sd;
+    if (wr) part[2] = sd;
 #pragma unroll
     for (int c = 0; c < DH_MAXR; ++c)
-      if (c < dR) { const float v = wsum(x[c] * dl); if (lane == 0) part[3 + c] = v; }
-  }
-}
-__global__ __launch_bounds__(1024) void k_dhead2(const DHeadArgs a, int nblocks) {
-  __shared__ float tot[DH_MAXR + 3];
-  const int q = threadIdx.x >> 4, j = threadIdx.x & 15;
-  const int nq = a.want_wgrads ? 3 + a.dR : 2;
-  float s = 0.f;
-  if (q < nq)
-    for (int b = j; b < nblocks; b += 16) s += a.part[(size_t)b * (DH_MAXR + 3) + q];
-  s += __shfl_xor(s, 8); s += __shfl_xor(s, 4); s += __shfl_xor(s, 2); s += __shfl_xor(s, 1);
-  if (q < nq && j == 0) {
-    tot[q] = s;
-    if (a.want_wgrads) {
-      if (q == 2) a.gb[0] = s;
-      if (q >= 3) a.gw[(size_t)(q - 3) * a.ldw] = s;
+      if (c < dR) { const float v = wsum(x[c] * dl); if (wr) part[3 + c] = v; }
+  }
+  if (!last_block_arrived(a.ticket, gridDim.x, sm + DH_MAXR + 1)) return;
+  const int nq = a.want_wgrads ? 3 + dR : 2;
+  const int j = threadIdx.x & 15;
+  for (int q = threadIdx.x >> 4; q < 64; q += 4 * DH_WAVES) {
+    float s = 0.f;
+    if (q < nq)
+      for (int b = j; b < nwaves; b += 16) s += a.part[(size_t)b * (DH_MAXR + 3) + q];
+    s += __shfl_xor(s, 8); s += __shfl_xor(s, 4); s += __shfl_xor(s, 2); s += __shfl_xor(s, 1);
+    if (q < nq && j == 0) {
+      tot[q] = s;
+      if (a.want_wgrads) {
+        if (q == 2) a.gb[0] = s;
+        if (q >= 3) a.gw[(size_t)(q - 3) * a.ldw] = s;
+      }
     }
   }
   __syncthreads();
   if (threadIdx.x == 0) {
-    const int nr_ = a.Bp > 0 ? a.n_real / a.Bp * a.Bt : a.n_real, nf_ = a.Bp > 0 ? (a.Nd - a.n_real) / a.Bp * a.Bt : a.Nd - a.n_real;
-    const float cr = (float)a.T * (float)nr_, cf = (float)a.T * (float)nf_;
     const float lr_ = a.n_real > 0 ? tot[0] / cr : 0.f;
     const float lf_ = (a.Nd - a.n_real) > 0 ? tot[1] / cf : 0.f;
     a.loss3[0] = lr_; a.loss3[1] = lf_; a.loss3[2] = lr_ + lf_;
+    if (a.fake_out) *a.fake_out = lf_;
   }
 }
 void launch_dhead(const DHeadArgs& a, hipStream_t s) {
-  const int rows = a.T * a.Nd, nb = (rows + 63) / 64;
-  hipLaunchKernelGGL(k_dhead1, dim3(nb), dim3(64), 0, s, a);
-  hipLaunchKernelGGL(k_dhead2, dim3(1), dim3(1024), 0, s, a, nb);
+  const int rows = a.T * a.Nd, nb = (rows + 64 * DH_WAVES - 1) / (64 * DH_WAVES);
+  hipLaunchKernelGGL(k_dhead, dim3(nb), dim3(64 * DH_WAVES), 0, s, a);
 }
 
 __global__ void k_build_joint(const float* __restrict__ x, int ldx, int off, int dim, const float* __restrict__ tail, int ldt, int Dt,
@@ -1631,10 +1653,10 @@
 }
 
 constexpr int MSE_BLOCKS = 256;
-__global__ __launch_bounds__(256) void k_mse1(const float* __restrict__ y, const float* __restrict__ lab, int ld,
-                                              float* __restrict__ dy, int rows, int D, const float* __restrict__ lambda,
-                                              int accumulate, float* __restrict__ scratch, int Bp, int Bt) {
-  __shared__ float red[16];
+__global__ __launch_bounds__(256) void k_mse(const float* __restrict__ y, const float* __restrict__ lab, int ld,
+                                             float* __restrict__ dy, int rows, int D, const float* __restrict__ lambda,
+                                             int accumulate, float* scratch, int Bp, int Bt, unsigned* ticket, float* out) {
+  __shared__ float sm[16 + 1 + MSE_BLOCKS];
   const size_t total = (size_t)rows * D;
   const int rows_eff = Bp > 0 ? rows / Bp * Bt : rows;
   const float scale = dy ? (*lambda) / (float)rows_eff : 0.f;
@@ -1647,20 +1669,21 @@
     s += d * d;
     if (dy) dy[o] = (accumulate ? dy[o] : 0.f) + scale * d;
   }
-  s = block_sum_1024(s, red);
+  s = block_sum_1024(s, sm);
   if (threadIdx.x == 0) scratch[blockIdx.x] = s;
-}
-__global__ void k_mse2(const float* __restrict__ scratch, int rows, float* __restrict__ out) {
+  if (!last_block_arrived(ticket, gridDim.x, sm + 16)) return;
+  float* part = sm + 17;
+  part[threadIdx.x] = scratch[threadIdx.x];
+  __syncthreads();
   if (threadIdx.x == 0) {
-    float s = 0.f;
-    for (int i = 0; i < MSE_BLOCKS; ++i) s += scratch[i];
-    *out = 0.5f * s / (float)rows;
+    float t = 0.f;
+    for (int i = 0; i < MSE_BLOCKS; ++i) t += part[i];
+    *out = 0.5f * t / (float)rows_eff;
   }
 }
 void launch_mse(const float* y, const float* lab, int ld, float* dy, int rows, int D, const float* lambda,
-                bool accumulate, float* loss_out, float* scratch, hipStream_t s, int Bp, int Bt) {
-  hipLaunchKernelGGL(k_mse1, dim3(MSE_BLOCKS), dim3(256), 0, s, y, lab, ld, dy, rows, D, lambda, accumulate ? 1 : 0, scratch, Bp, Bt);
-  hipLaunchKernelGGL(k_mse2, dim3(1), dim3(64), 0, s, scratch, Bp > 0 ? rows / Bp * Bt : rows, loss_out);
+                bool accumulate, float* loss_out, float* scratch, unsigned* ticket, hipStream_t s, int Bp, int Bt) {
+  hipLaunchKernelGGL(k_mse, dim3(MSE_BLOCKS), dim3(256), 0, s, y, lab, ld, dy, rows, D, lambda, accumulate ? 1 : 0, scratch, Bp, Bt, ticket, loss_out);
 }
 
 __global__ void k_g_total(float* l4, const float* lambda) {
@@ -1678,7 +1701,19 @@
 }
 
 
-__global__ __launch_bounds__(256) void k_sumsq(const float* __restrict__ g, ChunkTable ct, float* __restrict__ partial) {
+__device__ __forceinline__ void update_scalars(const UpdateScalars& u) {
+  if (u.l4) {
+    const float l2v = u.zero_l2 ? 0.f : u.l4[2];
+    u.l4[2] = l2v;
+    u.l4[3] = u.l4[0] + (*u.lambda) * u.l4[1] + l2v;
+  }
+  if (u.t) {
+    const int tt = *u.t + 1;
+    *u.t = tt;
+    u.dyn[u.lrt_slot] = (float)((double)u.dyn[u.lr_slot] * sqrt(1.0 - pow(u.b2, (double)tt)) / (1.0 - pow(u.b1, (double)tt)));
+  }
+}
+__global__ __launch_bounds__(256) void k_sumsq(const float* __restrict__ g, ChunkTable ct, float* __restrict__ partial, const UpdateScalars u) {
   __shared__ float red[16];
   const int c = blockIdx.x;
   const float* p = g + ct.off[c];
@@ -1690,9 +1725,10 @@
   }
   s = block_sum_1024(s, red);
   if (threadIdx.x == 0) partial[c] = s;
-}
-void launch_sumsq(const float* g, const ChunkTable& ct, float* partial, hipStream_t s) {
-  hipLaunchKernelGGL(k_sumsq, dim3(ct.n_chunks), dim3(256), 0, s, g, ct, partial);
+  if (c == 0 && threadIdx.x == 64) update_scalars(u);
+}
+void launch_sumsq(const float* g, const ChunkTable& ct, float* partial, hipStream_t s, const UpdateScalars& u) {
+  hipLaunchKernelGGL(k_sumsq, dim3(ct.n_chunks), dim3(256), 0, s, g, ct, partial, u);
 }
 
 __global__ __launch_bounds__(256) void k_dw_reduce(const float* __restrict__ ws, size_t stride, int ntiles, const long long* __restrict__ src,
diff --git a/rsrgan_amd/csrc/model.cpp b/rsrgan_amd/csrc/model.cpp
--- a/rsrgan_amd/csrc/model.cpp
+++ b/rsrgan_amd/csrc/model.cpp
@@ -530,6 +530,8 @@
                  hipEventCreateWithFlags(&ev_out, hipEventDisableTiming) != hipSuccess)) { (void)hipStreamDestroy(main_s); main_s = nullptr; }
   dyn = alloc<float>(DYN_COUNT); adam_t_dev = alloc<int>(1);
   losses = alloc<float>(8); tmp3 = alloc<float>(4);
+  tickets = (unsigned*)alloc<float>(4);
+  HIPC(hipMemset(tickets, 0, 4 * sizeof(unsigned)));
   size_t maxcols = 7 * (size_t)std::max(c.g_cells, c.d_cells);
   maxcols = std::max(maxcols, (size_t)Din + 4);
   maxcols = std::max(maxcols, (size_t)std::max(ldP, ldDin));
@@ -1671,7 +1673,7 @@
 }
 
 bool Model::d_head(int N, int T, int n_real, const float* t_real, const float* t_fake, float* loss3, bool want_grads, bool want_wgrads,
-                   hipStream_t s) {
+                   hipStream_t s, float* fake_out) {
   const int ldPd = pad4(dR), nb = (T * N + 63) / 64;
   if (!switches().dhead || d_dnn() || dl.empty() || dR % 4 != 0 || dR + 3 > 64 ||
       (size_t)nb * (DH_MAXR + 3) > scratch_floats) return false;
@@ -1681,6 +1683,7 @@
   a.T = T; a.Nd = N; a.n_real = n_real; a.dR = dR; a.t_real = t_real; a.t_fake = t_fake; a.loss3 = loss3; a.part = scratch;
   a.want_grads = want_grads ? 1 : 0; a.want_wgrads = want_wgrads ? 1 : 0;
   a.Bp = pad_Bp(); a.Bt = Bt;
+  a.ticket = tickets; a.fake_out = fake_out;
   launch_dhead(a, s);
   return true;
 }
@@ -1851,7 +1854,7 @@
     HIPC(hipMemsetAsync(losses + 3, 0, sizeof(float), s));
     if (want_grads) {
       float* dy = g_dC;
-      launch_mse(y_tm, lab_tm, ldDout, dy, T * B, Dout, dyn + DYN_LAMBDA, false, losses + 4, scratch, s, pad_Bp(), Bt);
+      launch_mse(y_tm, lab_tm, ldDout, dy, T * B, Dout, dyn + DYN_LAMBDA, false, losses + 4, scratch, tickets + 1, s, pad_Bp(), Bt);
       g_backward_pass(T, dy, s);
       if (l2s) {
         launch_l2(G.w, G.g, G.ct, dyn + DYN_L2, G.partial, s);
@@ -1859,7 +1862,7 @@
       }
       { finish_buckets(RSRGAN_NET_G, s); g_grads_ready = true; }
     } else {
-      launch_mse(y_tm, lab_tm, ldDout, nullptr, T * B, Dout, dyn + DYN_LAMBDA, false, losses + 4, scratch, s, pad_Bp(), Bt);
+      launch_mse(y_tm, lab_tm, ldDout, nullptr, T * B, Dout, dyn + DYN_LAMBDA, false, losses + 4, scratch, tickets + 1, s, pad_Bp(), Bt);
     }
     if (!(want_grads && l2s)) HIPC(hipMemsetAsync(losses + 5, 0, sizeof(float), s));
     launch_g_total(losses + 3, dyn + DYN_LAMBDA, s);
@@ -1921,6 +1924,10 @@
     }
     launch_g_total(losses + 3, dyn + DYN_LAMBDA, s);
   };
+  auto tail_apply = [&]() {
+    if (want_grads && l2_on) { tail_body(); apply_body(RSRGAN_NET_G, s); }
+    else apply_body(RSRGAN_NET_G, s, true);
+  };
 
   bool trail_plan = false;
   if (wave_bwd && want_grads && !d_dnn() && dl[0].ldI == ldDout && persist_backward_g(bw_chains[1], T, s, true)) {
@@ -1953,7 +1960,7 @@
       launch_colsum(dy, ldDout, nullptr, 0, G.Gd(g_fc_out_b), R, Dout, scratch, s);
     }
     g_gemm_workers = saved_w;
-    if (inl) { tail_body(); apply_body(RSRGAN_NET_G, s); }
+    if (inl) tail_apply();
   };
   run_seg(seg_key(SEG_G_MAIN, T, kbits | (trail_plan ? 64u : 0u) | (gsplit ? 128u : 0u)), s, [&]() {
   if (trail_plan) gpersist_arm_bytes(g_dA, (size_t)T * B * ldP * sizeof(float), s);
@@ -1996,20 +2003,20 @@
   if (d_dnn()) {
     d_dnn_forward_loss(T, B, 0, want_grads, tmp3, s);
   } else {
-    g_head = d_head(B, T, 0, dyn + DYN_D_REAL, dyn + DYN_D_REAL, tmp3, want_grads, false, s);
+    g_head = d_head(B, T, 0, dyn + DYN_D_REAL, dyn + DYN_D_REAL, tmp3, want_grads, false, s, losses + 3);
     if (!g_head) {
       d_logits(B, T, s);
       launch_lsgan(logits, 4, want_grads ? dlogits : nullptr, T, B, 0, dyn + DYN_D_REAL, dyn + DYN_D_REAL, tmp3, s, false, 0.f, 0.f, pad_Bp(), Bt);
     }
   }
-  launch_copy_f(tmp3 + 1, losses + 3, 1, s);
+  if (!g_head) launch_copy_f(tmp3 + 1, losses + 3, 1, s);
   if (want_grads && d_dnn()) {
     float* dyd = fc_backward(D, dfc, d_act, T * B, dlogits, false, true, s);
-    launch_mse(y_tm, lab_tm, ldDout, dyd, T * B, Dout, dyn + DYN_LAMBDA, true, losses + 4, scratch, s, pad_Bp(), Bt);
+    launch_mse(y_tm, lab_tm, ldDout, dyd, T * B, Dout, dyn + DYN_LAMBDA, true, losses + 4, scratch, tickets + 1, s, pad_Bp(), Bt);
     g_backward_pass(T, dyd, s);
   } else if (wave_bwd) {
     if (!g_head) gemm(dlogits, 4, true, D.W(d_fc_w), 4, true, d_dB, ldPd, R, dR, 1, nullptr, 0, 0.f, false, s);
-    launch_mse(y_tm, lab_tm, ldDout, dy, R, Dout, dyn + DYN_LAMBDA, false, losses + 4, scratch, s, pad_Bp(), Bt);
+    launch_mse(y_tm, lab_tm, ldDout, dy, R, Dout, dyn + DYN_LAMBDA, false, losses + 4, scratch, tickets + 1, s, pad_Bp(), Bt);
     FcStage F;
     F.offset = Ld; F.N = B; F.K = Dout; F.D = P;
     F.in = dy; F.ld_in = ldDout; F.WT = G.W(g_fc_out_w); F.y = g_dA; F.ldy = ldP; F.accumulate = false;
@@ -2057,12 +2064,12 @@
   } else if (want_grads) {
     d_backward_pass(B, T, false, true, dlogits, s, g_head);
     float* dyd = last_dx0;
-    launch_mse(y_tm, lab_tm, ldDout, dyd, T * B, Dout, dyn + DYN_LAMBDA, true, losses + 4, scratch, s, pad_Bp(), Bt);
+    launch_mse(y_tm, lab_tm, ldDout, dyd, T * B, Dout, dyn + DYN_LAMBDA, true, losses + 4, scratch, tickets + 1, s, pad_Bp(), Bt);
     g_backward_pass(T, dyd, s);
   } else {
-    launch_mse(y_tm, lab_tm, ldDout, nullptr, T * B, Dout, dyn + DYN_LAMBDA, false, losses + 4, scratch, s, pad_Bp(), Bt);
-  }
-  if (inl) { tail_body(); apply_body(RSRGAN_NET_G, s); }
+    launch_mse(y_tm, lab_tm, ldDout, nullptr, T * B, Dout, dyn + DYN_LAMBDA, false, losses + 4, scratch, tickets + 1, s, pad_Bp(), Bt);
+  }
+  if (inl) tail_apply();
   });
   if (gsplit) {
     defer_wgrads = false;
@@ -2118,7 +2125,7 @@
     bnl_forward(T, want_grads, s);
     (void)hipMemsetAsync(losses + 3, 0, sizeof(float), s);
     float* dy = want_grads ? g_dC : nullptr;
-    launch_mse(y_tm, lab_tm, ldDout, dy, T * B, Dout, dyn + DYN_LAMBDA, false, losses + 4, scratch, s, pad_Bp(), Bt);
+    launch_mse(y_tm, lab_tm, ldDout, dy, T * B, Dout, dyn + DYN_LAMBDA, false, losses + 4, scratch, tickets + 1, s, pad_Bp(), Bt);
     if (want_grads) bnl_backward(T, dy, s);
     if (l2s) {
       launch_l2(G.w, G.g, G.ct, dyn + DYN_L2, G.partial, s);
@@ -2135,20 +2142,25 @@
   return RSRGAN_OK;
 }
 
-void Model::apply_body(int net, hipStream_t s) {
+void Model::apply_body(int net, hipStream_t s, bool g_tail) {
   if (net == RSRGAN_NET_D) {
-    if (!d_partial_fresh) launch_sumsq(D.g, D.ct, D.partial, s);
+    UpdateScalars u{};
+    if (d_adam()) { u.dyn = dyn; u.t = adam_t_dev_d; u.b1 = (double)cfg.adam_beta1; u.b2 = (double)cfg.adam_beta2; u.lr_slot = DYN_D_LR; u.lrt_slot = DYN_ADAM_LRT_D; }
+    const bool fresh = d_partial_fresh;
+    if (!fresh) launch_sumsq(D.g, D.ct, D.partial, s, u);
     d_partial_fresh = false;
     if (d_adam()) {
-      launch_adam_tick(dyn, adam_t_dev_d, (double)cfg.adam_beta1, (double)cfg.adam_beta2, s, DYN_D_LR, DYN_ADAM_LRT_D);
+      if (fresh) launch_adam_tick(dyn, adam_t_dev_d, (double)cfg.adam_beta1, (double)cfg.adam_beta2, s, DYN_D_LR, DYN_ADAM_LRT_D);
       launch_apply_adam(D.w, D.g, D.m, D.v, D.ema, D.ct, D.partial, dyn, s, DYN_ADAM_LRT_D);
     } else {
       launch_apply_sgd(D.w, D.g, D.ema, D.ct, D.partial, dyn, s);
     }
     refresh_transposes(RSRGAN_NET_D, s);
   } else {
-    launch_sumsq(G.g, G.ct, G.partial, s);
-    launch_adam_tick(dyn, adam_t_dev, (double)cfg.adam_beta1, (double)cfg.adam_beta2, s);
+    UpdateScalars u{};
+    u.dyn = dyn; u.t = adam_t_dev; u.b1 = (double)cfg.adam_beta1; u.b2 = (double)cfg.adam_beta2; u.lr_slot = DYN_G_LR; u.lrt_slot = DYN_ADAM_LRT;
+    if (g_tail) { u.l4 = losses + 3; u.lambda = dyn + DYN_LAMBDA; u.zero_l2 = 1; }
+    launch_sumsq(G.g, G.ct, G.partial, s, u);
     launch_apply_adam(G.w, G.g, G.m, G.v, G.ema, G.ct, G.partial, dyn, s);
     refresh_transposes(RSRGAN_NET_G, s);
   }
diff --git a/rsrgan_amd/csrc/model.h b/rsrgan_amd/csrc/model.h
--- a/rsrgan_amd/csrc/model.h
+++ b/rsrgan_amd/csrc/model.h
@@ -264,6 +264,7 @@
   int *adam_t_dev = nullptr;
   float *losses = nullptr;
   float *tmp3 = nullptr;
+  unsigned *tickets = nullptr;
   float *scratch = nullptr;
   double scal[RSRGAN_SCALAR_COUNT_] = {0};
   bool g_fwd_valid = false;
@@ -281,14 +282,15 @@
   void g_forward_tail(int T, hipStream_t s);
   void d_logits(int N, int T, hipStream_t s);
   void d_backward_pass(int N, int T, bool want_wgrads, bool need_dx0, const float* dlog, hipStream_t s, bool head_done = false);
-  bool d_head(int N, int T, int n_real, const float* t_real, const float* t_fake, float* loss3, bool want_grads, bool want_wgrads, hipStream_t s);
+  bool d_head(int N, int T, int n_real, const float* t_real, const float* t_fake, float* loss3, bool want_grads, bool want_wgrads, hipStream_t s,
+              float* fake_out = nullptr);
   void g_backward_pass(int T, float* dy, hipStream_t s);
   int d_backward(const float* x, const float* labels, const int32_t* lengths, int T, const float* nr, const float* nf,
                  float* out_losses, bool want_grads, hipStream_t s);
   int g_backward(const float* x, const float* labels, const int32_t* lengths, int T, const float* nf,
                  float* out_losses, bool want_grads, bool reuse, hipStream_t s);
   int apply(int net, hipStream_t s);
-  void apply_body(int net, hipStream_t s);
+  void apply_body(int net, hipStream_t s, bool g_tail = false);
   int apply_inlined = 0;
   void refresh_transposes(int net, hipStream_t s);
   void refresh_swizzles(int net, hipStream_t s);
diff --git a/rsrgan_amd/engine_hip.py b/rsrgan_amd/engine_hip.py
--- a/rsrgan_amd/engine_hip.py
+++ b/rsrgan_amd/engine_hip.py
@@ -435,3 +435,11 @@
     def op_colsum(self, a, out, rows, cols, b=None, tall=False):
         check(self.lib.rsrgan_op_colsum(_ptr(a), a.stride(0), _ptr(b), 0 if b is None else b.stride(0), _ptr(out), rows, cols,
                                         1 if tall else 0, self._stream()))
+
+    def op_mse(self, y, lab, rows, D, lam, loss_out, dy=None, accumulate=False, Bp=0, Bt=0):
+        check(self.lib.rsrgan_op_mse(_ptr(y), _ptr(lab), y.stride(0), _ptr(dy), rows, D, _ptr(lam), 1 if accumulate else 0, _ptr(loss_out),
+                                     Bp, Bt, self._stream()))
+
+    def op_dhead(self, top, w, b, T, Nd, n_real, dR, t_real, t_fake, logits, loss3, dlogits=None, dout=None, gw=None, gb=None, Bp=0, Bt=0):
+        check(self.lib.rsrgan_op_dhead(_ptr(top), top.stride(0), _ptr(w), _ptr(b), T, Nd, n_real, dR, _ptr(t_real), _ptr(t_fake), _ptr(logits),
+                                       _ptr(dlogits), _ptr(dout), _ptr(gw), _ptr(gb), _ptr(loss3), Bp, Bt, self._stream()))
```

Result: no change. 1.335 million, median of 2 (+0.0%).
